# graphdeco-inria/hierarchical-3d-gaussians

Hardware: AMD Instinct MI355X
Metric: fwd+bwd frames/s @1080p, 1M Gaussians (higher is better)
Workload: dtype f32

## Files before the change

hierarchical-3d-gaussians_amd/csrc/abi.cpp:

```cpp
#include "common.h"

#include <pthread.h>
#include <sched.h>
#include <stdlib.h>
#include <time.h>
#include <string.h>

#include <atomic>
#include <cmath>
#include <mutex>
#include <vector>

namespace hgs {

enum Stage { ST_PREPROCESS_FWD = 0, ST_SCAN, ST_DUPLICATE, ST_SORT, ST_RANGES, ST_SORT_DEPTH, ST_RENDER_FWD,
             ST_MEMSET_BWD, ST_RENDER_BWD, ST_PREPROCESS_BWD, ST_SH_BATCHED, ST_COUNT };
static const char* kStageNames[ST_COUNT] = {"preprocess_fwd", "scan", "duplicate_keys", "tile_sort", "tile_ranges",
                                            "tile_depth_sort", "render_fwd", "memset_bwd", "render_bwd",
                                            "preprocess_bwd", "sh_bwd_batched"};
struct Pending { int stage; hipEvent_t a, b; };
static uint32_t g_timing = 0;
static std::mutex g_tmu;
static std::vector<Pending> g_pending;
static std::vector<hipEvent_t> g_pool;
static double g_ms[ST_COUNT];
static uint32_t g_calls[ST_COUNT];

struct StageTimer {
  int stage; hipStream_t s; hipEvent_t a = nullptr, b = nullptr; bool on;
  StageTimer(int st, hipStream_t stream) : stage(st), s(stream), on((g_timing & (1u | (2u << st))) != 0) {
    if (!on) return;
    std::lock_guard<std::mutex> lk(g_tmu);
    for (hipEvent_t* e : {&a, &b}) {
      if (!g_pool.empty()) { *e = g_pool.back(); g_pool.pop_back(); }
      else if (hipEventCreate(e) != hipSuccess) { on = false; return; }
    }
    (void)hipEventRecord(a, s);
  }
  ~StageTimer() {
    if (!on) return;
    (void)hipEventRecord(b, s);
    std::lock_guard<std::mutex> lk(g_tmu);
    g_pending.push_back({stage, a, b});
  }
};
#define HGS_TIMED(stage, stream, expr) [&]() { hgs::StageTimer _t(stage, stream); return (expr); }()

static thread_local char g_err[512] = "";

constexpr int kMaxDevices = 16;
struct ThreadHost {
  uint32_t* pinned_L = nullptr;
  hipEvent_t ev[kMaxDevices] = {};
};
static pthread_key_t g_host_key;
static pthread_once_t g_host_once = PTHREAD_ONCE_INIT;
static void thread_host_free(void* p) {
  ThreadHost* h = static_cast<ThreadHost*>(p);
  if (!h) return;
  for (int i = 0; i < kMaxDevices; ++i)
    if (h->ev[i]) (void)hipEventDestroy(h->ev[i]);
  if (h->pinned_L) (void)hipHostFree(h->pinned_L);
  delete h;
}
static void thread_host_key_init() { (void)pthread_key_create(&g_host_key, thread_host_free); }
static ThreadHost* thread_host(int device) {
  if (device < 0 || device >= kMaxDevices) return nullptr;
  (void)pthread_once(&g_host_once, thread_host_key_init);
  ThreadHost* h = static_cast<ThreadHost*>(pthread_getspecific(g_host_key));
  if (!h) {
    h = new ThreadHost();
    if (hipHostMalloc(reinterpret_cast<void**>(&h->pinned_L), sizeof(uint32_t), hipHostMallocPortable | hipHostMallocMapped) != hipSuccess) {
      thread_host_free(h);
      return nullptr;
    }
    (void)pthread_setspecific(g_host_key, h);
  }
  if (!h->ev[device] && hipEventCreateWithFlags(&h->ev[device], hipEventDisableTiming) != hipSuccess) {
    h->ev[device] = nullptr;
    return nullptr;
  }
  return h;
}

static bool blocking_waits() {
  static const bool b = getenv("HGS_BLOCKING_WAIT") != nullptr;
  return b;
}
static inline void cpu_relax() {
#if defined(__x86_64__) || defined(__i386__)
  __builtin_ia32_pause();
#elif defined(__aarch64__) || defined(__arm__)
  __asm__ __volatile__("yield");
#else
  sched_yield();
#endif
}
template <typename Query>
static bool poll_done(Query query, hipError_t* result) {
  if (blocking_waits()) return false;
  timespec t0;
  clock_gettime(CLOCK_MONOTONIC, &t0);
  for (unsigned i = 0;; ++i) {
    const hipError_t q = query();
    if (q != hipErrorNotReady) { *result = q; return true; }
    (void)hipGetLastError();
    cpu_relax();
    if ((i & 255u) == 255u) {
      timespec t;
      clock_gettime(CLOCK_MONOTONIC, &t);
      if ((t.tv_sec - t0.tv_sec) * 1000000000LL + (t.tv_nsec - t0.tv_nsec) > 200000000LL) return false;
    }
  }
}
hipError_t wait_stream(hipStream_t s) {
  hipError_t r;
  if (poll_done([&] { return hipStreamQuery(s); }, &r)) return r;
  return hipStreamSynchronize(s);
}
hipError_t wait_event(hipEvent_t e) {
  hipError_t r;
  if (poll_done([&] { return hipEventQuery(e); }, &r)) return r;
  return hipEventSynchronize(e);
}

int scan_resident_workgroups() {
  static std::atomic<int> cus[kMaxDevices];
  static const bool masked = getenv("HSA_CU_MASK") || getenv("ROC_GLOBAL_CU_MASK") || getenv("HSA_CU_MASK_SKIP_INIT");
  if (masked) return 1;
  int dev = 0;
  if (hipGetDevice(&dev) != hipSuccess || dev < 0 || dev >= kMaxDevices) return 1;
  int n = cus[dev].load(std::memory_order_relaxed);
  if (n == 0) {
    if (hipDeviceGetAttribute(&n, hipDeviceAttributeMultiprocessorCount, dev) != hipSuccess || n < 1) n = 1;
    cus[dev].store(n, std::memory_order_relaxed);
  }
  return n;
}
bool scan_split_forced() {
  static const bool b = getenv("HGS_SCAN_SPLIT") != nullptr;
  return b;
}

void set_error(const char* fmt, ...) {
  va_list ap;
  va_start(ap, fmt);
  vsnprintf(g_err, sizeof(g_err), fmt, ap);
  va_end(ap);
}

size_t GeomWs::bytes(int32_t P) {
  const size_t p = (size_t)(P > 0 ? P : 1);
  const size_t nblk = (p + kPreBlock - 1) / kPreBlock;
  const size_t jac_rows = (p + 63) / 64 * 64;
  return align_up(p * kRecFloats * 4) + align_up(p * 4) + align_up(p * 8) + 3 * align_up(p * 4) +
         align_up((nblk + 1) * 4) + align_up((nblk + 1) * kBands * 4) + align_up(jac_rows * kJacStride * 4) +
         align_up((size_t)(1 + kBands) * scan_chunks(nblk) * 8) + kAlign;
}
GeomWs GeomWs::carve_from(void* base, int32_t P) {
  const size_t p = (size_t)(P > 0 ? P : 1);
  const size_t nblk = (p + kPreBlock - 1) / kPreBlock;
  const size_t jac_rows = (p + 63) / 64 * 64;
  char* c = static_cast<char*>(base);
  GeomWs g;
  g.records = carve<float>(c, p * kRecFloats);
  g.depths = carve<float>(c, p);
  g.rects = carve<uint32_t>(c, p * 2);
  g.tiles_touched = carve<uint32_t>(c, p);
  g.offsets = carve<uint32_t>(c, p);
  g.flags = carve<uint32_t>(c, p);
  g.block_sums = carve<uint32_t>(c, nblk + 1);
  g.block_band = carve<uint32_t>(c, (nblk + 1) * kBands);
  g.shjac = carve<float>(c, jac_rows * kJacStride);
  g.scan_chain = carve<unsigned long long>(c, (size_t)(1 + kBands) * scan_chunks(nblk));
  return g;
}

size_t BinWs::bytes(uint32_t L, int32_t T) {
  const size_t l = L ? L : 1;
  const size_t tmp_sort = sort_tmp_bytes(L ? L : 1), tmp_bin = tile_bin_tmp_bytes(L, T);
  return 4 * align_up(l * 4) + align_up((size_t)T * 8) + align_up(((size_t)T * 3 + 3) * 4) + align_up(((size_t)T + 8) * 4) +
         (tmp_sort > tmp_bin ? tmp_sort : tmp_bin) + kAlign;
}
BinWs BinWs::carve_from(void* base, uint32_t L, int32_t T) {
  const size_t l = L ? L : 1;
  char* c = static_cast<char*>(base);
  BinWs b;
  b.keys_in = carve<uint32_t>(c, l);
  b.vals_in = carve<uint32_t>(c, l);
  b.keys_out = carve<uint32_t>(c, l);
  b.vals_out = carve<uint32_t>(c, l);
  b.ranges = carve<uint32_t>(c, (size_t)T * 2);
  b.big_tiles = carve<uint32_t>(c, (size_t)T * 3 + 3);
  b.tile_order = carve<uint32_t>(c, (size_t)T + 8);
  b.sort_tmp = c;
  return b;
}

size_t ImgWs::bytes(int32_t W, int32_t H) { return 2 * align_up((size_t)W * H * 4) + kAlign; }
ImgWs ImgWs::carve_from(void* base, int32_t W, int32_t H) {
  char* c = static_cast<char*>(base);
  ImgWs im;
  im.final_T = carve<float>(c, (size_t)W * H);
  im.n_contrib = carve<uint32_t>(c, (size_t)W * H);
  return im;
}

static int validate(const hgs_raster_args* a) {
  if (!a) { set_error("null args"); return HGS_ERR_INVALID; }
  if (a->P < 0 || a->width <= 0 || a->height <= 0) { set_error("bad sizes P=%d W=%d H=%d", a->P, a->width, a->height); return HGS_ERR_INVALID; }
  if (grid_x(a->width) > 1023 || grid_y(a->height) > 1023) { set_error("image larger than 16368 px per side is not supported"); return HGS_ERR_INVALID; }
  if (!a->bg || !a->viewmatrix || !a->projmatrix || !a->campos) { set_error("bg/viewmatrix/projmatrix/campos must be device pointers"); return HGS_ERR_INVALID; }
  if (a->P > 0) {
    if (!a->means3D || !a->opacities) { set_error("means3D/opacities missing"); return HGS_ERR_INVALID; }
    if ((a->shs != nullptr) == (a->colors_precomp != nullptr)) { set_error("provide exactly one of shs / colors_precomp"); return HGS_ERR_INVALID; }
    const bool sr = a->scales && a->rotations;
    if (sr == (a->cov3D_precomp != nullptr) || ((a->scales != nullptr) != (a->rotations != nullptr))) {
      set_error("provide exactly one of (scales, rotations) / cov3D_precomp");
      return HGS_ERR_INVALID;
    }
    if (a->shs) {
      if (a->sh_degree < 0 || a->sh_degree > 3) { set_error("sh_degree %d not in 0..3", a->sh_degree); return HGS_ERR_INVALID; }
      if (a->M < (a->sh_degree + 1) * (a->sh_degree + 1) || a->M > 16) { set_error("M=%d incompatible with sh_degree=%d (max 16 coefficients)", a->M, a->sh_degree); return HGS_ERR_INVALID; }
    }
    if (((uintptr_t)a->shs | (uintptr_t)a->shs_rest | (uintptr_t)a->rotations) & 15u) { set_error("shs / shs_rest / rotations must be 16-byte aligned"); return HGS_ERR_INVALID; }
    if (a->defer_sh_bwd && a->shs_rest) { set_error("defer_sh_bwd is not available with split SH storage (shs_rest)"); return HGS_ERR_INVALID; }
    if (a->shs_rest && (!a->shs || a->M < 2)) { set_error("shs_rest needs shs (features_dc) and M >= 2"); return HGS_ERR_INVALID; }
    if ((a->activations & HGS_ACT_OPACITY_SIGMOID) && (a->activations & HGS_ACT_OPACITY_ABS)) { set_error("choose one opacity activation"); return HGS_ERR_INVALID; }
    if ((a->activations & (HGS_ACT_SCALE_EXP | HGS_ACT_ROT_NORMALIZE)) && a->cov3D_precomp) { set_error("scale / rotation activations need scales and rotations"); return HGS_ERR_INVALID; }
    if ((a->interpolation_weights != nullptr) != (a->num_node_kids != nullptr)) { set_error("interpolation_weights and num_node_kids must be given together"); return HGS_ERR_INVALID; }
    if ((a->lod_render_indices != nullptr) != (a->lod_parent_indices != nullptr)) { set_error("lod_render_indices and lod_parent_indices must be given together"); return HGS_ERR_INVALID; }
    if (a->lod_render_indices) {
      if (!a->shs || a->shs_rest || !a->scales || !a->rotations || a->activations || !a->interpolation_weights) { set_error("in-kernel LOD interpolation needs shs, scales, rotations, interpolation_weights / num_node_kids and no activations"); return HGS_ERR_INVALID; }
      if (a->lod_n < 0 || a->lod_n > a->P || a->lod_rows < a->P - a->lod_n) { set_error("bad lod_n / lod_rows (P=%d lod_n=%d lod_rows=%d)", a->P, a->lod_n, a->lod_rows); return HGS_ERR_INVALID; }
      if (a->defer_sh_bwd || a->accumulate_grads) { set_error("defer_sh_bwd / accumulate_grads are not available with in-kernel LOD interpolation"); return HGS_ERR_INVALID; }
    }
  }
  return HGS_OK;
}

}

using namespace hgs;

extern "C" {

int hgs_abi_version(void) { return HGS_ABI_VERSION; }
const char* hgs_last_error(void) { return g_err; }
int hgs_device_count(void) {
  int n = 0;
  if (hipGetDeviceCount(&n) != hipSuccess) return -1;
  return n;
}

int hgs_raster_ws_sizes(int32_t P, int32_t width, int32_t height, uint32_t L, size_t* geom_bytes,
                        size_t* bin_bytes, size_t* img_bytes, size_t* bwd_bytes) {
  if (P < 0 || width <= 0 || height <= 0) { set_error("bad sizes"); return HGS_ERR_INVALID; }
  const int T = grid_x(width) * grid_y(height);
  if (geom_bytes) *geom_bytes = GeomWs::bytes(P);
  if (bin_bytes) *bin_bytes = BinWs::bytes(L, T);
  if (img_bytes) *img_bytes = ImgWs::bytes(width, height);
  if (bwd_bytes) *bwd_bytes = bwd_ws_bytes(L, P);
  return HGS_OK;
}

int hgs_raster_fwd_stage1(const hgs_raster_args* a, void* geom_ws, int32_t* radii, uint32_t* L_out_host,
                          hgs_stream_t stream, int device) {
  int rc = validate(a);
  if (rc) return rc;
  if (!geom_ws || !L_out_host || (a->P > 0 && !radii)) { set_error("null workspace/output"); return HGS_ERR_INVALID; }
  HGS_HIP(hipSetDevice(device));
  hipStream_t s = static_cast<hipStream_t>(stream);
  const GeomWs g = GeomWs::carve_from(geom_ws, a->P);
  *L_out_host = 0;
  if (a->P == 0) return HGS_OK;
  if ((rc = HGS_TIMED(ST_PREPROCESS_FWD, s, launch_preprocess_fwd(*a, g, radii, s)))) return rc;
  if ((rc = HGS_TIMED(ST_SCAN, s, launch_scan_block_sums(g, a->P, s, a->debug)))) return rc;
  const int nblk = (a->P + kPreBlock - 1) / kPreBlock;
  HGS_HIP(hipMemcpyAsync(L_out_host, g.block_sums + nblk, sizeof(uint32_t), hipMemcpyDeviceToHost, s));
  HGS_HIP(wait_stream(s));
  return HGS_OK;
}

static int enqueue_stage2(const hgs_raster_args* a, const GeomWs& g, const BinWs& b, const ImgWs& im, uint32_t L,
                          const uint32_t* L_dev, int T, float* out_color, float* out_invdepth, hipStream_t s,
                          uint32_t* super = nullptr, uint32_t* mirror = nullptr, uint32_t* stage = nullptr,
                          hipEvent_t ev = nullptr) {
  int rc;
  const bool bin = L > 0 && tile_bin_supported(T);
  if ((rc = HGS_TIMED(ST_DUPLICATE, s, launch_duplicate_tiles(*a, g, b, L, bin, s, super, mirror)))) return rc;
  if (super) {
    if (!mirror) HGS_HIP(hipMemcpyAsync(stage, L_dev, sizeof(uint32_t), hipMemcpyDeviceToHost, s));
    HGS_HIP(hipEventRecord(ev, s));
  }
  if (bin) {
    const int nblk = (a->P + kPreBlock - 1) / kPreBlock;
    if ((rc = HGS_TIMED(ST_SORT, s, launch_tile_bin(b.keys_in, b.vals_in, b.vals_out, b.sort_tmp, L, g.block_band, nblk, T, b.ranges, b.big_tiles, b.tile_order, super, s, a->debug)))) return rc;
  } else {
    if (L > 0) {
      if ((rc = HGS_TIMED(ST_SORT, s, sort_pairs32(b.keys_in, b.vals_in, b.keys_out, b.vals_out, b.sort_tmp, L, L_dev, tile_bits(T), s, a->debug)))) return rc;
    }
    if ((rc = HGS_TIMED(ST_RANGES, s, launch_tile_ranges(b, L, L_dev, T, s, a->debug)))) return rc;
  }
  if ((rc = HGS_TIMED(ST_SORT_DEPTH, s, launch_tile_depth_sort(*a, g, b, L, T, bin && a->debug, s)))) return rc;
  if (!bin && (rc = launch_tile_order(b, T, s, a->debug))) return rc;
  return HGS_TIMED(ST_RENDER_FWD, s, launch_render_fwd(*a, g, b, im, out_color, out_invdepth, s));
}

int hgs_raster_fwd_stage2(const hgs_raster_args* a, void* geom_ws, void* bin_ws, void* img_ws, uint32_t L,
                          float* out_color, float* out_invdepth, hgs_stream_t stream, int device) {
  int rc = validate(a);
  if (rc) return rc;
  if (!geom_ws || !bin_ws || !img_ws || !out_color) { set_error("null workspace/output"); return HGS_ERR_INVALID; }
  HGS_HIP(hipSetDevice(device));
  hipStream_t s = static_cast<hipStream_t>(stream);
  const int T = grid_x(a->width) * grid_y(a->height);
  const GeomWs g = GeomWs::carve_from(geom_ws, a->P);
  const BinWs b = BinWs::carve_from(bin_ws, L, T);
  const ImgWs im = ImgWs::carve_from(img_ws, a->width, a->height);
  return enqueue_stage2(a, g, b, im, L, nullptr, T, out_color, out_invdepth, s);
}

int hgs_raster_fwd(const hgs_raster_args* a, void* geom_ws, void* bin_ws, void* img_ws, uint32_t L_cap,
                   int32_t* radii, float* out_color, float* out_invdepth, uint32_t* L_out_host,
                   hgs_stream_t stream, int device) {
  int rc = validate(a);
  if (rc) return rc;
  if (!geom_ws || !bin_ws || !img_ws || !out_color || !L_out_host || (a->P > 0 && !radii)) {
    set_error("null workspace/output");
    return HGS_ERR_INVALID;
  }
  HGS_HIP(hipSetDevice(device));
  hipStream_t s = static_cast<hipStream_t>(stream);
  const int T = grid_x(a->width) * grid_y(a->height);
  const GeomWs g = GeomWs::carve_from(geom_ws, a->P);
  const BinWs b = BinWs::carve_from(bin_ws, L_cap, T);
  const ImgWs im = ImgWs::carve_from(img_ws, a->width, a->height);
  *L_out_host = 0;
  if (a->P == 0) return enqueue_stage2(a, g, b, im, 0, nullptr, T, out_color, out_invdepth, s);
  ThreadHost* th = thread_host(device);
  if (!th) { set_error("cannot allocate pinned host memory / event (device %d)", device); return HGS_ERR_NOMEM; }
  hipEvent_t ev = th->ev[device];
  uint32_t* stage = th->pinned_L;
  static const bool by_copy = getenv("HGS_COUNT_BY_COPY") != nullptr;
  void* mirror = nullptr;
  if (by_copy || hipHostGetDevicePointer(&mirror, stage, 0) != hipSuccess) { (void)hipGetLastError(); mirror = nullptr; }
  const int nblk = (a->P + kPreBlock - 1) / kPreBlock;
  uint32_t* super = nullptr;
  if (L_cap > 0 && tile_bin_supported(T) && nblk <= kSuper * kMaxSuper) super = super_block_acquire(s);
  if ((rc = HGS_TIMED(ST_PREPROCESS_FWD, s, launch_preprocess_fwd(*a, g, radii, s, super, super ? k3_heavy_threshold(L_cap, a->P) : 0u)))) {
    if (super) super_block_mark_dirty(super);
    return rc;
  }
  const uint32_t* L_dev = g.block_sums + nblk;
  hipError_t e = hipSuccess;
  if (!super) {
    if ((rc = HGS_TIMED(ST_SCAN, s, launch_scan_block_sums(g, a->P, s, a->debug, static_cast<uint32_t*>(mirror))))) return rc;
    if (!mirror) HGS_HIP(hipMemcpyAsync(stage, L_dev, sizeof(uint32_t), hipMemcpyDeviceToHost, s));
    e = hipEventRecord(ev, s);
  }
  if (e == hipSuccess) rc = enqueue_stage2(a, g, b, im, L_cap, L_dev, T, out_color, out_invdepth, s, super,
                                           static_cast<uint32_t*>(mirror), stage, ev);
  if (rc || e != hipSuccess) {
    if (super) super_block_mark_dirty(super);
    if (rc) return rc;
  }
  if (e == hipSuccess) e = wait_event(ev);
  if (e != hipSuccess) { set_error("hgs_raster_fwd: %s", hipGetErrorString(e)); return HGS_ERR_HIP; }
  *L_out_host = *stage;
  if (rc) return rc;
  if (*L_out_host > L_cap) {
    if (super) {
      HGS_HIP(hipMemsetAsync(g.scan_chain, 0, (size_t)(1 + kBands) * scan_chunks(nblk) * sizeof(unsigned long long), s));
      if ((rc = launch_scan_block_sums(g, a->P, s, a->debug, nullptr))) return rc;
    }
    set_error("instance count %u exceeds the capacity %u given to hgs_raster_fwd", *L_out_host, L_cap);
    return HGS_ERR_CAPACITY;
  }
  return HGS_OK;
}

int hgs_release_device_state(int device) { return super_block_release(device); }

int hgs_raster_bwd(const hgs_raster_args* a, const void* geom_ws, const void* bin_ws, const void* img_ws,
                   void* bwd_ws, uint32_t L, const float* out_color, const float* out_invdepth,
                   const float* dL_dcolor, const float* dL_dinvdepth, const hgs_raster_grads* grads,
                   hgs_stream_t stream, int device) {
  int rc = validate(a);
  if (rc) return rc;
  if (!geom_ws || !bin_ws || !img_ws || !bwd_ws || !out_color || !dL_dcolor || !grads) { set_error("null workspace/input"); return HGS_ERR_INVALID; }
  if (a->lod_render_indices && !a->prepare_backward) { set_error("the backward of an in-kernel LOD interpolation needs prepare_backward = 1 in the forward and the backward call"); return HGS_ERR_INVALID; }
  if (a->lod_scatter && (!a->lod_render_indices || ((a->M * 3) & 3) != 0 || a->accumulate_grads || a->defer_sh_bwd)) { set_error("lod_scatter needs in-kernel LOD interpolation, 3M %% 4 == 0, no accumulation and no deferred SH backward"); return HGS_ERR_INVALID; }
  if (a->P > 0) {
    if (!grads->dL_dmeans3D || !grads->dL_dmeans2D || !grads->dL_dopacity) { set_error("missing gradient outputs"); return HGS_ERR_INVALID; }
    if ((a->shs && !grads->dL_dshs) || (a->shs_rest && !grads->dL_dshs_rest) || (a->colors_precomp && !grads->dL_dcolors) ||
        (a->scales && (!grads->dL_dscales || !grads->dL_drotations)) || (a->cov3D_precomp && !grads->dL_dcov3D)) {
      set_error("gradient outputs do not match the inputs that were provided");
      return HGS_ERR_INVALID;
    }
  }
  HGS_HIP(hipSetDevice(device));
  hipStream_t s = static_cast<hipStream_t>(stream);
  if (a->P == 0) return HGS_OK;
  const int T = grid_x(a->width) * grid_y(a->height);
  const GeomWs g = GeomWs::carve_from(const_cast<void*>(geom_ws), a->P);
  const BinWs b = BinWs::carve_from(const_cast<void*>(bin_ws), L, T);
  const ImgWs im = ImgWs::carve_from(const_cast<void*>(img_ws), a->width, a->height);
  float* inst = static_cast<float*>(bwd_ws);
  float* drgb = bwd_ws_drgb(bwd_ws, L);
  if (L > 0) {
    if ((rc = HGS_TIMED(ST_RENDER_BWD, s, launch_render_bwd(*a, g, b, im, out_color, out_invdepth, dL_dcolor, dL_dinvdepth, inst, s)))) return rc;
  }
  hgs_raster_grads gr = *grads;
  if (!a->shs) gr.dL_dshs = nullptr;
  if (!a->shs_rest) gr.dL_dshs_rest = nullptr;
  if (!a->colors_precomp) gr.dL_dcolors = nullptr;
  if (!a->scales) { gr.dL_dscales = nullptr; gr.dL_drotations = nullptr; }
  if (!a->cov3D_precomp) gr.dL_dcov3D = nullptr;
  uint32_t* lod_flag = nullptr;
  if (a->lod_render_indices && a->lod_scatter) {
    lod_flag = bwd_ws_lod_flag(bwd_ws, L, a->P);
    HGS_HIP(hipMemsetAsync(lod_flag, 0, sizeof(uint32_t), s));
    if ((rc = launch_lod_monotone(a->lod_parent_indices, a->lod_n, lod_flag, s))) return rc;
  }
  return HGS_TIMED(ST_PREPROCESS_BWD, s, launch_preprocess_bwd(*a, g, inst, drgb, bwd_ws_dmean(bwd_ws, L, a->P), lod_flag, gr, L,
                                                             bwd_ws_work(bwd_ws, L, a->P), bwd_ws_work_counter(bwd_ws, L, a->P), s));
}

int hgs_raster_sh_bwd_batched(const hgs_sh_bwd_view* views, int32_t n_views, int32_t P, int32_t M, int32_t sh_degree,
                              const float* means3D, const float* shs, float* dL_dshs, float* dL_dmeans3D,
                              int32_t accumulate, hgs_stream_t stream, int device) {
  if (n_views <= 0 || P <= 0) return HGS_OK;
  if (!views || n_views > HGS_MAX_DEFERRED_VIEWS) { set_error("1..%d deferred views per call", HGS_MAX_DEFERRED_VIEWS); return HGS_ERR_INVALID; }
  if (!means3D || !shs || !dL_dshs || !dL_dmeans3D) { set_error("null argument"); return HGS_ERR_INVALID; }
  if (sh_degree < 0 || sh_degree > 3 || M < (sh_degree + 1) * (sh_degree + 1) || M > 16) { set_error("M=%d incompatible with sh_degree=%d", M, sh_degree); return HGS_ERR_INVALID; }
  if (((uintptr_t)shs | (uintptr_t)dL_dshs) & 15u) { set_error("shs / dL_dshs must be 16-byte aligned"); return HGS_ERR_INVALID; }
  ShBwdViews v;
  v.n = n_views;
  v.color = 0;
  for (int i = 0; i < HGS_MAX_DEFERRED_VIEWS; ++i) {
    const hgs_sh_bwd_view& w = views[i < n_views ? i : 0];
    if (!w.geom_ws || !w.bwd_ws || !w.campos) { set_error("deferred view %d has a null pointer", i); return HGS_ERR_INVALID; }
    v.mask[i] = GeomWs::carve_from(const_cast<void*>(w.geom_ws), P).tiles_touched;
    v.drgb[i] = bwd_ws_drgb(const_cast<void*>(w.bwd_ws), w.L);
    v.campos[i] = w.campos;
  }
  HGS_HIP(hipSetDevice(device));
  return HGS_TIMED(ST_SH_BATCHED, static_cast<hipStream_t>(stream),
                   launch_sh_bwd_batched(v, P, M, sh_degree, means3D, shs, dL_dshs, dL_dmeans3D, accumulate != 0,
                                         static_cast<hipStream_t>(stream)));
}

static int sh_color_check(const hgs_sh_color_view* views, int32_t n_views, int32_t M, int32_t sh_degree,
                          const float* means3D, const float* shs, bool backward) {
  if (!views || n_views > HGS_MAX_DEFERRED_VIEWS) { set_error("1..%d views per call", HGS_MAX_DEFERRED_VIEWS); return HGS_ERR_INVALID; }
  if (!means3D || !shs) { set_error("null argument"); return HGS_ERR_INVALID; }
  if (sh_degree < 0 || sh_degree > 3 || M < (sh_degree + 1) * (sh_degree + 1) || M > 16) { set_error("M=%d incompatible with sh_degree=%d", M, sh_degree); return HGS_ERR_INVALID; }
  if ((uintptr_t)shs & 15u) { set_error("shs must be 16-byte aligned"); return HGS_ERR_INVALID; }
  for (int i = 0; i < n_views; ++i)
    if (!views[i].campos || !views[i].clamp || (backward ? !views[i].d_rgb : !views[i].rgb)) { set_error("colour view %d has a null pointer", i); return HGS_ERR_INVALID; }
  return HGS_OK;
}

int hgs_sh_colors_batched(const hgs_sh_color_view* views, int32_t n_views, int32_t P, int32_t M, int32_t sh_degree,
                          const float* means3D, const float* shs, hgs_stream_t stream, int device) {
  if (n_views <= 0 || P <= 0) return HGS_OK;
  int rc = sh_color_check(views, n_views, M, sh_degree, means3D, shs, false);
  if (rc) return rc;
  ShFwdViews v;
  v.n = n_views;
  for (int i = 0; i < HGS_MAX_DEFERRED_VIEWS; ++i) {
    const hgs_sh_color_view& w = views[i < n_views ? i : 0];
    v.campos[i] = w.campos;
    v.rgb_out[i] = w.rgb;
    v.clamp_out[i] = w.clamp;
  }
  HGS_HIP(hipSetDevice(device));
  return launch_sh_colors_batched(v, P, M, sh_degree, means3D, shs, static_cast<hipStream_t>(stream));
}

int hgs_sh_colors_batched_bwd(const hgs_sh_color_view* views, int32_t n_views, int32_t P, int32_t M, int32_t sh_degree,
                              const float* means3D, const float* shs, float* dL_dshs, float* dL_dmeans3D,
                              int32_t accumulate, hgs_stream_t stream, int device) {
  if (n_views <= 0 || P <= 0) return HGS_OK;
  if (!dL_dshs || !dL_dmeans3D || ((uintptr_t)dL_dshs & 15u)) { set_error("dL_dshs (16-byte aligned) / dL_dmeans3D missing"); return HGS_ERR_INVALID; }
  int rc = sh_color_check(views, n_views, M, sh_degree, means3D, shs, true);
  if (rc) return rc;
  ShBwdViews v;
  v.n = n_views;
  v.color = 1;
  for (int i = 0; i < HGS_MAX_DEFERRED_VIEWS; ++i) {
    const hgs_sh_color_view& w = views[i < n_views ? i : 0];
    v.mask[i] = w.clamp;
    v.drgb[i] = w.d_rgb;
    v.campos[i] = w.campos;
  }
  HGS_HIP(hipSetDevice(device));
  return HGS_TIMED(ST_SH_BATCHED, static_cast<hipStream_t>(stream),
                   launch_sh_bwd_batched(v, P, M, sh_degree, means3D, shs, dL_dshs, dL_dmeans3D, accumulate != 0,
                                         static_cast<hipStream_t>(stream)));
}

int hgs_raster_views_get(int32_t P, int32_t width, int32_t height, uint32_t L, const void* geom_ws,
                         const void* bin_ws, const void* img_ws, hgs_raster_views* out) {
  if (!out || !geom_ws || !bin_ws || !img_ws) { set_error("null argument"); return HGS_ERR_INVALID; }
  const int T = grid_x(width) * grid_y(height);
  const GeomWs g = GeomWs::carve_from(const_cast<void*>(geom_ws), P);
  const BinWs b = BinWs::carve_from(const_cast<void*>(bin_ws), L, T);
  const ImgWs im = ImgWs::carve_from(const_cast<void*>(img_ws), width, height);
  out->tile_ids_sorted = b.keys_out;
  out->point_list = b.vals_out;
  out->ranges = b.ranges;
  out->tiles_touched = g.tiles_touched;
  out->offsets = g.offsets;
  out->depths = g.depths;
  out->rects = g.rects;
  out->records = g.records;
  out->final_T = im.final_T;
  out->n_contrib = im.n_contrib;
  return HGS_OK;
}

int hgs_timing_enable(int on) {
  std::lock_guard<std::mutex> lk(g_tmu);
  g_timing = (uint32_t)on;
  return HGS_OK;
}
int hgs_timing_stage_count(void) { return ST_COUNT; }
const char* hgs_timing_stage_name(int i) { return (i >= 0 && i < ST_COUNT) ? kStageNames[i] : ""; }
int hgs_timing_read(double* ms_out, uint32_t* calls_out, int reset) {
  std::lock_guard<std::mutex> lk(g_tmu);
  for (const Pending& p : g_pending) {
    float ms = 0.f;
    if (hipEventSynchronize(p.b) == hipSuccess && hipEventElapsedTime(&ms, p.a, p.b) == hipSuccess) {
      g_ms[p.stage] += ms;
      g_calls[p.stage] += 1;
    }
    g_pool.push_back(p.a);
    g_pool.push_back(p.b);
  }
  g_pending.clear();
  for (int i = 0; i < ST_COUNT; ++i) {
    if (ms_out) ms_out[i] = g_ms[i];
    if (calls_out) calls_out[i] = g_calls[i];
    if (reset) { g_ms[i] = 0.0; g_calls[i] = 0; }
  }
  return HGS_OK;
}

size_t hgs_sort_tmp_bytes(uint32_t n) { return sort_tmp_bytes(n ? n : 1); }

int hgs_sort_pairs(const uint64_t* keys_in, const uint32_t* vals_in, uint64_t* keys_out, uint32_t* vals_out,
                   void* tmp, uint32_t n, int end_bit, hgs_stream_t stream, int device) {
  if (n && (!keys_in || !vals_in || !keys_out || !vals_out || !tmp)) { set_error("null argument"); return HGS_ERR_INVALID; }
  HGS_HIP(hipSetDevice(device));
  return sort_pairs(keys_in, vals_in, keys_out, vals_out, tmp, n, end_bit, static_cast<hipStream_t>(stream), false);
}

constexpr int32_t kHierBuildMaxP = 1 << 30;

size_t hgs_hier_build_tmp_bytes(int32_t P) {
  if (P < 1 || P > kHierBuildMaxP) return 0;
  return hier_build_tmp_bytes(P);
}

int hgs_hier_build(const float* xyz, const float* scales, const float* rots, const float* opacity, const float* shs,
                   int32_t P, int32_t M, float* out_xyz, float* out_shs, float* out_alpha, float* out_log_scales,
                   float* out_rots, int32_t* out_nodes, float* out_boxes, void* tmp, hgs_stream_t stream, int device) {
  if (P < 1 || P > kHierBuildMaxP) { set_error("bad sizes: P=%d not in [1, 2^30]", P); return HGS_ERR_INVALID; }
  if (M != 1 && M != 4 && M != 9 && M != 16) { set_error("bad sizes: M=%d not in {1, 4, 9, 16}", M); return HGS_ERR_INVALID; }
  if (!xyz || !scales || !rots || !opacity || !shs || !out_xyz || !out_shs || !out_alpha || !out_log_scales ||
      !out_rots || !out_nodes || !out_boxes || !tmp) {
    set_error("null argument");
    return HGS_ERR_INVALID;
  }
  if (((uintptr_t)out_shs | (uintptr_t)out_rots | (uintptr_t)out_boxes) & 15u) { set_error("out_shs / out_rots / out_boxes must be 16-byte aligned"); return HGS_ERR_INVALID; }
  if ((uintptr_t)tmp & (kAlign - 1)) { set_error("tmp must be %d-byte aligned", (int)kAlign); return HGS_ERR_INVALID; }
  HGS_HIP(hipSetDevice(device));
  return launch_hier_build(xyz, scales, rots, opacity, shs, P, M, out_xyz, out_shs, out_alpha, out_log_scales, out_rots,
// ... 127 lines not shown
```

hierarchical-3d-gaussians_amd/csrc/binning.hip:

```cpp
#include "common.h"

#include <stdlib.h>

namespace hgs {
namespace {

__device__ __forceinline__ void divmod_rect(uint32_t k, uint32_t w, uint32_t& q, uint32_t& r) {
  q = (uint32_t)(((float)k + 0.5f) * __builtin_amdgcn_rcpf((float)w));
  r = k - q * w;
}


__device__ __forceinline__ uint32_t rect_count(uint2 r) {
  return ((r.y & 0xffffu) - (r.x & 0xffffu)) * ((r.y >> 16) - (r.x >> 16));
}

__global__ __launch_bounds__(kPreBlock) void duplicate_tiles_kernel(int P, int gx, GeomWs g, uint32_t cap,
                                                                    uint32_t* __restrict__ tile_keys,
                                                                    uint32_t* __restrict__ vals,
                                                                    uint32_t* __restrict__ ranges, int n_ranges) {
  for (int r = blockIdx.x * kPreBlock + threadIdx.x; r < n_ranges; r += gridDim.x * kPreBlock) ranges[r] = 0u;
  __shared__ uint32_t excl[kPreBlock + 1];
  __shared__ uint2 lrect[kPreBlock];
  __shared__ uint32_t wave_tot[kPreBlock / 64];
  const int tid = threadIdx.x, lane = tid & 63, wave = tid >> 6;
  const int i = blockIdx.x * kPreBlock + tid;
  const uint32_t gid = (uint32_t)i;
  const uint2 myrect = (i < P) ? reinterpret_cast<const uint2*>(g.rects)[gid] : make_uint2(0u, 0u);
  const uint32_t cnt = rect_count(myrect);
  lrect[tid] = myrect;
  uint32_t inc = cnt;
#pragma unroll
  for (int off = 1; off < 64; off <<= 1) {
    const uint32_t t = __shfl_up(inc, off, 64);
    if (lane >= off) inc += t;
  }
  if (lane == 63) wave_tot[wave] = inc;
  __syncthreads();
  uint32_t wbase = 0;
  for (int w = 0; w < wave; ++w) wbase += wave_tot[w];
  const uint32_t my_excl = wbase + inc - cnt;
  excl[tid] = my_excl;
  if (tid == kPreBlock - 1) excl[kPreBlock] = wbase + inc;
  const uint32_t block_base = g.block_sums[blockIdx.x];
  if (i < P && cnt) g.offsets[gid] = block_base + my_excl;
  __syncthreads();
  const uint32_t total = excl[kPreBlock];
  for (uint32_t s = tid; s < total; s += kPreBlock) {
    int lo = 0, hi = kPreBlock;
#pragma unroll
    for (int it = 0; it < 8; ++it) {
      const int mid = (lo + hi) >> 1;
      if (excl[mid] <= s) lo = mid; else hi = mid;
    }
    const uint32_t gg = blockIdx.x * kPreBlock + lo;
    const uint32_t k = s - excl[lo];
    const uint2 rc = lrect[lo];
    const uint32_t minx = rc.x & 0xffffu, miny = rc.x >> 16;
    const uint32_t w = (rc.y & 0xffffu) - minx;
    uint32_t kq, kr;
    divmod_rect(k, w, kq, kr);
    const uint32_t ty = miny + kq, tx = minx + kr;
    if (block_base + s < cap) {
      tile_keys[block_base + s] = ty * (uint32_t)gx + tx;
      vals[block_base + s] = gg;
    }
  }
}


template <int CTRL, int ROW_MASK>
__device__ __forceinline__ uint32_t dpp_add_u32(uint32_t v) {
  return v + (uint32_t)__builtin_amdgcn_update_dpp(0, (int)v, CTRL, ROW_MASK, 0xf, false);
}
__device__ __forceinline__ uint32_t wave_scan_incl(uint32_t v) {
  v = dpp_add_u32<0x111, 0xf>(v);
  v = dpp_add_u32<0x112, 0xf>(v);
  v = dpp_add_u32<0x114, 0xf>(v);
  v = dpp_add_u32<0x118, 0xf>(v);
  v = dpp_add_u32<0x142, 0xa>(v);
  v = dpp_add_u32<0x143, 0xc>(v);
  return v;
}

constexpr uint32_t kHeavyFloor = 4096u, kHeavyFactor = 2u, kShareMin = 1024u;

struct K3Lds {
  uint32_t pre9[1 + kBands], tot9[1 + kBands];
  uint32_t excl[kPreBlock + 1];
  uint2 lrect[kPreBlock];
  uint32_t wave_tot[kPreBlock / 64][kBands + 1];
  uint32_t bpos[kBands];
  uint32_t rb[kBands][kPreBlock];
  uint32_t hl_blk[kMaxHeavy], hl_pe[kMaxHeavy + 1];
  uint32_t scan_tmp[kPreBlock / 64];
};

__device__ __forceinline__ uint32_t k3_wg_scan_excl(uint32_t v, uint32_t* tmp, uint32_t& total) {
  const int lane = threadIdx.x & 63, wave = threadIdx.x >> 6;
  const uint32_t inc = wave_scan_incl(v);
  __syncthreads();
  if (lane == 63) tmp[wave] = inc;
  __syncthreads();
  uint32_t base = 0, t = 0;
#pragma unroll
  for (int w = 0; w < kPreBlock / 64; ++w) {
    const uint32_t x = tmp[w];
    base += (w < wave) ? x : 0u;
    t += x;
  }
  total = t;
  return base + inc - v;
}

template <bool OWN>
__device__ __forceinline__ void k3_prologue(K3Lds& l, int blk, int nblk, int P, int gx, int T, int per, const GeomWs& g,
                                            const uint32_t* __restrict__ super, uint32_t* __restrict__ total_mirror,
                                            uint32_t& heavy_n) {
  const int tid = threadIdx.x, lane = tid & 63, wave = tid >> 6;
  const int i = blk * kPreBlock + tid;
  const uint32_t gid = (uint32_t)i;
  const uint2 myrect = (i < P) ? reinterpret_cast<const uint2*>(g.rects)[gid] : make_uint2(0u, 0u);
  const int col = nblk + 1;
  uint32_t block_base = 0;
  uint32_t band_tot = 0, band_off = 0;
  heavy_n = 0u;
  if (!super) {
    block_base = g.block_sums[blk];
    if (tid < kBands) {
      band_tot = g.block_band[(size_t)tid * col + nblk];
      band_off = g.block_band[(size_t)tid * col + blk];
    }
  } else {
    const int sb = blk / kSuper, nsb = (nblk + kSuper - 1) / kSuper;
    constexpr int kWaves = kPreBlock / 64, kPer = (1 + kBands + kWaves - 1) / kWaves;
    uint32_t pre[kPer], x0[kPer];
    const int j = min(sb * kSuper + lane, blk);
#pragma unroll
    for (int u = 0; u < kPer; ++u) {
      const int a = min(wave + u * kWaves, kBands);
      const uint32_t* raw = a == 0 ? g.block_sums : g.block_band + (size_t)(a - 1) * col;
      pre[u] = raw[j];
      x0[u] = super[a * kMaxSuper + min(lane, nsb - 1)];
    }
    if constexpr (OWN) heavy_n = super[kHeavyRow];
#pragma unroll
    for (int u = 0; u < kPer; ++u) {
      const int a = min(wave + u * kWaves, kBands);
      uint32_t p = (sb * kSuper + lane < blk) ? pre[u] : 0u;
      uint32_t tot = (lane < nsb) ? x0[u] : 0u;
      p += (lane < sb) ? tot : 0u;
      for (int s0 = 64; s0 < nsb; s0 += 64) {
        const uint32_t x = (s0 + lane < nsb) ? super[a * kMaxSuper + s0 + lane] : 0u;
        tot += x;
        p += (s0 + lane < sb) ? x : 0u;
      }
      p = wave_scan_incl(p);
      tot = wave_scan_incl(tot);
      if (lane == 63) { l.pre9[a] = p; l.tot9[a] = tot; }
    }
  }
  const uint32_t cnt = rect_count(myrect);
  l.lrect[tid] = myrect;
  uint32_t cb[kBands];
#pragma unroll
  for (int b = 0; b < kBands; ++b) cb[b] = 0u;
  if (cnt) {
    const int minx = (int)(myrect.x & 0xffffu), miny = (int)(myrect.x >> 16);
    const int maxx = (int)(myrect.y & 0xffffu), maxy = (int)(myrect.y >> 16);
    const int w = maxx - minx;
    const int t_first = miny * gx + minx, t_last = (maxy - 1) * gx + maxx - 1;
    int b_first = 0, b_last = 0;
#pragma unroll
    for (int b = 1; b < kBands; ++b) {
      b_first += (t_first >= b * per) ? 1 : 0;
      b_last += (t_last >= b * per) ? 1 : 0;
    }
    if (b_first == b_last) {
#pragma unroll
      for (int b = 0; b < kBands; ++b) cb[b] = (b == b_first) ? cnt : 0u;
    } else {
      int prev = 0;
#pragma unroll
      for (int b = 0; b < kBands; ++b) {
        const int x = min((b + 1) * per, T);
        const int xr = x / gx, xc = x - xr * gx;
        int c = (min(max(xr, miny), maxy) - miny) * w;
        if (xr >= miny && xr < maxy) c += min(max(xc - minx, 0), w);
        cb[b] = (uint32_t)(c - prev);
        prev = c;
      }
    }
  }
  const uint32_t inc = wave_scan_incl(cnt);
  uint32_t incb[kBands];
#pragma unroll
  for (int b = 0; b < kBands; ++b) incb[b] = wave_scan_incl(cb[b]);
  if (lane == 63) {
    l.wave_tot[wave][kBands] = inc;
#pragma unroll
    for (int b = 0; b < kBands; ++b) l.wave_tot[wave][b] = incb[b];
  }
  if (!super && wave == 0) {
    const uint32_t incl = wave_scan_incl(tid < kBands ? band_tot : 0u);
    if (tid < kBands) l.bpos[tid] = incl - band_tot + band_off;
  }
  __syncthreads();
  if (super) {
    block_base = l.pre9[0];
    if (wave == 0) {
      if (tid < kBands) { band_tot = l.tot9[1 + tid]; band_off = l.pre9[1 + tid]; }
      const uint32_t incl = wave_scan_incl(tid < kBands ? band_tot : 0u);
      if (tid < kBands) l.bpos[tid] = incl - band_tot + band_off;
    }
    if (OWN && blk == nblk - 1 && tid <= kBands) {
      uint32_t* arr = tid == 0 ? g.block_sums : g.block_band + (size_t)(tid - 1) * col;
      arr[nblk] = l.tot9[tid];
      if (tid == 0 && total_mirror) *total_mirror = l.tot9[0];
    }
  }
  uint32_t wbase = 0;
  for (int w = 0; w < wave; ++w) wbase += l.wave_tot[w][kBands];
  const uint32_t my_excl = wbase + inc - cnt;
  l.excl[tid] = my_excl;
  if (tid == kPreBlock - 1) l.excl[kPreBlock] = wbase + inc;
  {
    uint32_t below = 0;
#pragma unroll
    for (int b = 0; b < kBands; ++b) {
      uint32_t wb = 0;
      for (int w = 0; w < wave; ++w) wb += l.wave_tot[w][b];
      l.rb[b][tid] = wb + incb[b] - cb[b] - below;
      below += cb[b];
    }
  }
  if (OWN && i < P && cnt) g.offsets[gid] = block_base + my_excl;
  __syncthreads();
}

__device__ __attribute__((noinline)) void k3_prologue_other(K3Lds* l, int blk, int nblk, int P, int gx, int T, int per,
                                                            uint32_t* rects, uint32_t* block_sums, uint32_t* block_band,
                                                            const uint32_t* super) {
  GeomWs g{};
  g.rects = rects;
  g.block_sums = block_sums;
  g.block_band = block_band;
  uint32_t unused;
  k3_prologue<false>(*l, blk, nblk, P, gx, T, per, g, super, nullptr, unused);
}

__device__ __forceinline__ void k3_emit(const K3Lds& l, int blk, uint32_t s_begin, uint32_t s_end, int gx, int per,
                                        uint32_t cap, uint32_t* __restrict__ tile_keys, uint32_t* __restrict__ vals) {
  const float rcp_per = __builtin_amdgcn_rcpf((float)per);
  for (uint32_t s = s_begin + threadIdx.x; s < s_end; s += kPreBlock) {
    int lo = 0, hi = kPreBlock;
#pragma unroll
    for (int it = 0; it < 8; ++it) {
      const int mid = (lo + hi) >> 1;
      if (l.excl[mid] <= s) lo = mid; else hi = mid;
    }
    const uint32_t gg = (uint32_t)blk * kPreBlock + lo;
    const uint32_t k = s - l.excl[lo];
    const uint2 rc = l.lrect[lo];
    const uint32_t minx = rc.x & 0xffffu, miny = rc.x >> 16;
    const uint32_t w = (rc.y & 0xffffu) - minx;
    uint32_t kq, kr;
    divmod_rect(k, w, kq, kr);
    const uint32_t tile = (miny + kq) * (uint32_t)gx + minx + kr;
    const uint32_t band = (uint32_t)(((float)tile + 0.5f) * rcp_per);
    const uint32_t pos = l.bpos[band] + l.rb[band][lo] + k;
    if (pos < cap) {
      tile_keys[pos] = tile - band * (uint32_t)per;
      vals[pos] = gg;
    }
  }
}

__global__ __launch_bounds__(kPreBlock) void duplicate_tiles_banded_kernel(int P, int gx, int T, int per, GeomWs g,
                                                                           uint32_t cap,
                                                                           uint32_t* __restrict__ tile_keys,
                                                                           uint32_t* __restrict__ vals,
                                                                           uint32_t* __restrict__ ranges, int n_ranges,
                                                                           const uint32_t* __restrict__ super,
                                                                           uint32_t* __restrict__ total_mirror,
                                                                           uint32_t* __restrict__ zero_words, int n_zero,
                                                                           int share_max, uint32_t thr) {
  for (int r = blockIdx.x * kPreBlock + threadIdx.x; r < n_ranges; r += gridDim.x * kPreBlock) ranges[r] = 0u;
  for (int r = blockIdx.x * kPreBlock + threadIdx.x; r < n_zero; r += gridDim.x * kPreBlock) zero_words[r] = 0u;
  __shared__ K3Lds l;
  const int tid = threadIdx.x, nblk = (int)gridDim.x, own = (int)blockIdx.x;
  uint32_t heavy_n;
  k3_prologue<true>(l, own, nblk, P, gx, T, per, g, super, total_mirror, heavy_n);
  const uint32_t total = l.excl[kPreBlock];
  if (!(super && share_max > 0 && thr != 0u && heavy_n != 0u)) {
    k3_emit(l, own, 0u, total, gx, per, cap, tile_keys, vals);
    return;
  }
  const int nh = (int)min(min(heavy_n, (uint32_t)kMaxHeavy), (uint32_t)share_max);
  if (tid < nh) {
    l.hl_blk[tid] = super[kHeavyRow + 1 + 2 * tid];
    l.hl_pe[tid] = super[kHeavyRow + 2 + 2 * tid] - thr;
  }
  __syncthreads();
  const uint32_t e = tid < nh ? l.hl_pe[tid] : 0u;
  const bool mine_listed = tid < nh && l.hl_blk[tid] == (uint32_t)own;
  uint32_t E;
  const uint32_t pe = k3_wg_scan_excl(e, l.scan_tmp, E);
  if (tid < nh) l.hl_pe[tid] = pe;
  if (tid == 0) l.hl_pe[nh] = E;
  const bool own_listed = __syncthreads_or(mine_listed) != 0;
  k3_emit(l, own, 0u, own_listed ? thr : total, gx, per, cap, tile_keys, vals);
  const uint64_t q = max((uint64_t)kShareMin, ((uint64_t)E + (uint64_t)nblk - 1u) / (uint64_t)nblk);
  const uint64_t lo = (uint64_t)own * q, hi = min(lo + q, (uint64_t)E);
  if (lo >= hi) return;
#pragma nounroll
  for (int i = 0; i < nh; ++i) {
    const uint64_t p0 = (uint32_t)__builtin_amdgcn_readfirstlane((int)l.hl_pe[i]);
    const uint64_t p1 = (uint32_t)__builtin_amdgcn_readfirstlane((int)l.hl_pe[i + 1]);
    if (p1 <= lo) continue;
    if (p0 >= hi) break;
    const int blk = __builtin_amdgcn_readfirstlane((int)l.hl_blk[i]);
    const uint32_t s0 = thr + (uint32_t)(max(lo, p0) - p0), s1 = thr + (uint32_t)(min(hi, p1) - p0);
    __syncthreads();
    k3_prologue_other(&l, blk, nblk, P, gx, T, per, g.rects, g.block_sums, g.block_band, super);
    k3_emit(l, blk, s0, s1, gx, per, cap, tile_keys, vals);
  }
}

constexpr uint32_t kLargeCap = 16384;

template <typename T>
__device__ __forceinline__ void cmp_swap(T& a, T& b, bool up) {
  const bool sw = (a > b) == up;
  const T lo = sw ? b : a, hi = sw ? a : b;
  a = lo;
  b = hi;
}

template <int LX>
__device__ __forceinline__ uint32_t lane_xor32(uint32_t v, int lane) {
  if constexpr (LX == 1) {
    return (uint32_t)__builtin_amdgcn_mov_dpp((int)v, 0xB1, 0xf, 0xf, true);
  } else if constexpr (LX == 2) {
    return (uint32_t)__builtin_amdgcn_mov_dpp((int)v, 0x4E, 0xf, 0xf, true);
  } else if constexpr (LX == 8) {
    return (uint32_t)__builtin_amdgcn_mov_dpp((int)v, 0x128, 0xf, 0xf, true);
  } else if constexpr (LX == 16) {
    const auto r = __builtin_amdgcn_permlane16_swap(v, v, false, false);
    return (lane & 16) ? r[0] : r[1];
  } else if constexpr (LX == 32) {
    const auto r = __builtin_amdgcn_permlane32_swap(v, v, false, false);
    return (lane & 32) ? r[0] : r[1];
  } else {
    return (uint32_t)__shfl_xor((int)v, LX, 64);
  }
}
template <int LX>
__device__ __forceinline__ uint64_t lane_xor64(uint64_t v, int lane) {
  return ((uint64_t)lane_xor32<LX>((uint32_t)(v >> 32), lane) << 32) | lane_xor32<LX>((uint32_t)v, lane);
}

template <int LX>
__device__ __forceinline__ uint64_t lane_xor(uint64_t v, int lane) { return lane_xor64<LX>(v, lane); }
template <int LX>
__device__ __forceinline__ uint32_t lane_xor(uint32_t v, int lane) { return lane_xor32<LX>(v, lane); }

template <int E, int K, int J, typename T>
__device__ __forceinline__ void wave_sort_stage(T (&key)[E], int lane, uint32_t base) {
  if constexpr (J >= E) {
    constexpr int LX = J / E;
    const bool lower = (lane & LX) == 0;
// ... 675 lines not shown
```

hierarchical-3d-gaussians_amd/csrc/common.h:

```cpp
#pragma once
#include <hip/hip_runtime.h>
#include <stdint.h>
#include <stddef.h>
#include <stdio.h>
#include <stdarg.h>

#include "../../include/hgs.h"

namespace hgs {

void set_error(const char* fmt, ...);

#define HGS_HIP(call)                                                                   \
  do {                                                                                  \
    hipError_t _e = (call);                                                             \
    if (_e != hipSuccess) {                                                             \
      hgs::set_error("%s:%d: %s -> %s", __FILE__, __LINE__, #call, hipGetErrorString(_e)); \
      return HGS_ERR_HIP;                                                               \
    }                                                                                   \
  } while (0)

#define HGS_LAUNCH_CHECK(name, stream, debug)                                           \
  do {                                                                                  \
    hipError_t _e = hipGetLastError();                                                  \
    if (_e == hipSuccess && (debug)) _e = hipStreamSynchronize(stream);                 \
    if (_e != hipSuccess) {                                                             \
      hgs::set_error("kernel %s failed: %s", name, hipGetErrorString(_e));              \
      return HGS_ERR_HIP;                                                               \
    }                                                                                   \
  } while (0)

constexpr size_t kAlign = 256;
inline size_t align_up(size_t x) { return (x + kAlign - 1) / kAlign * kAlign; }

template <typename T>
inline T* carve(char*& p, size_t count) {
  T* r = reinterpret_cast<T*>(p);
  p += align_up(count * sizeof(T));
  return r;
}

constexpr int kTile = HGS_TILE;
constexpr int kRecFloats = 16;
constexpr int kRecVec = kRecFloats / 4;
constexpr int kInstStride = HGS_INST_GRAD_STRIDE;
constexpr int kJacStride = 9;
constexpr int kPreBlock = 256;
constexpr int kBands = 8;
__host__ __device__ inline int band_tiles(int T) { return (T + kBands - 1) / kBands; }

struct GeomWs {
  float* records;
  float* depths;
  uint32_t* rects;
  uint32_t* tiles_touched;
  uint32_t* offsets;
  uint32_t* flags;
  uint32_t* block_sums;
  uint32_t* block_band;
  float* shjac;
  unsigned long long* scan_chain;
  static size_t bytes(int32_t P);
  static GeomWs carve_from(void* base, int32_t P);
};

struct BinWs {
  uint32_t* keys_in;
  uint32_t* vals_in;
  uint32_t* keys_out;
  uint32_t* vals_out;
  uint32_t* ranges;
  uint32_t* big_tiles;
  uint32_t* tile_order;
  void* sort_tmp;
  static size_t bytes(uint32_t L, int32_t T);
  static BinWs carve_from(void* base, uint32_t L, int32_t T);
};

struct ImgWs {
  float* final_T;
  uint32_t* n_contrib;
  static size_t bytes(int32_t W, int32_t H);
  static ImgWs carve_from(void* base, int32_t W, int32_t H);
};

inline int grid_x(int W) { return (W + kTile - 1) / kTile; }
inline int grid_y(int H) { return (H + kTile - 1) / kTile; }
inline int tile_bits(int T) {
  int b = 0;
  while ((1 << b) < T) ++b;
  return b < 1 ? 1 : b;
}

constexpr int kScanPer = 8;
constexpr int kScanChunk = 1024 * kScanPer;
__host__ __device__ inline int scan_chunks(size_t n) { return (int)((n + kScanChunk - 1) / kScanChunk) + (n == 0 ? 1 : 0); }

#ifdef __HIPCC__
__device__ __forceinline__ uint32_t chained_scan_inplace(uint32_t* __restrict__ sums, int n,
                                                         unsigned long long* __restrict__ chain, int c_off = 0,
                                                         int chunks_all = 0) {
  __shared__ uint32_t scan_wave_tot[16];
  __shared__ uint32_t scan_prefix;
  const int tid = threadIdx.x, lane = tid & 63, wave = tid >> 6;
  const int c = (int)blockIdx.x + c_off, chunks = chunks_all ? chunks_all : (int)gridDim.x;
  const int i0 = c * kScanChunk + tid * kScanPer;
  uint32_t v[kScanPer], mine = 0;
#pragma unroll
  for (int k = 0; k < kScanPer; ++k) v[k] = sums[max(min(i0 + k, n - 1), 0)];
#pragma unroll
  for (int k = 0; k < kScanPer; ++k) {
    v[k] = (i0 + k < n) ? v[k] : 0u;
    mine += v[k];
  }
  uint32_t inc = mine;
#pragma unroll
  for (int off = 1; off < 64; off <<= 1) {
    const uint32_t t = __shfl_up(inc, off, 64);
    if (lane >= off) inc += t;
  }
  if (lane == 63) scan_wave_tot[wave] = inc;
  __syncthreads();
  uint32_t wbase = 0, total = 0;
#pragma unroll
  for (int w = 0; w < 16; ++w) {
    const uint32_t t = scan_wave_tot[w];
    wbase += (w < wave) ? t : 0u;
    total += t;
  }
  if (tid == 0) __hip_atomic_store(&chain[c], (1ull << 32) | (unsigned long long)total, __ATOMIC_RELEASE, __HIP_MEMORY_SCOPE_AGENT);
  if (wave == 0) {
    uint32_t before = 0;
    for (int q = lane; q < c; q += 64) {
      unsigned long long x;
      do { x = __hip_atomic_load(&chain[q], __ATOMIC_ACQUIRE, __HIP_MEMORY_SCOPE_AGENT); } while ((x >> 32) == 0ull);
      before += (uint32_t)x;
    }
#pragma unroll
    for (int off = 32; off > 0; off >>= 1) before += __shfl_xor(before, off, 64);
    if (lane == 0) scan_prefix = before;
  }
  __syncthreads();
  const uint32_t prefix = scan_prefix;
  uint32_t run = prefix + wbase + inc - mine;
#pragma unroll
  for (int k = 0; k < kScanPer; ++k) {
    if (i0 + k < n) sums[i0 + k] = run;
    run += v[k];
  }
  if (c != chunks - 1) return 0u;
  if (tid == 0) sums[n] = prefix + total;
  return prefix + total;
}
#endif

hipError_t wait_stream(hipStream_t s);
hipError_t wait_event(hipEvent_t e);

int scan_resident_workgroups();
bool scan_split_forced();

int launch_preprocess_fwd(const hgs_raster_args& a, const GeomWs& g, int32_t* radii, hipStream_t s,
                          uint32_t* super = nullptr, uint32_t heavy_thr = 0);
constexpr int kSuper = 64;
constexpr int kMaxSuper = 1024;
constexpr int kMaxHeavy = 256;
constexpr int kHeavyRow = (1 + kBands) * kMaxSuper;
static_assert(1 + 2 * kMaxHeavy <= kMaxSuper, "the heavy list fits the row");
uint32_t k3_heavy_threshold(uint32_t L_cap, int32_t P);
uint32_t* super_block_acquire(hipStream_t s);
size_t super_block_bytes();
void super_block_mark_dirty(const uint32_t* words);
int super_block_release(int device);
int launch_scan_block_sums(const GeomWs& g, int32_t P, hipStream_t s, bool debug, uint32_t* total_mirror = nullptr);
int launch_duplicate_tiles(const hgs_raster_args& a, const GeomWs& g, const BinWs& b, uint32_t L_cap, bool banded,
                           hipStream_t s, const uint32_t* super = nullptr, uint32_t* total_mirror = nullptr);
uint32_t* tile_bin_zero_words(void* tmp, uint32_t L_cap, int32_t T);
int tile_bin_zero_count(int32_t T);
int launch_tile_ranges(const BinWs& b, uint32_t L_cap, const uint32_t* L_dev, int32_t T, hipStream_t s, bool debug);
int launch_tile_order(const BinWs& b, int32_t T, hipStream_t s, bool debug);
int launch_tile_depth_sort(const hgs_raster_args& a, const GeomWs& g, const BinWs& b, uint32_t L, int32_t T,
                           bool fill_tile_ids, hipStream_t s);
int launch_render_fwd(const hgs_raster_args& a, const GeomWs& g, const BinWs& b, const ImgWs& im,
                      float* out_color, float* out_invdepth, hipStream_t s);
int launch_render_bwd(const hgs_raster_args& a, const GeomWs& g, const BinWs& b, const ImgWs& im,
                      const float* out_color, const float* out_invdepth, const float* dL_dcolor,
                      const float* dL_dinvdepth, float* inst_grads, hipStream_t s);
int launch_preprocess_bwd(const hgs_raster_args& a, const GeomWs& g, const float* inst_grads, float* drgb,
                          float* dmean_rows, const uint32_t* lod_flag, const hgs_raster_grads& out, uint32_t L,
                          uint2* work, uint32_t* work_counter, hipStream_t s);
int launch_lod_monotone(const int32_t* parent_indices, int32_t n, uint32_t* flag, hipStream_t s);
struct ShBwdViews {
  const void* mask[HGS_MAX_DEFERRED_VIEWS];
  const float* drgb[HGS_MAX_DEFERRED_VIEWS];
  const float* campos[HGS_MAX_DEFERRED_VIEWS];
  int n;
  int color;
};
struct ShFwdViews {
  const float* campos[HGS_MAX_DEFERRED_VIEWS];
  float* rgb_out[HGS_MAX_DEFERRED_VIEWS];
  uint8_t* clamp_out[HGS_MAX_DEFERRED_VIEWS];
  int n;
};
int launch_sh_colors_batched(const ShFwdViews& v, int32_t P, int32_t M, int32_t sh_degree, const float* means3D,
                             const float* shs, hipStream_t s);
int launch_sh_bwd_batched(const ShBwdViews& v, int32_t P, int32_t M, int32_t sh_degree, const float* means3D,
                          const float* shs, float* dL_dshs, float* dL_dmeans3D, bool accumulate, hipStream_t s);
inline float* bwd_ws_drgb(void* bwd_ws, uint32_t L) {
  return reinterpret_cast<float*>(static_cast<char*>(bwd_ws) + align_up((size_t)(L ? L : 1) * kInstStride * 4));
}
inline float* bwd_ws_dmean(void* bwd_ws, uint32_t L, int32_t P) {
  return reinterpret_cast<float*>(reinterpret_cast<char*>(bwd_ws_drgb(bwd_ws, L)) + align_up((size_t)(P > 0 ? P : 1) * 3 * 4));
}
inline uint32_t* bwd_ws_lod_flag(void* bwd_ws, uint32_t L, int32_t P) {
  return reinterpret_cast<uint32_t*>(reinterpret_cast<char*>(bwd_ws_dmean(bwd_ws, L, P)) + align_up((size_t)(P > 0 ? P : 1) * 3 * 4));
}
constexpr uint32_t kK8LongRun = 48;
constexpr uint32_t kK8Seg = 512;
inline uint32_t* bwd_ws_work_counter(void* bwd_ws, uint32_t L, int32_t P) { return bwd_ws_lod_flag(bwd_ws, L, P) + 16; }
inline uint2* bwd_ws_work(void* bwd_ws, uint32_t L, int32_t P) {
  return reinterpret_cast<uint2*>(reinterpret_cast<char*>(bwd_ws_lod_flag(bwd_ws, L, P)) + kAlign);
}
inline size_t bwd_ws_work_items(uint32_t L) { return (size_t)(L ? L : 1) / kK8LongRun + 2; }
inline size_t bwd_ws_bytes(uint32_t L, int32_t P) {
  return align_up((size_t)(L ? L : 1) * kInstStride * 4) + 2 * align_up((size_t)(P > 0 ? P : 1) * 3 * 4) + 2 * kAlign +
         align_up(bwd_ws_work_items(L) * sizeof(uint2));
}
bool tile_bin_supported(int32_t T);
size_t tile_bin_tmp_bytes(uint32_t L, int32_t T);
int launch_tile_bin(const uint32_t* keys, const uint32_t* vals, uint32_t* vals_out, void* tmp, uint32_t L_cap,
                    const uint32_t* band_totals, int32_t nblk, int32_t T, uint32_t* ranges, uint32_t* big,
                    uint32_t* tile_order, uint32_t* super, hipStream_t s, bool debug);
size_t sort_tmp_bytes(uint32_t n);
int sort_pairs(const uint64_t* keys_in, const uint32_t* vals_in, uint64_t* keys_out, uint32_t* vals_out,
               void* tmp, uint32_t n, int end_bit, hipStream_t s, bool debug);
int sort_pairs32(const uint32_t* keys_in, const uint32_t* vals_in, uint32_t* keys_out, uint32_t* vals_out,
                 void* tmp, uint32_t n, const uint32_t* n_dev, int end_bit, hipStream_t s, bool debug);
size_t hier_build_tmp_bytes(int32_t P);
int launch_hier_build(const float* xyz, const float* scales, const float* rots, const float* opacity, const float* shs,
                      int32_t P, int32_t M, float* out_xyz, float* out_shs, float* out_alpha, float* out_log_scales,
                      float* out_rots, int32_t* out_nodes, float* out_boxes, void* tmp, hipStream_t s);
int launch_hier_merge_place(const hgs_hier_view& chunk, int32_t index, int64_t base, const hgs_hier_view& merged,
                            void* tmp, hgs_hier_merge_report* report, hipStream_t s);
int launch_hier_merge_root(const hgs_hier_view& merged, int32_t k, hipStream_t s);
size_t hier_align_tmp_bytes(int64_t N);
int launch_hier_align(const int32_t* nodes, int64_t N, float* log_scales, float* rots, void* tmp,
                      hgs_hier_align_report* report, hipStream_t s);
bool ssim_sizes_ok(int32_t N, int32_t C, int32_t H, int32_t W);
size_t ssim_tmp_bytes(int32_t N, int32_t C, int32_t H, int32_t W);
int launch_ssim_fwd(const float* img1, const float* img2, int32_t N, int32_t C, int32_t H, int32_t W,
                    float* out_image, float* out_mean, float* maps, void* tmp, hipStream_t s);
int launch_ssim_bwd(const float* img1, const float* img2, const float* maps, const float* grad_out, int32_t per_image,
                    int32_t N, int32_t C, int32_t H, int32_t W, float* grad_img1, hipStream_t s);
size_t photo_tmp_bytes(int32_t N, int32_t C, int32_t H, int32_t W);
int launch_photo_fwd(const hgs_photo_args& a, float* out, float* maps, void* tmp, hipStream_t s);
int launch_photo_bwd(const hgs_photo_args& a, const float* maps, const float* grad_out, float* grad_rendered,
                     float* grad_exposure, float* grad_invdepth, void* tmp, hipStream_t s);

}
```

hierarchical-3d-gaussians_amd/csrc/gaussian_math.h:

```cpp
#pragma once
#include "common.h"

namespace hgs {

struct Proj {
  float tx, ty, tz;
  float hx, hy, hw, pw;
  float txc, tyc;
  bool clampx, clampy;
  float fx, fy;
  float J00, J02, J11, J12;
  float T0[3], T1[3];
  float U0[3], U1[3];
  float c3[6];
  float a, b, c, det;
  float conA, conB, conC;
  float px, py;
  float rad_f;
  int minx, miny, maxx, maxy;
  bool visible;
};

__device__ __forceinline__ void quat_to_rot(const float q[4], float R[9]) {
#pragma clang fp contract(off)
// ... 84 lines not shown
#pragma unroll
  for (int j = 0; j < 3; ++j) {
    o.U0[j] = (o.T0[0] * S[0][j] + o.T0[1] * S[1][j]) + o.T0[2] * S[2][j];
    o.U1[j] = (o.T1[0] * S[0][j] + o.T1[1] * S[1][j]) + o.T1[2] * S[2][j];
  }
  o.a = ((o.U0[0] * o.T0[0] + o.U0[1] * o.T0[1]) + o.U0[2] * o.T0[2]) + 0.3f;
  o.b = (o.U0[0] * o.T1[0] + o.U0[1] * o.T1[1]) + o.U0[2] * o.T1[2];
  o.c = ((o.U1[0] * o.T1[0] + o.U1[1] * o.T1[1]) + o.U1[2] * o.T1[2]) + 0.3f;
  o.det = o.a * o.c - o.b * o.b;
  if (o.det == 0.0f) o.visible = false;
  const float det_inv = 1.0f / o.det;
  o.conA = o.c * det_inv;
  o.conB = (-o.b) * det_inv;
  o.conC = o.a * det_inv;

  const float mid = 0.5f * (o.a + o.c);
  const float disc = fmaxf(0.1f, mid * mid - o.det);
  const float sq = sqrtf(disc);
  const float lam = fmaxf(mid + sq, mid - sq);
  o.rad_f = ceilf(3.0f * sqrtf(lam));
  o.px = ((ndcx + 1.0f) * (float)W - 1.0f) * 0.5f;
  o.py = ((ndcy + 1.0f) * (float)H - 1.0f) * 0.5f;
  o.minx = tile_clamp(o.px - o.rad_f, gx);
  o.maxx = tile_clamp(o.px + o.rad_f + 15.0f, gx);
  o.miny = tile_clamp(o.py - o.rad_f, gy);
  o.maxy = tile_clamp(o.py + o.rad_f + 15.0f, gy);
  const bool finite = (fabsf(o.rad_f) <= 3.0e38f) && (fabsf(o.px) <= 3.0e38f) && (fabsf(o.py) <= 3.0e38f);
  if (!finite || (o.maxx - o.minx) * (o.maxy - o.miny) <= 0) o.visible = false;
}


__device__ __forceinline__ double rcp_d(double d) {
  const double r = (double)__builtin_amdgcn_rcpf((float)d);
  return fma(fma(-d, r, 1.0), r, r);
}

struct ProjD {
  double tx, ty, tz, hx, hy, hw, pw, itz, di;
  double txc, tyc, fx, fy;
  double T0[3], T1[3], U0[3], U1[3];
  double c3[6];
  double R[9], s[3];
  double a, b, c, det, conA, conB, conC;
  double px, py;
};

__device__ __forceinline__ void cov3d_from_scale_rot_d(const float sc[3], float mod, const float q[4], ProjD& o) {
  const double r = q[0], x = q[1], y = q[2], z = q[3];
  o.s[0] = (double)mod * sc[0];
  o.s[1] = (double)mod * sc[1];
  o.s[2] = (double)mod * sc[2];
  double* R = o.R;
  R[0] = 1.0 - 2.0 * (y * y + z * z); R[1] = 2.0 * (x * y - r * z);       R[2] = 2.0 * (x * z + r * y);
  R[3] = 2.0 * (x * y + r * z);       R[4] = 1.0 - 2.0 * (x * x + z * z); R[5] = 2.0 * (y * z - r * x);
  R[6] = 2.0 * (x * z - r * y);       R[7] = 2.0 * (y * z + r * x);       R[8] = 1.0 - 2.0 * (x * x + y * y);
  double L[9];
#pragma unroll
  for (int i = 0; i < 3; ++i)
#pragma unroll
    for (int k = 0; k < 3; ++k) L[i * 3 + k] = R[i * 3 + k] * o.s[k];
  int n = 0;
#pragma unroll
  for (int i = 0; i < 3; ++i)
#pragma unroll
    for (int j = i; j < 3; ++j)
      o.c3[n++] = L[i * 3 + 0] * L[j * 3 + 0] + L[i * 3 + 1] * L[j * 3 + 1] + L[i * 3 + 2] * L[j * 3 + 2];
}

__device__ __forceinline__ void project_gaussian_d(const float p[3], const float* vm, const float* pm, int W, int H,
                                                   float tanfovx, float tanfovy, bool clampx, bool clampy,
                                                   ProjD& o) {
  const double x = p[0], y = p[1], z = p[2];
  o.tx = (double)vm[0] * x + (double)vm[4] * y + (double)vm[8] * z + (double)vm[12];
  o.ty = (double)vm[1] * x + (double)vm[5] * y + (double)vm[9] * z + (double)vm[13];
  o.tz = (double)vm[2] * x + (double)vm[6] * y + (double)vm[10] * z + (double)vm[14];
  o.hx = (double)pm[0] * x + (double)pm[4] * y + (double)pm[8] * z + (double)pm[12];
  o.hy = (double)pm[1] * x + (double)pm[5] * y + (double)pm[9] * z + (double)pm[13];
  o.hw = (double)pm[3] * x + (double)pm[7] * y + (double)pm[11] * z + (double)pm[15];
  o.pw = rcp_d(o.hw + 1e-7);
  o.px = ((o.hx * o.pw + 1.0) * (double)W - 1.0) * 0.5;
  o.py = ((o.hy * o.pw + 1.0) * (double)H - 1.0) * 0.5;
  o.fx = (double)W / (2.0 * (double)tanfovx);
  o.fy = (double)H / (2.0 * (double)tanfovy);
  const double limx = 1.3 * (double)tanfovx, limy = 1.3 * (double)tanfovy;
  o.txc = clampx ? (o.tx < 0.0 ? -limx : limx) * o.tz : o.tx;
  o.tyc = clampy ? (o.ty < 0.0 ? -limy : limy) * o.tz : o.ty;
  const double itz = o.itz = rcp_d(o.tz);
  const double J00 = o.fx * itz, J02 = -(o.fx * o.txc) * itz * itz;
  const double J11 = o.fy * itz, J12 = -(o.fy * o.tyc) * itz * itz;
#pragma unroll
  for (int j = 0; j < 3; ++j) {
    o.T0[j] = J00 * (double)vm[j * 4 + 0] + J02 * (double)vm[j * 4 + 2];
    o.T1[j] = J11 * (double)vm[j * 4 + 1] + J12 * (double)vm[j * 4 + 2];
  }
  const double* c3 = o.c3;
  const double S[3][3] = {{c3[0], c3[1], c3[2]}, {c3[1], c3[3], c3[4]}, {c3[2], c3[4], c3[5]}};
#pragma unroll
  for (int j = 0; j < 3; ++j) {
    o.U0[j] = o.T0[0] * S[0][j] + o.T0[1] * S[1][j] + o.T0[2] * S[2][j];
    o.U1[j] = o.T1[0] * S[0][j] + o.T1[1] * S[1][j] + o.T1[2] * S[2][j];
  }
  o.a = o.U0[0] * o.T0[0] + o.U0[1] * o.T0[1] + o.U0[2] * o.T0[2] + 0.3;
  o.b = o.U0[0] * o.T1[0] + o.U0[1] * o.T1[1] + o.U0[2] * o.T1[2];
  o.c = o.U1[0] * o.T1[0] + o.U1[1] * o.T1[1] + o.U1[2] * o.T1[2] + 0.3;
  o.det = o.a * o.c - o.b * o.b;
  const double di = o.di = rcp_d(o.det);
  o.conA = o.c * di;
  o.conB = -o.b * di;
  o.conC = o.a * di;
}

struct LodRow {
  size_t r, p;
  float w, u;
};
template <bool LOD>
__device__ __forceinline__ LodRow lod_row(const hgs_raster_args& a, int idx) {
  LodRow l;
  if constexpr (!LOD) { l.r = l.p = (size_t)idx; l.w = 1.0f; l.u = 0.0f; return l; }
  if (idx < a.lod_n) {
    l.r = (size_t)a.lod_render_indices[idx];
    l.p = (size_t)a.lod_parent_indices[idx];
    l.w = a.interpolation_weights[idx];
    l.u = 1.0f - l.w;
  } else {
    l.r = l.p = (size_t)(a.lod_rows - (a.P - a.lod_n) + (idx - a.lod_n));
    l.w = 1.0f; l.u = 0.0f;
  }
  return l;
}
template <bool LOD>
__device__ __forceinline__ LodRow lod_row_gather(const hgs_raster_args& a, int idx) {
  LodRow l = lod_row<LOD>(a, idx);
  if constexpr (LOD) {
    if (l.w == 1.0f) l.p = l.r;
  }
  return l;
}
__device__ __forceinline__ float lod_lerp(float x, float y, float w, float u) {
#pragma clang fp contract(off)
  const float a = w * x, b = u * y;
  return a + b;
}
template <bool LOD>
__device__ __forceinline__ void load_mean(const hgs_raster_args& a, const LodRow& l, float p[3]) {
#pragma unroll
  for (int k = 0; k < 3; ++k) {
    const float x = a.means3D[l.r * 3 + k];
    if constexpr (LOD) p[k] = lod_lerp(x, a.means3D[l.p * 3 + k], l.w, l.u);
    else p[k] = x;
  }
}

template <bool LOD>
__device__ __forceinline__ void load_scale_rot(const hgs_raster_args& a, int idx, float sc[3], float q[4],
                                               double* nrm) {
  if constexpr (LOD) {
    const LodRow l = lod_row_gather<true>(a, idx);
#pragma unroll
    for (int k = 0; k < 3; ++k) sc[k] = lod_lerp(a.scales[l.r * 3 + k], a.scales[l.p * 3 + k], l.w, l.u);
    const float4 qa = reinterpret_cast<const float4*>(a.rotations)[l.r];
    float4 qb = reinterpret_cast<const float4*>(a.rotations)[l.p];
    const float sgn = (qa.x * qb.x + qa.y * qb.y + qa.z * qb.z + qa.w * qb.w) < 0.0f ? -1.0f : 1.0f;
    q[0] = lod_lerp(qa.x, sgn * qb.x, l.w, l.u); q[1] = lod_lerp(qa.y, sgn * qb.y, l.w, l.u);
    q[2] = lod_lerp(qa.z, sgn * qb.z, l.w, l.u); q[3] = lod_lerp(qa.w, sgn * qb.w, l.w, l.u);
    if (nrm) *nrm = 1.0;
    return;
  }
  sc[0] = a.scales[idx * 3 + 0]; sc[1] = a.scales[idx * 3 + 1]; sc[2] = a.scales[idx * 3 + 2];
  if (a.activations & HGS_ACT_SCALE_EXP) {
#pragma unroll
    for (int i = 0; i < 3; ++i) sc[i] = (float)exp((double)sc[i]);
  }
  const float4 qv = reinterpret_cast<const float4*>(a.rotations)[idx];
  q[0] = qv.x; q[1] = qv.y; q[2] = qv.z; q[3] = qv.w;
  double n = 1.0;
  if (a.activations & HGS_ACT_ROT_NORMALIZE) {
    const double w = q[0], x = q[1], y = q[2], z = q[3];
    n = fmax(sqrt(((w * w + x * x) + y * y) + z * z), 1e-12);
    q[0] = (float)(w / n); q[1] = (float)(x / n); q[2] = (float)(y / n); q[3] = (float)(z / n);
  }
  if (nrm) *nrm = n;
}

template <bool LOD>
__device__ __forceinline__ float load_opacity(const hgs_raster_args& a, int idx, double* dact) {
  if constexpr (LOD) {
    const LodRow l = lod_row_gather<true>(a, idx);
    if (dact) *dact = 1.0;
    return lod_lerp(a.opacities[l.r], a.opacities[l.p], l.w, l.u);
  }
  const float raw = a.opacities[idx];
  if (a.activations & HGS_ACT_OPACITY_SIGMOID) {
    const double o = 1.0 / (1.0 + exp(-(double)raw));
    if (dact) *dact = o * (1.0 - o);
    return (float)o;
  }
  if (a.activations & HGS_ACT_OPACITY_ABS) {
    if (dact) *dact = raw > 0.f ? 1.0 : (raw < 0.f ? -1.0 : 0.0);
    return fabsf(raw);
  }
  if (dact) *dact = 1.0;
  return raw;
}

__device__ __forceinline__ float lod_opacity(float o, float w, int kids, float* dout_do) {
  if (kids < 2) {
    if (dout_do) *dout_do = 1.0f;
    return o;
  }
  const float invk = 1.0f / (float)kids;
  const float oc = fminf(o, 0.99f);
  const float base = 1.0f - oc;
  const float pw = powf(base, invk);
  if (dout_do) {
    const float dstack = (o < 0.99f) ? invk * pw / base : 0.0f;
    *dout_do = w + (1.0f - w) * dstack;
  }
  return w * o + (1.0f - w) * (1.0f - pw);
}

__device__ __forceinline__ float unit_dir(const float p[3], const float* cam, float& dx, float& dy, float& dz) {
#pragma clang fp contract(off)
  dx = p[0] - cam[0]; dy = p[1] - cam[1]; dz = p[2] - cam[2];
  const float inv = 1.0f / sqrtf((dx * dx + dy * dy) + dz * dz);
  dx *= inv; dy *= inv; dz *= inv;
  return inv;
}

constexpr float SH_C0 = 0.28209479177387814f;
constexpr float SH_C1 = 0.4886025119029199f;
constexpr float SH_C2_0 = 1.0925484305920792f;
constexpr float SH_C2_1 = -1.0925484305920792f;
constexpr float SH_C2_2 = 0.31539156525252005f;
constexpr float SH_C2_3 = -1.0925484305920792f;
constexpr float SH_C2_4 = 0.5462742152960396f;
constexpr float SH_C3_0 = -0.5900435899266435f;
constexpr float SH_C3_1 = 2.890611442640554f;
constexpr float SH_C3_2 = -0.4570457994644658f;
constexpr float SH_C3_3 = 0.3731763325901154f;
constexpr float SH_C3_4 = -0.4570457994644658f;
constexpr float SH_C3_5 = 1.445305721320277f;
constexpr float SH_C3_6 = -0.5900435899266435f;

__device__ __forceinline__ void sh_basis(int deg, float x, float y, float z, float b[16]) {
#pragma clang fp contract(off)
  b[0] = SH_C0;
  if (deg > 0) {
    b[1] = -SH_C1 * y;
    b[2] = SH_C1 * z;
    b[3] = -SH_C1 * x;
    if (deg > 1) {
      const float xx = x * x, yy = y * y, zz = z * z, xy = x * y, yz = y * z, xz = x * z;
      b[4] = SH_C2_0 * xy;
      b[5] = SH_C2_1 * yz;
      b[6] = SH_C2_2 * (2.0f * zz - xx - yy);
      b[7] = SH_C2_3 * xz;
      b[8] = SH_C2_4 * (xx - yy);
      if (deg > 2) {
        b[9] = SH_C3_0 * y * (3.0f * xx - yy);
        b[10] = SH_C3_1 * xy * z;
        b[11] = SH_C3_2 * y * (4.0f * zz - xx - yy);
        b[12] = SH_C3_3 * z * (2.0f * zz - 3.0f * xx - 3.0f * yy);
        b[13] = SH_C3_4 * x * (4.0f * zz - xx - yy);
        b[14] = SH_C3_5 * z * (xx - yy);
        b[15] = SH_C3_6 * x * (xx - 3.0f * yy);
      }
    }
  }
}

__device__ __forceinline__ void sh_basis_grad(int deg, float x, float y, float z, float dbx[16],
                                              float dby[16], float dbz[16]) {
#pragma clang fp contract(off)
  dbx[0] = dby[0] = dbz[0] = 0.0f;
  if (deg > 0) {
    dbx[1] = 0.0f;      dby[1] = -SH_C1;    dbz[1] = 0.0f;
    dbx[2] = 0.0f;      dby[2] = 0.0f;      dbz[2] = SH_C1;
    dbx[3] = -SH_C1;    dby[3] = 0.0f;      dbz[3] = 0.0f;
    if (deg > 1) {
      const float xx = x * x, yy = y * y, zz = z * z, xy = x * y, yz = y * z, xz = x * z;
      dbx[4] = SH_C2_0 * y;          dby[4] = SH_C2_0 * x;          dbz[4] = 0.0f;
      dbx[5] = 0.0f;                 dby[5] = SH_C2_1 * z;          dbz[5] = SH_C2_1 * y;
      dbx[6] = SH_C2_2 * -2.0f * x;  dby[6] = SH_C2_2 * -2.0f * y;  dbz[6] = SH_C2_2 * 4.0f * z;
      dbx[7] = SH_C2_3 * z;          dby[7] = 0.0f;                 dbz[7] = SH_C2_3 * x;
      dbx[8] = SH_C2_4 * 2.0f * x;   dby[8] = SH_C2_4 * -2.0f * y;  dbz[8] = 0.0f;
      if (deg > 2) {
        dbx[9] = SH_C3_0 * 6.0f * xy;               dby[9] = SH_C3_0 * (3.0f * xx - 3.0f * yy);      dbz[9] = 0.0f;
        dbx[10] = SH_C3_1 * yz;                     dby[10] = SH_C3_1 * xz;                          dbz[10] = SH_C3_1 * xy;
        dbx[11] = SH_C3_2 * -2.0f * xy;             dby[11] = SH_C3_2 * (4.0f * zz - xx - 3.0f * yy); dbz[11] = SH_C3_2 * 8.0f * yz;
        dbx[12] = SH_C3_3 * -6.0f * xz;             dby[12] = SH_C3_3 * -6.0f * yz;                  dbz[12] = SH_C3_3 * (6.0f * zz - 3.0f * xx - 3.0f * yy);
        dbx[13] = SH_C3_4 * (4.0f * zz - 3.0f * xx - yy); dby[13] = SH_C3_4 * -2.0f * xy;            dbz[13] = SH_C3_4 * 8.0f * xz;
        dbx[14] = SH_C3_5 * 2.0f * xz;              dby[14] = SH_C3_5 * -2.0f * yz;                  dbz[14] = SH_C3_5 * (xx - yy);
        dbx[15] = SH_C3_6 * (3.0f * xx - 3.0f * yy); dby[15] = SH_C3_6 * -6.0f * xy;                 dbz[15] = 0.0f;
      }
    }
  }
}

}
```

hierarchical-3d-gaussians_amd/csrc/preprocess.hip:

```cpp
#include "gaussian_math.h"

#include <stdlib.h>

#include <mutex>

namespace hgs {

namespace {

struct CamLds {
  float vm[16];
  float pm[16];
  float cam[3];
};

__device__ __forceinline__ void load_camera(const hgs_raster_args& a, CamLds& c) {
#pragma unroll
  for (int i = 0; i < 16; ++i) {
    c.vm[i] = a.viewmatrix[i];
    c.pm[i] = a.projmatrix[i];
  }
  c.cam[0] = a.campos[0];
  c.cam[1] = a.campos[1];
  c.cam[2] = a.campos[2];
// ... 277 lines not shown
  const char* src = reinterpret_cast<const char*>(shs + (size_t)block_first * 48);
  const int wave_base = (int)(threadIdx.x & ~63u);
  constexpr int kPer = 12;
#pragma unroll
  for (int k = 0; k < kPer; ++k) {
    const int slot = k * kPreBlock + (int)threadIdx.x;
    const int row_l = slot / 12, cs = slot - row_l * 12;
    int c = cs - ((row_l >> 2) & 3);
    c = c < 0 ? c + 12 : c;
    const int row = row_l;
    char* dst = reinterpret_cast<char*>(lds) + (size_t)(k * kPreBlock + wave_base) * 16;
    if (row < count && c < nchunks)
      __builtin_amdgcn_global_load_lds((gptr_t)(src + (size_t)row * 192 + c * 16), (lptr_t)dst, 16, 0, 0);
  }
}
template <int Q>
__device__ __forceinline__ void sh48_read_row_quarter(const float* lds, int row_l, float v[12]) {
  const int f = (row_l >> 2) & 3;
  const float* row = lds + row_l * 48;
#pragma unroll
  for (int c = 0; c < 3; ++c) {
    int sl = Q * 3 + c + f;
    sl = sl >= 12 ? sl - 12 : sl;
    const float4 t = *reinterpret_cast<const float4*>(row + sl * 4);
    v[c * 4 + 0] = t.x; v[c * 4 + 1] = t.y; v[c * 4 + 2] = t.z; v[c * 4 + 3] = t.w;
  }
}
template <bool JAC>
__device__ __forceinline__ void sh48_row_from_lds(const float* lds, int row_l, bool vis, int deg, float dx, float dy,
                                                  float dz, float rgb[3], float J[9]) {
  const int nb = (deg + 1) * (deg + 1);
  float sh[12];
  sh48_read_row_quarter<0>(lds, row_l, sh);
  if (vis) sh48_accumulate4<JAC, 0>(deg, dx, dy, dz, sh, rgb, J);
  if (nb > 4) {
    sh48_read_row_quarter<1>(lds, row_l, sh);
    if (vis) sh48_accumulate4<JAC, 4>(deg, dx, dy, dz, sh, rgb, J);
    if (nb > 8) {
      sh48_read_row_quarter<2>(lds, row_l, sh);
      if (vis) sh48_accumulate4<JAC, 8>(deg, dx, dy, dz, sh, rgb, J);
      sh48_read_row_quarter<3>(lds, row_l, sh);
      if (vis) sh48_accumulate4<JAC, 12>(deg, dx, dy, dz, sh, rgb, J);
    }
  }
}

__device__ __forceinline__ void k1_band_count(const Proj& pr, uint32_t touched, int gx, int gy, uint32_t* band_cnt) {
  const int T = gx * gy, per = band_tiles(T), w = pr.maxx - pr.minx;
  const int t_first = pr.miny * gx + pr.minx, t_last = (pr.maxy - 1) * gx + pr.maxx - 1;
  int b_first = 0, b_last = 0;
#pragma unroll
  for (int b = 1; b < kBands; ++b) {
    b_first += (t_first >= b * per) ? 1 : 0;
    b_last += (t_last >= b * per) ? 1 : 0;
  }
  if (b_first == b_last) {
    atomicAdd(&band_cnt[b_first], touched);
  } else {
    int prev = 0;
    for (int b = b_first; b <= b_last; ++b) {
      const int x = min((b + 1) * per, T);
      const int xr = x / gx, xc = x - xr * gx;
      int cnt = (min(max(xr, pr.miny), pr.maxy) - pr.miny) * w;
      if (xr >= pr.miny && xr < pr.maxy) cnt += min(max(xc - pr.minx, 0), w);
      if (cnt > prev) atomicAdd(&band_cnt[b], (uint32_t)(cnt - prev));
      prev = cnt;
    }
  }
}

struct K1Rec {
  float opac, thr, ext_x, ext_y, invz;
  float gx_hi, gy_hi, gx_lo, gy_lo, A2, B2, C2;
};
__device__ __forceinline__ void k1_continuous(const hgs_raster_args& a, const CamLds& cam, const Proj& pr,
                                              const float p[3], const float sc_act[3], const float q_act[4],
                                              float opac, K1Rec& o) {
  o.opac = opac;
  ProjD pd;
  if (a.cov3D_precomp) {
#pragma unroll
    for (int i = 0; i < 6; ++i) pd.c3[i] = (double)pr.c3[i];
  } else {
    cov3d_from_scale_rot_d(sc_act, a.scale_modifier, q_act, pd);
  }
  project_gaussian_d(p, cam.vm, cam.pm, a.width, a.height, a.tanfovx, a.tanfovy, pr.clampx, pr.clampy, pd);
  o.gx_hi = (float)pd.px; o.gy_hi = (float)pd.py;
  o.gx_lo = (float)(pd.px - (double)o.gx_hi); o.gy_lo = (float)(pd.py - (double)o.gy_hi);
  const double kLog2e = 1.4426950408889634;
  o.A2 = (float)(-0.5 * kLog2e * pd.conA);
  o.B2 = (float)(-kLog2e * pd.conB);
  o.C2 = (float)(-0.5 * kLog2e * pd.conC);
  {
    const double lim = 4.0 * (double)o.A2 * (double)o.C2;
    if (!((double)o.B2 * (double)o.B2 < lim)) o.B2 = (float)copysign(sqrt(fmax(lim, 0.0)) * (1.0 - 1.0e-6), (double)o.B2);
  }
  o.thr = (-7.994353436858858f - 1.0e-3f) - __builtin_amdgcn_logf(opac);
  o.ext_x = -1.0f; o.ext_y = -1.0f;
  {
    const float T2 = -1.3862943611198906f * o.thr;
    const float sxx = (float)pd.a, syy = (float)pd.c;
    if (T2 > 0.0f) {
      const bool sane = sxx < 3.0e38f && syy < 3.0e38f;
      o.ext_x = sane ? sqrtf(T2 * sxx) * 1.0001f + 5.0e-3f : 1.0e9f;
      o.ext_y = sane ? sqrtf(T2 * syy) * 1.0001f + 5.0e-3f : 1.0e9f;
    }
  }
  o.invz = (float)pd.itz;
}

template <int NV>
__device__ __forceinline__ void wave_store_rows(float4* __restrict__ dst, size_t row0, const float4 (&v)[NV],
                                                unsigned long long mask, float4* wave_lds) {
  const int lane = threadIdx.x & 63;
#pragma unroll
  for (int q = 0; q < NV; ++q) wave_lds[lane * NV + q] = v[q];
  __builtin_amdgcn_fence(__ATOMIC_RELEASE, "wavefront");
  __builtin_amdgcn_wave_barrier();
  __builtin_amdgcn_fence(__ATOMIC_ACQUIRE, "wavefront");
#pragma unroll
  for (int j = 0; j < NV; ++j) {
    const int i = j * 64 + lane;
    const int r = i / NV;
    const float4 t = wave_lds[i];
    if ((mask >> r) & 1ull) dst[row0 * NV + i] = t;
  }
  __builtin_amdgcn_fence(__ATOMIC_RELEASE, "wavefront");
  __builtin_amdgcn_wave_barrier();
}

__device__ __forceinline__ void wave_store_jac(float* __restrict__ dst, size_t row0, const float (&J)[9],
                                               unsigned long long mask, float4* wave_lds) {
  const int lane = threadIdx.x & 63;
  float* wl = reinterpret_cast<float*>(wave_lds);
#pragma unroll
  for (int k = 0; k < 9; ++k) wl[lane * 9 + k] = J[k];
  __builtin_amdgcn_fence(__ATOMIC_RELEASE, "wavefront");
  __builtin_amdgcn_wave_barrier();
  __builtin_amdgcn_fence(__ATOMIC_ACQUIRE, "wavefront");
  float4* d4 = reinterpret_cast<float4*>(dst + row0 * kJacStride);
  if (mask) {
#pragma unroll
    for (int j = 0; j < 3; ++j) {
      const int i = j * 64 + lane;
      if (i < 64 * 9 / 4) d4[i] = wave_lds[i];
    }
  }
  __builtin_amdgcn_fence(__ATOMIC_RELEASE, "wavefront");
  __builtin_amdgcn_wave_barrier();
}

template <bool JAC, bool LOD, bool DEFER, bool H48>
__device__ __forceinline__ void preprocess_fwd_body(const hgs_raster_args& a, const GeomWs& g,
                                                    int32_t* __restrict__ radii, uint32_t* __restrict__ super, uint32_t heavy_thr) {
  static_assert(!(H48 && (LOD || DEFER)), "the DMA route is the plain layout's");
  extern __shared__ __attribute__((aligned(16))) unsigned char smem_raw[];
  float* lds_sh = reinterpret_cast<float*>(smem_raw);
  __shared__ uint32_t wave_tot[kPreBlock / 64];
  __shared__ uint32_t band_cnt[kBands];
  if (threadIdx.x < kBands) band_cnt[threadIdx.x] = 0u;
  if (!super && blockIdx.x == 0)
    for (int t = threadIdx.x; t < (1 + kBands) * scan_chunks(gridDim.x); t += kPreBlock) g.scan_chain[t] = 0ull;
  __syncthreads();
  const int idx = blockIdx.x * kPreBlock + threadIdx.x;
  const int gx = (a.width + kTile - 1) / kTile;
  const int gy = (a.height + kTile - 1) / kTile;
  CamLds cam;
  load_camera(a, cam);

  uint32_t touched = 0;
  Proj pr;
  pr.visible = false;
  float p[3] = {0.f, 0.f, 0.f};
  float sc_act[3] = {0.f, 0.f, 0.f}, q_act[4] = {1.f, 0.f, 0.f, 0.f};
  float opac = 0.f;
  constexpr bool lod = LOD;
  const int shn = a.M * 3;
  if (idx < a.P) {
    const LodRow lr = lod_row_gather<LOD>(a, idx);
    load_mean<LOD>(a, lr, p);
    if (lod && a.shs && (shn & 3) == 0) {
      float* pad = lds_sh + threadIdx.x * sh_row_stride(shn) + shn;
      pad[0] = __uint_as_float((uint32_t)lr.r); pad[1] = __uint_as_float((uint32_t)lr.p); pad[2] = lr.w;
    }
    if constexpr (H48) {
      opac = load_opacity<LOD>(a, idx, nullptr);
      if (a.interpolation_weights && a.num_node_kids && !a.lod_per_pixel)
        opac = lod_opacity(opac, a.interpolation_weights[idx], a.num_node_kids[idx], nullptr);
    }
    if (a.cov3D_precomp) {
#pragma unroll
      for (int i = 0; i < 6; ++i) pr.c3[i] = a.cov3D_precomp[(size_t)idx * 6 + i];
    } else {
      load_scale_rot<LOD>(a, idx, sc_act, q_act, nullptr);
      float R[9], s[3];
      cov3d_from_scale_rot(sc_act, a.scale_modifier, q_act, pr.c3, R, s);
    }
    project_gaussian(p, cam.vm, cam.pm, a.width, a.height, a.tanfovx, a.tanfovy, gx, gy, pr);
  }
  if (idx < a.P && pr.visible) {
    touched = (uint32_t)((pr.maxx - pr.minx) * (pr.maxy - pr.miny));
    k1_band_count(pr, touched, gx, gy, band_cnt);
  }
  {
    const uint32_t ws = wave_sum_u32(touched);
    if ((threadIdx.x & 63) == 0) wave_tot[threadIdx.x >> 6] = ws;
  }
  bool coop = false, deferred = false;
  const bool sh_lds = a.shs && (shn & 3) == 0;
  const int nvis = __syncthreads_count(pr.visible);
  if (threadIdx.x < 64) {
    uint32_t mine = 0;
    if (threadIdx.x == 0) {
#pragma unroll
      for (int w = 0; w < kPreBlock / 64; ++w) mine += wave_tot[w];
      g.block_sums[blockIdx.x] = mine;
    } else if (threadIdx.x <= kBands) {
      mine = band_cnt[threadIdx.x - 1];
      g.block_band[(size_t)(threadIdx.x - 1) * (gridDim.x + 1) + blockIdx.x] = mine;
    }
    if (super && threadIdx.x <= kBands && mine)
      __hip_atomic_fetch_add(&super[threadIdx.x * kMaxSuper + (blockIdx.x / kSuper)], mine, __ATOMIC_RELAXED,
                             __HIP_MEMORY_SCOPE_AGENT);
    if (super && threadIdx.x == 0 && heavy_thr != 0u && mine > heavy_thr) {
      const uint32_t slot = __hip_atomic_fetch_add(&super[kHeavyRow], 1u, __ATOMIC_RELAXED, __HIP_MEMORY_SCOPE_AGENT);
      if (slot < (uint32_t)kMaxHeavy) {
        super[kHeavyRow + 1 + 2 * slot] = blockIdx.x;
        super[kHeavyRow + 2 + 2 * slot] = mine;
      }
    }
  }
  float4 shreg[DEFER ? 12 : 1];
  if (sh_lds) {
    coop = nvis * 2 >= kPreBlock;
    if (coop) {
      if constexpr (H48) {
        sh48_issue_rows(a.shs, blockIdx.x * kPreBlock, a.P, ((a.sh_degree + 1) * (a.sh_degree + 1) * 3 + 3) / 4, lds_sh);
      } else if (lod) {
        coop_gather_sh(a.shs, blockIdx.x * kPreBlock, a.P, shn, lds_sh);
      } else if (a.shs_rest) {
        coop_load_seg(a.shs, blockIdx.x * kPreBlock, a.P, 3, 0, sh_row_stride(shn), lds_sh);
        coop_load_seg(a.shs_rest, blockIdx.x * kPreBlock, a.P, shn - 3, 3, sh_row_stride(shn), lds_sh);
      } else if constexpr (DEFER) {
        coop_issue_sh(a.shs, blockIdx.x * kPreBlock, a.P, shn, shreg);
        deferred = true;
      } else {
        coop_load_sh(a.shs, blockIdx.x * kPreBlock, a.P, shn, lds_sh);
      }
    }
  }
  int32_t rad = 0;
  uint32_t flags = 0;
  K1Rec rec;
  rec.opac = 0.f; rec.thr = 0.f; rec.ext_x = -1.0f; rec.ext_y = -1.0f; rec.invz = 0.f;
  rec.gx_hi = 0.f; rec.gy_hi = 0.f; rec.gx_lo = 0.f; rec.gy_lo = 0.f; rec.A2 = 0.f; rec.B2 = 0.f; rec.C2 = 0.f;
  if (idx < a.P && pr.visible) {
    rad = (int32_t)pr.rad_f;
    if (pr.clampx) flags |= 8u;
    if (pr.clampy) flags |= 16u;
    if constexpr (!H48) {
      opac = load_opacity<LOD>(a, idx, nullptr);
      if (a.interpolation_weights && a.num_node_kids && !a.lod_per_pixel)
        opac = lod_opacity(opac, a.interpolation_weights[idx], a.num_node_kids[idx], nullptr);
    }
    k1_continuous(a, cam, pr, p, sc_act, q_act, opac, rec);
  }
  if constexpr (DEFER) {
    if (deferred) coop_commit_sh(shreg, blockIdx.x * kPreBlock, a.P, shn, lds_sh);
  }
  if constexpr (H48) {
    if (coop) asm volatile("s_waitcnt vmcnt(0)" ::: "memory");
  }
  if (coop) __syncthreads();
  float rgb[3] = {0.f, 0.f, 0.f};
  const bool vis = idx < a.P && pr.visible;
  float J[JAC ? 9 : 1];
  if constexpr (H48) {
    float dx, dy, dz;
    unit_dir(p, cam.cam, dx, dy, dz);
    float Jt[9] = {0.f, 0.f, 0.f, 0.f, 0.f, 0.f, 0.f, 0.f, 0.f};
    if (coop) {
      sh48_row_from_lds<JAC>(lds_sh, (int)threadIdx.x, vis, a.sh_degree, dx, dy, dz, rgb, Jt);
    } else if (vis) {
      sh48_row_from_global<JAC>(a.shs, idx, a.sh_degree, dx, dy, dz, rgb, Jt);
    }
    if constexpr (JAC) {
#pragma unroll
      for (int i = 0; i < 9; ++i) J[i] = Jt[i];
    }
    if (vis) {
      rgb[0] += 0.5f; rgb[1] += 0.5f; rgb[2] += 0.5f;
      if (rgb[0] < 0.f) { rgb[0] = 0.f; flags |= 1u; }
      if (rgb[1] < 0.f) { rgb[1] = 0.f; flags |= 2u; }
      if (rgb[2] < 0.f) { rgb[2] = 0.f; flags |= 4u; }
    }
  } else if (vis) {
    if (a.colors_precomp) {
      rgb[0] = a.colors_precomp[idx * 3 + 0];
      rgb[1] = a.colors_precomp[idx * 3 + 1];
      rgb[2] = a.colors_precomp[idx * 3 + 2];
    } else {
      float sh[48];
      if (coop) lds_row_read(lds_sh, shn, sh);
      else if (lod) load_sh_lod(a, idx, sh);
      else if (a.shs_rest) load_sh_split(a.shs, a.shs_rest, idx, a.M, sh);
      else load_sh(a.shs, idx, a.M, sh);
      float dx, dy, dz;
      unit_dir(p, cam.cam, dx, dy, dz);
      float Jt[9] = {0.f, 0.f, 0.f, 0.f, 0.f, 0.f, 0.f, 0.f, 0.f};
      sh48_accumulate4<JAC, 0>(a.sh_degree, dx, dy, dz, sh, rgb, Jt);
      sh48_accumulate4<JAC, 4>(a.sh_degree, dx, dy, dz, sh + 12, rgb, Jt);
      sh48_accumulate4<JAC, 8>(a.sh_degree, dx, dy, dz, sh + 24, rgb, Jt);
      sh48_accumulate4<JAC, 12>(a.sh_degree, dx, dy, dz, sh + 36, rgb, Jt);
      if constexpr (JAC) {
        float* jd = g.shjac + (size_t)idx * kJacStride;
#pragma unroll
        for (int k = 0; k < 9; ++k) jd[k] = Jt[k];
      }
      float r0 = rgb[0], r1 = rgb[1], r2 = rgb[2];
      r0 += 0.5f; r1 += 0.5f; r2 += 0.5f;
      if (r0 < 0.f) { r0 = 0.f; flags |= 1u; }
      if (r1 < 0.f) { r1 = 0.f; flags |= 2u; }
      if (r2 < 0.f) { r2 = 0.f; flags |= 4u; }
      rgb[0] = r0; rgb[1] = r1; rgb[2] = r2;
    }
  }
  const uint32_t rectbits = (uint32_t)pr.minx | ((uint32_t)pr.miny << 10) | ((uint32_t)(pr.maxx - pr.minx) << 20);
  bool rows_stored = false;
  if constexpr (H48) {
    if (coop) {
      rows_stored = true;
      float4* wl = reinterpret_cast<float4*>(reinterpret_cast<char*>(lds_sh) +
                                             (threadIdx.x >> 6) * (kK1ImageBytes / (kPreBlock / 64)));
      const unsigned long long vmask = __ballot(vis);
      const size_t row0 = (size_t)blockIdx.x * kPreBlock + (threadIdx.x & ~63u);
      const float4 r4[4] = {make_float4(rec.gx_hi, rec.gy_hi, rec.A2, rec.B2), make_float4(rec.C2, rec.opac, rgb[0], rgb[1]),
                            make_float4(rgb[2], rec.invz, rec.ext_x, __uint_as_float(rectbits)),
                            make_float4(rec.gx_lo, rec.gy_lo, rec.thr, rec.ext_y)};
      wave_store_rows<4>(reinterpret_cast<float4*>(g.records), row0, r4, vmask, wl);
      if constexpr (JAC) {
        wave_store_jac(g.shjac, row0, J, vmask, wl);
      }
    }
  }
  if (idx < a.P) {
    if (pr.visible && !rows_stored) {
      float4* recp = reinterpret_cast<float4*>(g.records) + (size_t)idx * kRecVec;
      recp[0] = make_float4(rec.gx_hi, rec.gy_hi, rec.A2, rec.B2);
      recp[1] = make_float4(rec.C2, rec.opac, rgb[0], rgb[1]);
      recp[2] = make_float4(rgb[2], rec.invz, rec.ext_x, __uint_as_float(rectbits));
      recp[3] = make_float4(rec.gx_lo, rec.gy_lo, rec.thr, rec.ext_y);
      if constexpr (H48 && JAC) {
        float* jd = g.shjac + (size_t)idx * kJacStride;
#pragma unroll
        for (int k = 0; k < 9; ++k) jd[k] = J[k];
      }
    }
    reinterpret_cast<uint2*>(g.rects)[idx] =
        pr.visible ? make_uint2((uint32_t)pr.minx | ((uint32_t)pr.miny << 16), (uint32_t)pr.maxx | ((uint32_t)pr.maxy << 16))
                   : make_uint2(0u, 0u);
    radii[idx] = rad;
    g.depths[idx] = pr.tz;
    g.tiles_touched[idx] = touched;
    g.flags[idx] = flags;
  }
}

template <bool JAC, bool LOD, bool DEFER>
__global__ __launch_bounds__(kPreBlock) void preprocess_fwd_kernel(hgs_raster_args a, GeomWs g,
                                                                   int32_t* __restrict__ radii, uint32_t* __restrict__ super, uint32_t heavy_thr) {
  preprocess_fwd_body<JAC, LOD, DEFER, false>(a, g, radii, super, heavy_thr);
}
template <bool JAC>
__global__ __launch_bounds__(kPreBlock, 4) void preprocess_fwd_h48_kernel(hgs_raster_args a, GeomWs g,
                                                                          int32_t* __restrict__ radii,
                                                                          uint32_t* __restrict__ super, uint32_t heavy_thr) {
  preprocess_fwd_body<JAC, false, false, true>(a, g, radii, super, heavy_thr);
}

__global__ __launch_bounds__(1024) void scan_block_sums_kernel(uint32_t* __restrict__ sums0,
                                                               uint32_t* __restrict__ bands, int n,
                                                               unsigned long long* __restrict__ chain,
                                                               uint32_t* __restrict__ total_mirror, int c_off,
                                                               int chunks) {
  uint32_t* __restrict__ sums = blockIdx.y == 0 ? sums0 : bands + (size_t)(blockIdx.y - 1) * (n + 1);
  const uint32_t total = chained_scan_inplace(sums, n, chain + (size_t)blockIdx.y * chunks, c_off, chunks);
  if (threadIdx.x == 0 && blockIdx.y == 0 && (int)blockIdx.x + c_off == chunks - 1 && total_mirror) *total_mirror = total;
}

__device__ __forceinline__ int lod_parent_at(const hgs_raster_args& a, int i) {
  return i < a.lod_n ? a.lod_parent_indices[i] : a.lod_rows - (a.P - a.lod_n) + (i - a.lod_n);
}
struct LodRun {
  bool leader;
  bool atomic;
  int end;
};
__device__ __forceinline__ LodRun lod_run(const hgs_raster_args& a, const int* lds_par, int t, int count, int block_first,
                                          bool nonmono) {
  LodRun r;
  const int p = lds_par[t];
  r.leader = (t == 0) || lds_par[t - 1] != p;
  r.end = t + 1;
  r.atomic = nonmono;
  if (r.leader) {
    while (r.end < count && lds_par[r.end] == p) ++r.end;
    if (t == 0 && block_first > 0 && lod_parent_at(a, block_first - 1) == p) r.atomic = true;
    if (r.end == count && block_first + count < a.P && lod_parent_at(a, block_first + count) == p) r.atomic = true;
  }
  return r;
}
__device__ __forceinline__ void lod_add(float* dst, float v, bool atomic) {
  if (atomic) atomicAdd(dst, v); else *dst = v;
}

__device__ __forceinline__ uint32_t k8_nseg(uint32_t n) {
  uint32_t c = (n + kK8Seg - 1u) / kK8Seg;
  if (c > 1u && n - (c - 1u) * kK8Seg < 2u) --c;
  return c;
}
constexpr int kWorklistGrid = 256;
__global__ __launch_bounds__(kPreBlock) void k8_worklist_kernel(int P, const uint32_t* __restrict__ tiles_touched,
                                                                uint2* __restrict__ work, uint32_t* __restrict__ counter) {
  __shared__ uint32_t wave_tot[kPreBlock / 64];
  __shared__ uint32_t base_s;
  const int lane = threadIdx.x & 63, wave = threadIdx.x >> 6;
  const int nblk = (P + kPreBlock - 1) / kPreBlock;
  const int per = (nblk + (int)gridDim.x - 1) / (int)gridDim.x;
  const int b0 = (int)blockIdx.x * per, b1 = min(b0 + per, nblk);
  uint32_t mine = 0;
  for (int b = b0; b < b1; ++b) {
    const int idx = b * kPreBlock + (int)threadIdx.x;
    const uint32_t n = idx < P ? tiles_touched[idx] : 0u;
    mine += n > kK8LongRun ? k8_nseg(n) : 0u;
  }
#pragma unroll
  for (int off = 32; off > 0; off >>= 1) mine += __shfl_xor(mine, off, 64);
  if (lane == 0) wave_tot[wave] = mine;
  __syncthreads();
  uint32_t total = 0;
#pragma unroll
  for (int w = 0; w < kPreBlock / 64; ++w) total += wave_tot[w];
  if (total == 0u) return;
  if (threadIdx.x == 0) base_s = atomicAdd(counter, total);
  __syncthreads();
  uint32_t run = base_s;
  for (int b = b0; b < b1; ++b) {
    const int idx = b * kPreBlock + (int)threadIdx.x;
    const uint32_t n = idx < P ? tiles_touched[idx] : 0u;
    const uint32_t c = n > kK8LongRun ? k8_nseg(n) : 0u;
    uint32_t inc = c;
#pragma unroll
    for (int off = 1; off < 64; off <<= 1) {
      const uint32_t t = __shfl_up(inc, off, 64);
      if (lane >= off) inc += t;
    }
    __syncthreads();
    if (lane == 63) wave_tot[wave] = inc;
    __syncthreads();
    uint32_t before = 0, tot = 0;
#pragma unroll
    for (int w = 0; w < kPreBlock / 64; ++w) {
      const uint32_t t = wave_tot[w];
      before += w < wave ? t : 0u;
      tot += t;
    }
    uint2* dst = work + run + before + inc - c;
    for (uint32_t j = 0; j < c; ++j) dst[j] = make_uint2((uint32_t)idx, j);
    run += tot;
  }
}

constexpr int kPresumGrid = 2048;
__global__ __launch_bounds__(kPreBlock) void k8_presum_work_kernel(const uint2* __restrict__ work,
                                                                   const uint32_t* __restrict__ counter,
                                                                   const uint32_t* __restrict__ tiles_touched,
                                                                   const uint32_t* __restrict__ offsets,
                                                                   float* __restrict__ inst) {
  __shared__ double red_all[kPreBlock / 64][640 + 40];
  const int lane = threadIdx.x & 63, wave = threadIdx.x >> 6;
  const uint32_t n_work = *counter;
  double* red = red_all[wave];
  for (uint32_t item = blockIdx.x * (kPreBlock / 64) + wave; item < n_work; item += gridDim.x * (kPreBlock / 64)) {
    const uint2 w = work[item];
    const uint32_t n = tiles_touched[w.x];
    const uint32_t r0 = w.y * kK8Seg;
    const uint32_t r1 = (w.y + 1u == k8_nseg(n)) ? n : r0 + kK8Seg;
    const size_t rbase = (size_t)offsets[w.x] + r0;
    const float2* ip = reinterpret_cast<const float2*>(inst) + rbase * 5;
    double t[10];
#pragma unroll
    for (int i = 0; i < 10; ++i) t[i] = 0.0;
#pragma unroll 4
    for (uint32_t k = (uint32_t)lane; k < r1 - r0; k += 64u) {
      const float2 v0 = ip[k * 5 + 0], v1 = ip[k * 5 + 1], v2 = ip[k * 5 + 2], v3 = ip[k * 5 + 3], v4 = ip[k * 5 + 4];
      t[0] += v0.x; t[1] += v0.y; t[2] += v1.x; t[3] += v1.y;
      t[4] += v2.x; t[5] += v2.y; t[6] += v3.x; t[7] += v3.y;
      t[8] += v4.x; t[9] += v4.y;
    }
#pragma unroll
    for (int i = 0; i < 10; ++i) red[i * 64 + lane] = t[i];
    __builtin_amdgcn_fence(__ATOMIC_RELEASE, "wavefront");
    __builtin_amdgcn_wave_barrier();
    __builtin_amdgcn_fence(__ATOMIC_ACQUIRE, "wavefront");
    if (lane < 40) {
      double acc = 0.0;
      const double* src = red + (lane >> 2) * 64 + (lane & 3) * 16;
#pragma unroll
      for (int j = 0; j < 16; ++j) acc += src[j];
      red[640 + lane] = acc;
    }
    __builtin_amdgcn_fence(__ATOMIC_RELEASE, "wavefront");
    __builtin_amdgcn_wave_barrier();
    __builtin_amdgcn_fence(__ATOMIC_ACQUIRE, "wavefront");
    if (lane < 10) {
      const double* q = red + 640 + lane * 4;
      reinterpret_cast<double*>(inst + rbase * kInstStride)[lane] = ((q[0] + q[1]) + q[2]) + q[3];
    }
    __builtin_amdgcn_fence(__ATOMIC_RELEASE, "wavefront");
    __builtin_amdgcn_wave_barrier();
  }
}

constexpr uint32_t kK8StageRec = 256;
__device__ __forceinline__ void k8_sum_runs(const GeomWs& g, const float* __restrict__ inst, int idx, uint32_t n,
                                            int presummed, float2* st, double (&s)[10]) {
  const int lane = threadIdx.x & 63;
  const unsigned long long long_mask = presummed ? __ballot(n > kK8LongRun) : 0ull;
  if (long_mask == 0ull) {
    uint32_t incl = n;
#pragma unroll
    for (int off = 1; off < 64; off <<= 1) {
      const uint32_t t = __shfl_up(incl, off, 64);
      if (lane >= off) incl += t;
    }
    const uint32_t my0 = incl - n, my1 = incl;
    const uint32_t total = __shfl(incl, 63, 64);
    if (total) {
      const unsigned long long nz = __ballot(n != 0u);
      const int first = __ffsll((long long)nz) - 1;
      const uint32_t off_mine = n ? g.offsets[idx] : 0u;
      const size_t base = (size_t)__shfl(off_mine, first, 64);
      for (uint32_t c0 = 0; c0 < total; c0 += kK8StageRec) {
        const uint32_t cn = min(kK8StageRec, total - c0) * 5u;
        const float2* src = reinterpret_cast<const float2*>(inst) + (base + c0) * 5;
        for (uint32_t t0 = 0; t0 < cn; t0 += 64u * 4u) {
          float2 v[4];
#pragma unroll
          for (int j = 0; j < 4; ++j) {
            const uint32_t t = t0 + (uint32_t)j * 64u + (uint32_t)lane;
            v[j] = src[min(t, cn - 1u)];
          }
#pragma unroll
          for (int j = 0; j < 4; ++j) {
            const uint32_t t = t0 + (uint32_t)j * 64u + (uint32_t)lane;
            if (t < cn) st[t] = v[j];
          }
        }
        __builtin_amdgcn_fence(__ATOMIC_RELEASE, "wavefront");
        __builtin_amdgcn_wave_barrier();
        __builtin_amdgcn_fence(__ATOMIC_ACQUIRE, "wavefront");
        const uint32_t k0 = max(my0, c0), k1 = min(my1, c0 + kK8StageRec);
        for (uint32_t k = k0; k < k1; ++k) {
          const float2* r = st + (k - c0) * 5u;
          const float2 v0 = r[0], v1 = r[1], v2 = r[2], v3 = r[3], v4 = r[4];
          s[0] += v0.x; s[1] += v0.y; s[2] += v1.x; s[3] += v1.y;
          s[4] += v2.x; s[5] += v2.y; s[6] += v3.x; s[7] += v3.y;
          s[8] += v4.x; s[9] += v4.y;
        }
        __builtin_amdgcn_fence(__ATOMIC_RELEASE, "wavefront");
        __builtin_amdgcn_wave_barrier();
      }
    }
  } else if (n != 0u) {
    const size_t off = (size_t)g.offsets[idx];
    if (n > kK8LongRun) {
      const uint32_t nseg = k8_nseg(n);
      for (uint32_t j = 0; j < nseg; ++j) {
        const double* ps = reinterpret_cast<const double*>(inst + (off + (size_t)j * kK8Seg) * kInstStride);
#pragma unroll
        for (int i = 0; i < 10; ++i) s[i] += ps[i];
      }
    } else {
      const float2* ip = reinterpret_cast<const float2*>(inst) + off * 5;
#pragma unroll 2
      for (uint32_t k = 0; k < n; ++k) {
        const float2 v0 = ip[k * 5 + 0], v1 = ip[k * 5 + 1], v2 = ip[k * 5 + 2], v3 = ip[k * 5 + 3], v4 = ip[k * 5 + 4];
        s[0] += v0.x; s[1] += v0.y; s[2] += v1.x; s[3] += v1.y;
        s[4] += v2.x; s[5] += v2.y; s[6] += v3.x; s[7] += v3.y;
        s[8] += v4.x; s[9] += v4.y;
      }
    }
  }
}

template <bool LOD>
__device__ __forceinline__ void k8_chain(const hgs_raster_args& a, const GeomWs& g, int idx, const double (&s)[10],
                                         float (&p)[3], float (&d_mean)[3], float (&d_m2)[3], float& d_op,
                                         float (&d_scale)[3], float (&d_rot)[4], float (&d_c3)[6], float (&gr)[3]) {
  CamLds cam;
  load_camera(a, cam);
  gr[0] = (float)s[6]; gr[1] = (float)s[7]; gr[2] = (float)s[8];
  const uint32_t flags = g.flags[idx];
  load_mean<LOD>(a, lod_row_gather<LOD>(a, idx), p);
  float q[4] = {1.f, 0.f, 0.f, 0.f};
  float sc[3] = {1.f, 1.f, 1.f};
  double qnorm = 1.0;
  ProjD pd;
  if (a.cov3D_precomp) {
#pragma unroll
    for (int i = 0; i < 6; ++i) pd.c3[i] = (double)a.cov3D_precomp[(size_t)idx * 6 + i];
  } else {
    load_scale_rot<LOD>(a, idx, sc, q, &qnorm);
    cov3d_from_scale_rot_d(sc, a.scale_modifier, q, pd);
  }
  project_gaussian_d(p, cam.vm, cam.pm, a.width, a.height, a.tanfovx, a.tanfovy, (flags & 8u) != 0,
                     (flags & 16u) != 0, pd);

  const double A = pd.conA, B = pd.conB, C = pd.conC;
  const double gA = -0.5 * s[2], gB = -s[3], gC = -0.5 * s[4];
  const double ggx = -(A * s[0] + B * s[1]);
  const double ggy = -(C * s[1] + B * s[0]);
  const double dm2x = ggx * 0.5 * (double)a.width, dm2y = ggy * 0.5 * (double)a.height;
  d_m2[0] = (float)dm2x;
  d_m2[1] = (float)dm2y;
  double dmean[3] = {0.0, 0.0, 0.0};

  const double dhx = dm2x * pd.pw, dhy = dm2y * pd.pw;
  const double dhw = -(dm2x * pd.hx + dm2y * pd.hy) * pd.pw * pd.pw;
#pragma unroll
  for (int j = 0; j < 3; ++j)
    dmean[j] += (double)cam.pm[j * 4 + 0] * dhx + (double)cam.pm[j * 4 + 1] * dhy + (double)cam.pm[j * 4 + 3] * dhw;

  const double a2 = pd.a, b2 = pd.b, c2 = pd.c;
  const double di2 = pd.di * pd.di;
  const double ga = (-c2 * c2 * gA + b2 * c2 * gB - b2 * b2 * gC) * di2;
  const double gb = (2.0 * b2 * c2 * gA - (a2 * c2 + b2 * b2) * gB + 2.0 * a2 * b2 * gC) * di2;
  const double gc = (-b2 * b2 * gA + a2 * b2 * gB - a2 * a2 * gC) * di2;
  const double hb = 0.5 * gb;
  double Gs[3][3];
#pragma unroll
  for (int i = 0; i < 3; ++i)
#pragma unroll
    for (int j = i; j < 3; ++j)
      Gs[i][j] = Gs[j][i] = pd.T0[i] * (ga * pd.T0[j] + hb * pd.T1[j]) + pd.T1[i] * (hb * pd.T0[j] + gc * pd.T1[j]);
  d_c3[0] = (float)Gs[0][0];
  d_c3[1] = (float)(2.0 * Gs[0][1]);
  d_c3[2] = (float)(2.0 * Gs[0][2]);
  d_c3[3] = (float)Gs[1][1];
  d_c3[4] = (float)(2.0 * Gs[1][2]);
  d_c3[5] = (float)Gs[2][2];
  double dT0[3], dT1[3];
#pragma unroll
  for (int j = 0; j < 3; ++j) {
    dT0[j] = 2.0 * ga * pd.U0[j] + gb * pd.U1[j];
    dT1[j] = gb * pd.U0[j] + 2.0 * gc * pd.U1[j];
  }
  double gJ00 = 0.0, gJ02 = 0.0, gJ11 = 0.0, gJ12 = 0.0;
#pragma unroll
  for (int j = 0; j < 3; ++j) {
    gJ00 += dT0[j] * (double)cam.vm[j * 4 + 0];
    gJ02 += dT0[j] * (double)cam.vm[j * 4 + 2];
    gJ11 += dT1[j] * (double)cam.vm[j * 4 + 1];
    gJ12 += dT1[j] * (double)cam.vm[j * 4 + 2];
  }
  const double itz = pd.itz, itz2 = itz * itz, itz3 = itz2 * itz;
  const double g_txc = -pd.fx * itz2 * gJ02;
  const double g_tyc = -pd.fy * itz2 * gJ12;
  double g_tz = -pd.fx * itz2 * gJ00 + 2.0 * pd.fx * pd.txc * itz3 * gJ02 - pd.fy * itz2 * gJ11 +
                2.0 * pd.fy * pd.tyc * itz3 * gJ12;
  double g_tx = 0.0, g_ty = 0.0;
  if (flags & 8u) g_tz += g_txc * (pd.txc * itz); else g_tx = g_txc;
  if (flags & 16u) g_tz += g_tyc * (pd.tyc * itz); else g_ty = g_tyc;
  g_tz += -s[9] * itz2;
#pragma unroll
  for (int j = 0; j < 3; ++j)
    dmean[j] += (double)cam.vm[j * 4 + 0] * g_tx + (double)cam.vm[j * 4 + 1] * g_ty + (double)cam.vm[j * 4 + 2] * g_tz;
  d_mean[0] = (float)dmean[0]; d_mean[1] = (float)dmean[1]; d_mean[2] = (float)dmean[2];

  if (!a.cov3D_precomp) {
    const double* R = pd.R;
    const double* sv = pd.s;
    double dM[3][3];
#pragma unroll
    for (int i = 0; i < 3; ++i)
#pragma unroll
      for (int k = 0; k < 3; ++k) {
        double acc = 0.0;
#pragma unroll
        for (int j = 0; j < 3; ++j) acc += Gs[i][j] * (R[j * 3 + k] * sv[k]);
        dM[i][k] = 2.0 * acc;
      }
    double gR[3][3];
#pragma unroll
    for (int k = 0; k < 3; ++k) {
      double acc = 0.0;
#pragma unroll
      for (int i = 0; i < 3; ++i) {
        acc += R[i * 3 + k] * dM[i][k];
        gR[i][k] = dM[i][k] * sv[k];
      }
      double dsk = (double)a.scale_modifier * acc;
      if (a.activations & HGS_ACT_SCALE_EXP) dsk *= (double)sc[k];
      d_scale[k] = (float)dsk;
    }
    const double r = q[0], x = q[1], y = q[2], z = q[3];
    double dq[4];
    dq[0] = 2.0 * (-z * gR[0][1] + y * gR[0][2] + z * gR[1][0] - x * gR[1][2] - y * gR[2][0] + x * gR[2][1]);
    dq[1] = 2.0 * (y * gR[0][1] + z * gR[0][2] + y * gR[1][0] - 2.0 * x * gR[1][1] - r * gR[1][2] +
                   z * gR[2][0] + r * gR[2][1] - 2.0 * x * gR[2][2]);
    dq[2] = 2.0 * (-2.0 * y * gR[0][0] + x * gR[0][1] + r * gR[0][2] + x * gR[1][0] + z * gR[1][2] -
                   r * gR[2][0] + z * gR[2][1] - 2.0 * y * gR[2][2]);
    dq[3] = 2.0 * (-2.0 * z * gR[0][0] - r * gR[0][1] + x * gR[0][2] + r * gR[1][0] - 2.0 * z * gR[1][1] +
                   y * gR[1][2] + x * gR[2][0] + y * gR[2][1]);
    if (a.activations & HGS_ACT_ROT_NORMALIZE) {
      const double dot = r * dq[0] + x * dq[1] + y * dq[2] + z * dq[3];
      const double inv = 1.0 / qnorm;
      dq[0] = (dq[0] - r * dot) * inv; dq[1] = (dq[1] - x * dot) * inv;
      dq[2] = (dq[2] - y * dot) * inv; dq[3] = (dq[3] - z * dot) * inv;
    }
    d_rot[0] = (float)dq[0]; d_rot[1] = (float)dq[1]; d_rot[2] = (float)dq[2]; d_rot[3] = (float)dq[3];
  }

  {
    float dod = 1.0f;
    double dact = 1.0;
    const float o_act = load_opacity<LOD>(a, idx, &dact);
    float o_rec = o_act;
    if (a.interpolation_weights && a.num_node_kids && !a.lod_per_pixel)
      o_rec = lod_opacity(o_act, a.interpolation_weights[idx], a.num_node_kids[idx], &dod);
    const float sums5 = o_rec > 0.0f ? (float)(s[5] / (double)o_rec) : 0.0f;
    d_op = a.activations ? (float)((double)sums5 * (double)dod * dact) : sums5 * dod;
  }

  if (!a.colors_precomp) {
    if (flags & 1u) gr[0] = 0.f;
    if (flags & 2u) gr[1] = 0.f;
    if (flags & 4u) gr[2] = 0.f;
  }
}

template <bool ACC>
__device__ __forceinline__ void k8_store_row(const hgs_raster_grads& out, int idx, const float (&d_m2)[3], float d_op,
                                             const float (&d_scale)[3], const float (&d_rot)[4], const float (&d_c3)[6],
                                             const float (&d_col)[3]) {
  constexpr bool acc = ACC;
#pragma unroll
  for (int j = 0; j < 3; ++j) out.dL_dmeans2D[idx * 3 + j] = d_m2[j];
  out.dL_dopacity[idx] = d_op + (acc ? out.dL_dopacity[idx] : 0.f);
  if (out.dL_dcolors) {
#pragma unroll
    for (int j = 0; j < 3; ++j) out.dL_dcolors[idx * 3 + j] = d_col[j];
  }
  if (out.dL_dscales) {
#pragma unroll
    for (int j = 0; j < 3; ++j) out.dL_dscales[idx * 3 + j] = d_scale[j] + (acc ? out.dL_dscales[idx * 3 + j] : 0.f);
  }
  if (out.dL_drotations) {
    float4* dst = reinterpret_cast<float4*>(out.dL_drotations) + idx;
    float4 v = make_float4(d_rot[0], d_rot[1], d_rot[2], d_rot[3]);
    if (acc) { const float4 o = *dst; v.x += o.x; v.y += o.y; v.z += o.z; v.w += o.w; }
    *dst = v;
  }
  if (out.dL_dcov3D) {
#pragma unroll
    for (int j = 0; j < 6; ++j) out.dL_dcov3D[(size_t)idx * 6 + j] = d_c3[j] + (acc ? out.dL_dcov3D[(size_t)idx * 6 + j] : 0.f);
  }
}

template <bool ACC, bool LOD>
__global__ __launch_bounds__(kPreBlock) void preprocess_bwd_kernel(hgs_raster_args a, GeomWs g,
                                                                   const float* __restrict__ inst,
                                                                   float* __restrict__ drgb,
                                                                   float* __restrict__ dmean_rows,
                                                                   const uint32_t* __restrict__ lod_flag,
                                                                   hgs_raster_grads out, int presummed) {
  const int idx = blockIdx.x * kPreBlock + threadIdx.x;
  const bool in_range = idx < a.P;
  const uint32_t n = in_range ? g.tiles_touched[idx] : 0u;

  double s[10];
#pragma unroll
  for (int i = 0; i < 10; ++i) s[i] = 0.0;
  static_assert(kInstStride == 10, "instance record = the ten sums, 40 bytes");
  __shared__ float2 stage[kPreBlock / 64][kK8StageRec * 5];
  k8_sum_runs(g, inst, idx, n, presummed, stage[threadIdx.x >> 6], s);
  if constexpr (!LOD) {
    if (!in_range) return;
  }

  float d_mean[3] = {0.f, 0.f, 0.f};
  float d_m2[3] = {0.f, 0.f, 0.f};
  float d_op = 0.f;
  float d_scale[3] = {0.f, 0.f, 0.f};
  float d_rot[4] = {0.f, 0.f, 0.f, 0.f};
  float d_c3[6] = {0.f, 0.f, 0.f, 0.f, 0.f, 0.f};
  float gr[3] = {0.f, 0.f, 0.f};
  float d_col[3] = {0.f, 0.f, 0.f};
  if (n != 0) {
    float p[3];
    k8_chain<LOD>(a, g, idx, s, p, d_mean, d_m2, d_op, d_scale, d_rot, d_c3, gr);
    if (a.colors_precomp) {
      d_col[0] = gr[0]; d_col[1] = gr[1]; d_col[2] = gr[2];
    } else {
      drgb[idx * 3 + 0] = gr[0];
      drgb[idx * 3 + 1] = gr[1];
      drgb[idx * 3 + 2] = gr[2];
    }
  }

  if constexpr (LOD) {
    if (a.lod_scatter) {
      __shared__ float lds_v[8 * kPreBlock];
      __shared__ int lds_par[kPreBlock];
      __shared__ unsigned char lds_vis[kPreBlock];
      const int t = threadIdx.x;
      const int block_first = blockIdx.x * kPreBlock;
      const int count = min(kPreBlock, a.P - block_first);
      LodRow l;
      l.r = l.p = 0; l.w = 1.0f; l.u = 0.0f;
      if (in_range) l = lod_row<true>(a, idx);
      const bool self = l.p == l.r;
      const bool vis = in_range && n != 0;
      const float wn = self ? 1.0f : l.w, u = (self || !vis) ? 0.0f : l.u;
      float sgn = 1.0f;
      if (vis && !self && u != 0.0f) {
        const float4 qa = reinterpret_cast<const float4*>(a.rotations)[l.r];
        const float4 qb = reinterpret_cast<const float4*>(a.rotations)[l.p];
        sgn = (qa.x * qb.x + qa.y * qb.y + qa.z * qb.z + qa.w * qb.w) < 0.0f ? -1.0f : 1.0f;
      }
      if (in_range) {
#pragma unroll
        for (int j = 0; j < 3; ++j) {
          dmean_rows[idx * 3 + j] = d_mean[j];
          out.dL_dmeans2D[idx * 3 + j] = d_m2[j];
        }
      }
      if (vis) {
        out.dL_dopacity[l.r] = wn * d_op;
#pragma unroll
        for (int j = 0; j < 3; ++j) out.dL_dscales[l.r * 3 + j] = wn * d_scale[j];
        reinterpret_cast<float4*>(out.dL_drotations)[l.r] = make_float4(wn * d_rot[0], wn * d_rot[1], wn * d_rot[2], wn * d_rot[3]);
      }
      lds_par[t] = in_range ? (int)l.p : -1;
      lds_vis[t] = (vis && !self) ? 1 : 0;
#pragma unroll
      for (int j = 0; j < 3; ++j) lds_v[j * kPreBlock + t] = u * d_scale[j];
#pragma unroll
      for (int j = 0; j < 4; ++j) lds_v[(3 + j) * kPreBlock + t] = (u * sgn) * d_rot[j];
      lds_v[7 * kPreBlock + t] = u * d_op;
      __syncthreads();
      if (t < count) {
        const LodRun run = lod_run(a, lds_par, t, count, block_first, *lod_flag != 0u);
        if (run.leader) {
          float acc8[8] = {0.f, 0.f, 0.f, 0.f, 0.f, 0.f, 0.f, 0.f};
          bool any = false;
          for (int j = t; j < run.end; ++j) {
            if (!lds_vis[j]) continue;
            any = true;
#pragma unroll
            for (int k = 0; k < 8; ++k) acc8[k] += lds_v[k * kPreBlock + j];
          }
          if (any) {
            const size_t pp = (size_t)lds_par[t];
#pragma unroll
            for (int k = 0; k < 3; ++k) lod_add(out.dL_dscales + pp * 3 + k, acc8[k], run.atomic);
#pragma unroll
            for (int k = 0; k < 4; ++k) lod_add(out.dL_drotations + pp * 4 + k, acc8[3 + k], run.atomic);
            lod_add(out.dL_dopacity + pp, acc8[7], run.atomic);
          }
        }
      }
      return;
    }
    if (!in_range) return;
  }
#pragma unroll
  for (int j = 0; j < 3; ++j) out.dL_dmeans3D[idx * 3 + j] = d_mean[j] + (ACC ? out.dL_dmeans3D[idx * 3 + j] : 0.f);
  k8_store_row<ACC>(out, idx, d_m2, d_op, d_scale, d_rot, d_c3, d_col);
}


template <bool ACC, bool JAC, bool LOD>
__global__ __launch_bounds__(kPreBlock) void sh_bwd_kernel(hgs_raster_args a, GeomWs g,
                                                           const float* __restrict__ drgb,
                                                           const float* __restrict__ dmean_rows,
                                                           const uint32_t* __restrict__ lod_flag, hgs_raster_grads out) {
  extern __shared__ __attribute__((aligned(16))) unsigned char smem_raw[];
  float* lds = reinterpret_cast<float*>(smem_raw);
  const int n = a.M * 3;
  const bool split = a.shs_rest != nullptr;
  const bool coop = (n & 3) == 0;
// ... 43 lines not shown
      gdz = gr[0] * J[6] + gr[1] * J[7] + gr[2] * J[8];
#pragma unroll
      for (int k = 0; k < 16; ++k) {
        if (k < nb) { dsh[k * 3 + 0] = b[k] * gr[0]; dsh[k * 3 + 1] = b[k] * gr[1]; dsh[k * 3 + 2] = b[k] * gr[2]; }
      }
    } else {
      float dbx[16], dby[16], dbz[16];
      sh_basis_grad(a.sh_degree, ux, uy, uz, dbx, dby, dbz);
#pragma unroll
      for (int k = 0; k < 16; ++k) {
        if (k < nb) {
          dsh[k * 3 + 0] = b[k] * gr[0]; dsh[k * 3 + 1] = b[k] * gr[1]; dsh[k * 3 + 2] = b[k] * gr[2];
          const float dotc = gr[0] * sh[k * 3 + 0] + gr[1] * sh[k * 3 + 1] + gr[2] * sh[k * 3 + 2];
          gdx += dbx[k] * dotc; gdy += dby[k] * dotc; gdz += dbz[k] * dotc;
        }
      }
    }
    const float dot = ux * gdx + uy * gdy + uz * gdz;
    vdir[0] = (gdx - ux * dot) * inv; vdir[1] = (gdy - uy * dot) * inv; vdir[2] = (gdz - uz * dot) * inv;
    if (!(LOD && a.lod_scatter)) {
      out.dL_dmeans3D[idx * 3 + 0] += vdir[0];
      out.dL_dmeans3D[idx * 3 + 1] += vdir[1];
      out.dL_dmeans3D[idx * 3 + 2] += vdir[2];
    }
  }
  if constexpr (LOD) {
    if (a.lod_scatter) {
      __shared__ float lds_m[3 * kPreBlock];
      __shared__ int lds_par[kPreBlock];
      const int t = threadIdx.x;
      const int count = min(kPreBlock, a.P - block_first);
      const int stride = sh_row_stride(n), cpr = n >> 2;
      LodRow l;
      l.r = l.p = 0; l.w = 1.0f; l.u = 0.0f;
      if (valid) l = lod_row<true>(a, idx);
      if (valid) {
        lds_row_write(lds, n, dsh);
        float* pad = lds + t * stride + n;
        pad[0] = __uint_as_float((uint32_t)l.r); pad[1] = __uint_as_float((uint32_t)l.p); pad[2] = l.w;
        pad[3] = __uint_as_float(active ? 1u : 0u);
#pragma unroll
        for (int j = 0; j < 3; ++j) lds_m[j * kPreBlock + t] = active ? dmean_rows[idx * 3 + j] + vdir[j] : 0.0f;
      }
      lds_par[t] = valid ? (int)l.p : -1;
      __syncthreads();
      const bool nonmono = *lod_flag != 0u;
      float4* dsh_full = reinterpret_cast<float4*>(out.dL_dshs);
      for (int v = t; v < count * cpr; v += kPreBlock) {
        const int row = v / cpr, c = v - row * cpr;
        const float* rp = lds + row * stride;
        const uint32_t r = __float_as_uint(rp[n]), pr = __float_as_uint(rp[n + 1]);
        const bool self = r == pr;
        if (__float_as_uint(rp[n + 3])) {
          const float wn = self ? 1.0f : rp[n + 2];
          const float4 g4 = *reinterpret_cast<const float4*>(rp + c * 4);
          dsh_full[(size_t)r * cpr + c] = make_float4(wn * g4.x, wn * g4.y, wn * g4.z, wn * g4.w);
        }
        const LodRun run = lod_run(a, lds_par, row, count, block_first, nonmono);
        if (run.leader) {
          float4 acc = make_float4(0.f, 0.f, 0.f, 0.f);
          bool any = false;
          for (int j = row; j < run.end; ++j) {
            const float* rj = lds + j * stride;
            if (!__float_as_uint(rj[n + 3]) || __float_as_uint(rj[n]) == __float_as_uint(rj[n + 1])) continue;
            any = true;
            const float uj = 1.0f - rj[n + 2];
            const float4 g4 = *reinterpret_cast<const float4*>(rj + c * 4);
            acc.x += uj * g4.x; acc.y += uj * g4.y; acc.z += uj * g4.z; acc.w += uj * g4.w;
          }
          if (any) {
            float* dst = reinterpret_cast<float*>(dsh_full + (size_t)pr * cpr + c);
            if (run.atomic) {
              atomicAdd(dst + 0, acc.x); atomicAdd(dst + 1, acc.y); atomicAdd(dst + 2, acc.z); atomicAdd(dst + 3, acc.w);
            } else {
              *reinterpret_cast<float4*>(dst) = acc;
            }
          }
        }
      }
      if (t < count) {
        const float* rp = lds + t * stride;
        const uint32_t r = __float_as_uint(rp[n]), pr = __float_as_uint(rp[n + 1]);
        const bool self = r == pr;
        if (__float_as_uint(rp[n + 3])) {
          const float wn = self ? 1.0f : rp[n + 2];
#pragma unroll
          for (int j = 0; j < 3; ++j) out.dL_dmeans3D[(size_t)r * 3 + j] = wn * lds_m[j * kPreBlock + t];
        }
        const LodRun run = lod_run(a, lds_par, t, count, block_first, nonmono);
        if (run.leader) {
          float acc3[3] = {0.f, 0.f, 0.f};
          bool any = false;
          for (int j = t; j < run.end; ++j) {
            const float* rj = lds + j * stride;
            if (!__float_as_uint(rj[n + 3]) || __float_as_uint(rj[n]) == __float_as_uint(rj[n + 1])) continue;
            any = true;
            const float uj = 1.0f - rj[n + 2];
#pragma unroll
            for (int k = 0; k < 3; ++k) acc3[k] += uj * lds_m[k * kPreBlock + j];
          }
          if (any) {
#pragma unroll
            for (int k = 0; k < 3; ++k) lod_add(out.dL_dmeans3D + (size_t)pr * 3 + k, acc3[k], run.atomic);
          }
        }
      }
      return;
    }
  }
  if (coop) {
    if (valid) lds_row_write(lds, n, dsh);
    __syncthreads();
    if (split) {
      coop_store_seg<ACC>(out.dL_dshs, block_first, a.P, 3, 0, sh_row_stride(n), lds);
      coop_store_seg<ACC>(out.dL_dshs_rest, block_first, a.P, n - 3, 3, sh_row_stride(n), lds);
    } else {
      coop_store_sh<ACC>(out.dL_dshs, block_first, a.P, n, lds);
    }
  } else if (valid && split) {
    float* d0 = out.dL_dshs + (size_t)idx * 3;
    float* d1 = out.dL_dshs_rest + (size_t)idx * (n - 3);
#pragma unroll
    for (int i = 0; i < 48; ++i) {
      if (i < 3) d0[i] = dsh[i] + (ACC ? d0[i] : 0.f);
      else if (i < n) d1[i - 3] = dsh[i] + (ACC ? d1[i - 3] : 0.f);
    }
  } else if (valid) {
    if (ACC) {
      const float* old = out.dL_dshs + (size_t)idx * n;
#pragma unroll
      for (int i = 0; i < 48; ++i)
        if (i < n) dsh[i] += old[i];
    }
    store_sh(out.dL_dshs, idx, a.M, dsh);
  }
}

__device__ __forceinline__ float k8_dot3(float x0, float y0, float x1, float y1, float x2, float y2) {
#pragma clang fp contract(off)
  return __fmaf_rn(x2, y2, __fmaf_rn(x0, y0, x1 * y1));
}
__device__ __forceinline__ void k8_add_view_term(const float (&gr)[3], const float (&J)[9], float ux, float uy, float uz,
                                                 float inv, float (&d_mean)[3]) {
#pragma clang fp contract(off)
  const float gdx = k8_dot3(gr[0], J[0], gr[1], J[1], gr[2], J[2]);
  const float gdy = k8_dot3(gr[0], J[3], gr[1], J[4], gr[2], J[5]);
  const float gdz = k8_dot3(gr[0], J[6], gr[1], J[7], gr[2], J[8]);
  const float dot = k8_dot3(ux, gdx, uy, gdy, uz, gdz);
  d_mean[0] = __fmaf_rn(__fmaf_rn(-ux, dot, gdx), inv, d_mean[0] + 0.f);
  d_mean[1] = __fmaf_rn(__fmaf_rn(-uy, dot, gdy), inv, d_mean[1] + 0.f);
  d_mean[2] = __fmaf_rn(__fmaf_rn(-uz, dot, gdz), inv, d_mean[2] + 0.f);
}

__global__ __launch_bounds__(kPreBlock) void preprocess_bwd_sh_kernel(hgs_raster_args a, GeomWs g,
                                                                         const float* __restrict__ inst,
                                                                         hgs_raster_grads out, int presummed) {
  extern __shared__ __attribute__((aligned(16))) unsigned char smem_raw[];
  const int block_first = blockIdx.x * kPreBlock;
  const int idx = block_first + threadIdx.x;
  const bool in_range = idx < a.P;
  const uint32_t n = in_range ? g.tiles_touched[idx] : 0u;

  double s[10];
#pragma unroll
  for (int i = 0; i < 10; ++i) s[i] = 0.0;
  k8_sum_runs(g, inst, idx, n, presummed, reinterpret_cast<float2*>(smem_raw) + (threadIdx.x >> 6) * (kK8StageRec * 5), s);

  float d_mean[3] = {0.f, 0.f, 0.f};
  float d_m2[3] = {0.f, 0.f, 0.f};
  float d_op = 0.f;
  float d_scale[3] = {0.f, 0.f, 0.f};
  float d_rot[4] = {0.f, 0.f, 0.f, 0.f};
  float d_c3[6] = {0.f, 0.f, 0.f, 0.f, 0.f, 0.f};
  float gr[3] = {0.f, 0.f, 0.f};
  float b[16];
  const int nb = (a.sh_degree + 1) * (a.sh_degree + 1);
  float p[3];
  if (n != 0) k8_chain<false>(a, g, idx, s, p, d_mean, d_m2, d_op, d_scale, d_rot, d_c3, gr);
  if (in_range) {
    const float d_col[3] = {0.f, 0.f, 0.f};
    k8_store_row<false>(out, idx, d_m2, d_op, d_scale, d_rot, d_c3, d_col);
  }
  __builtin_amdgcn_sched_barrier(0);
  if (n != 0) {
    float ux, uy, uz;
    const float inv = unit_dir(p, a.campos, ux, uy, uz);
    sh_basis(a.sh_degree, ux, uy, uz, b);
    const float* jp = g.shjac + (size_t)idx * kJacStride;
    float J[9];
#pragma unroll
    for (int k = 0; k < 9; ++k) J[k] = jp[k];
    k8_add_view_term(gr, J, ux, uy, uz, inv, d_mean);
  } else {
#pragma unroll
    for (int j = 0; j < 3; ++j) d_mean[j] = 0.f;
  }
  if (in_range) {
#pragma unroll
    for (int j = 0; j < 3; ++j) out.dL_dmeans3D[idx * 3 + j] = d_mean[j];
  }

  float* lds = reinterpret_cast<float*>(smem_raw);
  const int nc = a.M * 3, stride = sh_row_stride(nc);
  __syncthreads();
  if (in_range) {
    float* row = lds + threadIdx.x * stride;
#pragma unroll
    for (int i = 0; i < 12; ++i) {
      if (i * 4 < nc) {
        float v[4];
#pragma unroll
        for (int c = 0; c < 4; ++c) {
          const int k = (i * 4 + c) / 3, ch = (i * 4 + c) % 3;
          v[c] = (n != 0 && k < nb) ? b[k] * gr[ch] : 0.f;
        }
        *reinterpret_cast<float4*>(row + i * 4) = make_float4(v[0], v[1], v[2], v[3]);
      }
    }
  }
  __syncthreads();
  coop_store_sh<false>(out.dL_dshs, block_first, a.P, nc, lds);
}

template <bool ACC, bool COOP, bool COLOR>
__device__ __forceinline__ void sh_bwd_batched_body(const ShBwdViews& v, int P, int M, int sh_degree,
                                                    const float* __restrict__ means3D, const float* __restrict__ shs,
                                                    float* __restrict__ dL_dshs, float* __restrict__ dL_dmeans3D) {
  extern __shared__ __attribute__((aligned(16))) unsigned char smem_raw[];
  float* lds = reinterpret_cast<float*>(smem_raw);
  const int n = M * 3;
  constexpr bool coop = COOP;
  const int block_first = blockIdx.x * kPreBlock;
  const int idx = block_first + threadIdx.x;
  const bool valid = idx < P;
  if (coop) {
    coop_load_sh(shs, block_first, P, n, lds);
    __syncthreads();
  }
  float sh_reg[COOP ? 1 : 48];
  if constexpr (!COOP) { if (valid) load_sh(shs, idx, M, sh_reg); }
  float dsh[48];
#pragma unroll
  for (int i = 0; i < 48; ++i) dsh[i] = 0.f;
  float gm0 = 0.f, gm1 = 0.f, gm2 = 0.f;
  if (valid) {
    const float px = means3D[idx * 3 + 0], py = means3D[idx * 3 + 1], pz = means3D[idx * 3 + 2];
    const int nb = (sh_degree + 1) * (sh_degree + 1);
    for (int w = 0; w < v.n; ++w) {
      if (!COLOR && static_cast<const uint32_t*>(v.mask[w])[idx] == 0) continue;
      float gr0 = v.drgb[w][idx * 3 + 0], gr1 = v.drgb[w][idx * 3 + 1], gr2 = v.drgb[w][idx * 3 + 2];
      if (COLOR) {
        const uint32_t m = static_cast<const uint8_t*>(v.mask[w])[idx];
        if (m & 1u) gr0 = 0.f;
        if (m & 2u) gr1 = 0.f;
        if (m & 4u) gr2 = 0.f;
        if (gr0 == 0.f && gr1 == 0.f && gr2 == 0.f) continue;
      }
      float dotc[16];
#pragma unroll
      for (int k = 0; k < 16; ++k) dotc[k] = 0.f;
      if constexpr (COOP) {
        const float4* row4 = reinterpret_cast<const float4*>(lds + threadIdx.x * sh_row_stride(n));
#pragma unroll
        for (int i = 0; i < 12; ++i) {
          if (i * 4 < n) {
            const float4 t = row4[i];
            const float tv[4] = {t.x, t.y, t.z, t.w};
#pragma unroll
            for (int c = 0; c < 4; ++c) {
              const int ch = (i * 4 + c) % 3;
              dotc[(i * 4 + c) / 3] += (ch == 0 ? gr0 : ch == 1 ? gr1 : gr2) * tv[c];
            }
          }
        }
      } else {
#pragma unroll
        for (int i = 0; i < 48; ++i) dotc[i / 3] += (i % 3 == 0 ? gr0 : i % 3 == 1 ? gr1 : gr2) * sh_reg[i];
      }
      const float pxyz[3] = {px, py, pz};
      float ux, uy, uz;
      const float inv = unit_dir(pxyz, v.campos[w], ux, uy, uz);
      {
        float b[16];
        sh_basis(sh_degree, ux, uy, uz, b);
#pragma unroll
        for (int k = 0; k < 16; ++k) {
          if (k < nb) { dsh[k * 3 + 0] += b[k] * gr0; dsh[k * 3 + 1] += b[k] * gr1; dsh[k * 3 + 2] += b[k] * gr2; }
        }
      }
      float gdx = 0.f, gdy = 0.f, gdz = 0.f;
      {
        float dbx[16], dby[16], dbz[16];
        sh_basis_grad(sh_degree, ux, uy, uz, dbx, dby, dbz);
#pragma unroll
        for (int k = 0; k < 16; ++k) {
          if (k < nb) { gdx += dbx[k] * dotc[k]; gdy += dby[k] * dotc[k]; gdz += dbz[k] * dotc[k]; }
        }
      }
      const float dot = ux * gdx + uy * gdy + uz * gdz;
      gm0 += (gdx - ux * dot) * inv;
      gm1 += (gdy - uy * dot) * inv;
      gm2 += (gdz - uz * dot) * inv;
    }
    dL_dmeans3D[idx * 3 + 0] += gm0;
    dL_dmeans3D[idx * 3 + 1] += gm1;
    dL_dmeans3D[idx * 3 + 2] += gm2;
  }
  if (coop) {
    __syncthreads();
    if (valid) lds_row_write(lds, n, dsh);
    __syncthreads();
    coop_store_sh<ACC>(dL_dshs, block_first, P, n, lds);
  } else if (valid) {
    if (ACC) {
      const float* old = dL_dshs + (size_t)idx * n;
#pragma unroll
      for (int i = 0; i < 48; ++i)
        if (i < n) dsh[i] += old[i];
    }
    store_sh(dL_dshs, idx, M, dsh);
  }
}

}

template <bool ACC, bool COOP>
__global__ __launch_bounds__(kPreBlock) void sh_bwd_batched_kernel(ShBwdViews v, int P, int M, int sh_degree,
                                                                   const float* __restrict__ means3D,
                                                                   const float* __restrict__ shs,
                                                                   float* __restrict__ dL_dshs,
                                                                   float* __restrict__ dL_dmeans3D) {
  sh_bwd_batched_body<ACC, COOP, false>(v, P, M, sh_degree, means3D, shs, dL_dshs, dL_dmeans3D);
}
template <bool ACC, bool COOP>
__global__ __launch_bounds__(kPreBlock, 3) void sh_bwd_batched_color_kernel(ShBwdViews v, int P, int M, int sh_degree,
                                                                            const float* __restrict__ means3D,
                                                                            const float* __restrict__ shs,
                                                                            float* __restrict__ dL_dshs,
                                                                            float* __restrict__ dL_dmeans3D) {
  sh_bwd_batched_body<ACC, COOP, true>(v, P, M, sh_degree, means3D, shs, dL_dshs, dL_dmeans3D);
}

__global__ __launch_bounds__(kPreBlock) void sh_colors_batched_kernel(ShFwdViews v, int P, int M, int sh_degree,
                                                                      const float* __restrict__ means3D,
                                                                      const float* __restrict__ shs) {
  extern __shared__ __attribute__((aligned(16))) unsigned char smem_raw[];
  float* lds = reinterpret_cast<float*>(smem_raw);
  const int n = M * 3;
  const bool coop = (n & 3) == 0;
  const int block_first = blockIdx.x * kPreBlock;
  const int idx = block_first + threadIdx.x;
  if (coop) {
    coop_load_sh(shs, block_first, P, n, lds);
    __syncthreads();
  }
  if (idx >= P) return;
  float sh[48];
  if (coop) lds_row_read(lds, n, sh); else load_sh(shs, idx, M, sh);
  const float px = means3D[idx * 3 + 0], py = means3D[idx * 3 + 1], pz = means3D[idx * 3 + 2];
  const int nb = (sh_degree + 1) * (sh_degree + 1);
  for (int w = 0; w < v.n; ++w) {
    const float pxyz[3] = {px, py, pz};
    float dx, dy, dz;
    unit_dir(pxyz, v.campos[w], dx, dy, dz);
    float b[16];
    sh_basis(sh_degree, dx, dy, dz, b);
    float r0 = 0.f, r1 = 0.f, r2 = 0.f;
#pragma unroll
    for (int k = 0; k < 16; ++k) {
      if (k < nb) {
        r0 += b[k] * sh[k * 3 + 0];
        r1 += b[k] * sh[k * 3 + 1];
        r2 += b[k] * sh[k * 3 + 2];
      }
    }
    r0 += 0.5f; r1 += 0.5f; r2 += 0.5f;
    uint32_t m = 0;
    if (r0 < 0.f) { r0 = 0.f; m |= 1u; }
    if (r1 < 0.f) { r1 = 0.f; m |= 2u; }
    if (r2 < 0.f) { r2 = 0.f; m |= 4u; }
    v.rgb_out[w][idx * 3 + 0] = r0;
    v.rgb_out[w][idx * 3 + 1] = r1;
    v.rgb_out[w][idx * 3 + 2] = r2;
    v.clamp_out[w][idx] = (uint8_t)m;
  }
}

int launch_sh_colors_batched(const ShFwdViews& v, int32_t P, int32_t M, int32_t sh_degree, const float* means3D,
                             const float* shs, hipStream_t s) {
  const int nblk = (P + kPreBlock - 1) / kPreBlock;
  if (nblk <= 0) return HGS_OK;
  const size_t lds_bytes = (size_t)kPreBlock * (M * 3 + 4) * sizeof(float);
  hipLaunchKernelGGL(sh_colors_batched_kernel, dim3(nblk), dim3(kPreBlock), lds_bytes, s, v, P, M, sh_degree, means3D, shs);
  HGS_LAUNCH_CHECK("sh_colors_batched", s, false);
  return HGS_OK;
}

int launch_sh_bwd_batched(const ShBwdViews& v, int32_t P, int32_t M, int32_t sh_degree, const float* means3D,
                          const float* shs, float* dL_dshs, float* dL_dmeans3D, bool accumulate, hipStream_t s) {
  const int nblk = (P + kPreBlock - 1) / kPreBlock;
  if (nblk <= 0) return HGS_OK;
  const size_t lds_bytes = (size_t)kPreBlock * (M * 3 + 4) * sizeof(float);
  const bool coop = ((M * 3) & 3) == 0;
  const bool color = v.color != 0;
  auto kern = color ? (coop ? (accumulate ? sh_bwd_batched_color_kernel<true, true> : sh_bwd_batched_color_kernel<false, true>)
                            : (accumulate ? sh_bwd_batched_color_kernel<true, false> : sh_bwd_batched_color_kernel<false, false>))
                    : (coop ? (accumulate ? sh_bwd_batched_kernel<true, true> : sh_bwd_batched_kernel<false, true>)
                            : (accumulate ? sh_bwd_batched_kernel<true, false> : sh_bwd_batched_kernel<false, false>));
  hipLaunchKernelGGL(kern, dim3(nblk), dim3(kPreBlock), lds_bytes, s, v, P, M, sh_degree, means3D, shs, dL_dshs,
                     dL_dmeans3D);
  HGS_LAUNCH_CHECK("sh_bwd_batched", s, false);
  return HGS_OK;
}

namespace {
constexpr int kMaxSyncBlocks = 64;
struct SyncBlock { int device; hipStream_t stream; uint32_t* words; bool dirty; };
std::mutex g_sync_mu;
SyncBlock g_sync[kMaxSyncBlocks];
int g_sync_n = 0;
}
size_t super_block_bytes() { return (size_t)(2 + kBands) * kMaxSuper * sizeof(uint32_t); }
uint32_t* super_block_acquire(hipStream_t s) {
  static const bool off = getenv("HGS_SCAN_LAUNCH") != nullptr;
  if (off) return nullptr;
  if (s == hipStreamPerThread) return nullptr;
  hipStreamCaptureStatus cap = hipStreamCaptureStatusNone;
  if (hipStreamIsCapturing(s, &cap) != hipSuccess) { (void)hipGetLastError(); return nullptr; }
  if (cap != hipStreamCaptureStatusNone) return nullptr;
  int dev = 0;
  if (hipGetDevice(&dev) != hipSuccess) { (void)hipGetLastError(); return nullptr; }
  std::lock_guard<std::mutex> lk(g_sync_mu);
  for (int i = 0; i < g_sync_n; ++i) {
    SyncBlock& b = g_sync[i];
    if (b.device != dev || b.stream != s) continue;
    if (b.dirty) {
      if (hipMemsetAsync(b.words, 0, super_block_bytes(), s) != hipSuccess) { (void)hipGetLastError(); return nullptr; }
      b.dirty = false;
    }
    return b.words;
  }
  if (g_sync_n == kMaxSyncBlocks) return nullptr;
  uint32_t* w = nullptr;
  if (hipMalloc(reinterpret_cast<void**>(&w), super_block_bytes()) != hipSuccess) { (void)hipGetLastError(); return nullptr; }
  if (hipMemsetAsync(w, 0, super_block_bytes(), s) != hipSuccess) { (void)hipGetLastError(); (void)hipFree(w); return nullptr; }
  g_sync[g_sync_n++] = {dev, s, w, false};
  return w;
}
int super_block_release(int device) {
  std::lock_guard<std::mutex> lk(g_sync_mu);
  int kept = 0, freed = 0;
  for (int i = 0; i < g_sync_n; ++i) {
    if (device < 0 || g_sync[i].device == device) {
      int cur = 0;
      const bool sw = hipGetDevice(&cur) == hipSuccess && cur != g_sync[i].device && hipSetDevice(g_sync[i].device) == hipSuccess;
      (void)hipFree(g_sync[i].words);
      if (sw) (void)hipSetDevice(cur);
      ++freed;
    } else {
      g_sync[kept++] = g_sync[i];
    }
  }
  g_sync_n = kept;
  return freed;
}
void super_block_mark_dirty(const uint32_t* words) {
  std::lock_guard<std::mutex> lk(g_sync_mu);
  for (int i = 0; i < g_sync_n; ++i)
    if (g_sync[i].words == words) g_sync[i].dirty = true;
}

int launch_preprocess_fwd(const hgs_raster_args& a, const GeomWs& g, int32_t* radii, hipStream_t s, uint32_t* super,
                          uint32_t heavy_thr) {
  const int nblk = (a.P + kPreBlock - 1) / kPreBlock;
  if (nblk > 0) {
    const bool jac = a.prepare_backward && a.shs;
    const bool plain = a.shs && !a.shs_rest && !a.lod_render_indices && ((a.M * 3) & 3) == 0;
    const bool h48 = plain && a.M == 16;
    const bool defer = plain && !h48;
    const size_t lds_bytes = !a.shs ? 0 : h48 ? (size_t)kK1ImageBytes : (size_t)kPreBlock * (a.M * 3 + 4) * sizeof(float);
    auto k1 = a.lod_render_indices ? (jac ? preprocess_fwd_kernel<true, true, false> : preprocess_fwd_kernel<false, true, false>)
              : h48   ? (jac ? preprocess_fwd_h48_kernel<true> : preprocess_fwd_h48_kernel<false>)
              : defer ? (jac ? preprocess_fwd_kernel<true, false, true> : preprocess_fwd_kernel<false, false, true>)
                      : (jac ? preprocess_fwd_kernel<true, false, false> : preprocess_fwd_kernel<false, false, false>);
    hipLaunchKernelGGL(k1, dim3(nblk), dim3(kPreBlock), lds_bytes, s, a, g, radii, super, heavy_thr);
    HGS_LAUNCH_CHECK("preprocess_fwd", s, a.debug);
  }
  return HGS_OK;
}

int launch_scan_block_sums(const GeomWs& g, int32_t P, hipStream_t s, bool debug, uint32_t* total_mirror) {
  const int nblk = (P + kPreBlock - 1) / kPreBlock;
  const int chunks = scan_chunks(nblk), resident = scan_resident_workgroups();
  if (chunks * (1 + kBands) <= resident && !scan_split_forced()) {
    hipLaunchKernelGGL(scan_block_sums_kernel, dim3(chunks, 1 + kBands), dim3(1024), 0, s, g.block_sums, g.block_band,
                       nblk, g.scan_chain, total_mirror, 0, chunks);
    HGS_LAUNCH_CHECK("scan_block_sums", s, debug);
    return HGS_OK;
  }
  for (int y = 0; y < 1 + kBands; ++y) {
    uint32_t* sums = y == 0 ? g.block_sums : g.block_band + (size_t)(y - 1) * (nblk + 1);
    for (int c0 = 0; c0 < chunks; c0 += resident) {
      hipLaunchKernelGGL(scan_block_sums_kernel, dim3(min(resident, chunks - c0), 1), dim3(1024), 0, s, sums, g.block_band,
                         nblk, g.scan_chain + (size_t)y * chunks, y == 0 ? total_mirror : nullptr, c0, chunks);
      HGS_LAUNCH_CHECK("scan_block_sums", s, debug);
    }
  }
  return HGS_OK;
}

int launch_preprocess_bwd(const hgs_raster_args& a, const GeomWs& g, const float* inst_grads, float* drgb,
                          float* dmean_rows, const uint32_t* lod_flag, const hgs_raster_grads& out, uint32_t L,
                          uint2* work, uint32_t* work_counter, hipStream_t s) {
  const int nblk = (a.P + kPreBlock - 1) / kPreBlock;
  if (nblk > 0) {
    static const char* force = getenv("HGS_K8_PRESUM");
    const bool presum = force ? force[0] == '1' : (uint64_t)L > 6ull * (uint64_t)a.P;
    if (presum) {
      HGS_HIP(hipMemsetAsync(work_counter, 0, sizeof(uint32_t), s));
      hipLaunchKernelGGL(k8_worklist_kernel, dim3(nblk < kWorklistGrid ? nblk : kWorklistGrid), dim3(kPreBlock), 0, s, a.P,
                         g.tiles_touched, work, work_counter);
      HGS_LAUNCH_CHECK("preprocess_bwd_worklist", s, a.debug);
      const int want = (int)(((size_t)L / 64 + 3) / 4);
      hipLaunchKernelGGL(k8_presum_work_kernel, dim3(want < 1 ? 1 : (want < kPresumGrid ? want : kPresumGrid)), dim3(kPreBlock), 0,
                         s, work, work_counter, g.tiles_touched, g.offsets, const_cast<float*>(inst_grads));
      HGS_LAUNCH_CHECK("preprocess_bwd_long_runs", s, a.debug);
    }
    const char* fuse_env = getenv("HGS_K8_FUSE");
    const bool fused = !(fuse_env && fuse_env[0] == '0') && !a.lod_render_indices && !a.accumulate_grads &&
                       !a.defer_sh_bwd && a.shs && !a.shs_rest && out.dL_dshs && a.prepare_backward && !a.colors_precomp &&
                       ((a.M * 3) & 3) == 0;
    if (fused) {
      const size_t stage_bytes = (size_t)(kPreBlock / 64) * kK8StageRec * 5 * sizeof(float2);
      const size_t rows_bytes = (size_t)kPreBlock * (a.M * 3 + 4) * sizeof(float);
      hipLaunchKernelGGL(preprocess_bwd_sh_kernel, dim3(nblk), dim3(kPreBlock),
                         stage_bytes > rows_bytes ? stage_bytes : rows_bytes, s, a, g, inst_grads, out, presum ? 1 : 0);
      HGS_LAUNCH_CHECK("preprocess_bwd_sh", s, a.debug);
      return HGS_OK;
    }
    auto k8a = a.lod_render_indices ? preprocess_bwd_kernel<false, true>
                                    : (a.accumulate_grads ? preprocess_bwd_kernel<true, false> : preprocess_bwd_kernel<false, false>);
    hipLaunchKernelGGL(k8a, dim3(nblk), dim3(kPreBlock), 0, s, a, g, inst_grads, drgb, dmean_rows, lod_flag, out,
                       presum ? 1 : 0);
    HGS_LAUNCH_CHECK("preprocess_bwd", s, a.debug);
    if (a.shs && out.dL_dshs && !a.defer_sh_bwd) {
      const size_t lds_bytes = (size_t)kPreBlock * (a.M * 3 + 4) * sizeof(float);
      auto k8b = a.lod_render_indices ? sh_bwd_kernel<false, true, true>
                 : (a.prepare_backward && a.shs) ? (a.accumulate_grads ? sh_bwd_kernel<true, true, false> : sh_bwd_kernel<false, true, false>)
                                                 : (a.accumulate_grads ? sh_bwd_kernel<true, false, false> : sh_bwd_kernel<false, false, false>);
      hipLaunchKernelGGL(k8b, dim3(nblk), dim3(kPreBlock), lds_bytes, s, a, g, drgb, dmean_rows, lod_flag, out);
      HGS_LAUNCH_CHECK("sh_bwd", s, a.debug);
    }
  }
  return HGS_OK;
}

}
```

Before: 1521.

## Hoist per-Gaussian loads early in preprocess kernels, gated by per-stream route history

Adds an early-load path to the H48 forward preprocess kernel and the fused backward SH kernel. Each Gaussian's mean, opacity, scale/rotation, Jacobian and camera data are issued up front, ahead of the SH row DMA and the run summation, to overlap memory latency. A host-side table stores, per thread/stream and per workspace, how many blocks took the non-cooperative route on the last frame, copied back through an extra pinned word, and uses it to decide whether to speculate or load unconditionally. This costs extra registers and LDS, plus wasted loads for culled Gaussians, and adds history-dependent control that is on by default.

```diff
diff --git a/hierarchical-3d-gaussians_amd/csrc/abi.cpp b/hierarchical-3d-gaussians_amd/csrc/abi.cpp
--- a/hierarchical-3d-gaussians_amd/csrc/abi.cpp
+++ b/hierarchical-3d-gaussians_amd/csrc/abi.cpp
@@ -1,4 +1,5 @@
 #include "common.h"
+#include "early_loads.h"
 
 #include <pthread.h>
 #include <sched.h>
@@ -47,6 +48,9 @@
 #define HGS_TIMED(stage, stream, expr) [&]() { hgs::StageTimer _t(stage, stream); return (expr); }()
 
 static thread_local char g_err[512] = "";
+
+static EarlyTable g_early;
+static uintptr_t this_thread() { return (uintptr_t)pthread_self(); }
 
 constexpr int kMaxDevices = 16;
 struct ThreadHost {
@@ -70,7 +74,7 @@
   ThreadHost* h = static_cast<ThreadHost*>(pthread_getspecific(g_host_key));
   if (!h) {
     h = new ThreadHost();
-    if (hipHostMalloc(reinterpret_cast<void**>(&h->pinned_L), sizeof(uint32_t), hipHostMallocPortable | hipHostMallocMapped) != hipSuccess) {
+    if (hipHostMalloc(reinterpret_cast<void**>(&h->pinned_L), 2 * sizeof(uint32_t), hipHostMallocPortable | hipHostMallocMapped) != hipSuccess) {
       thread_host_free(h);
       return nullptr;
     }
@@ -274,7 +278,11 @@
   const GeomWs g = GeomWs::carve_from(geom_ws, a->P);
   *L_out_host = 0;
   if (a->P == 0) return HGS_OK;
-  if ((rc = HGS_TIMED(ST_PREPROCESS_FWD, s, launch_preprocess_fwd(*a, g, radii, s)))) return rc;
+  const EarlyMode early = early_mode(getenv("HGS_EARLY_LOADS"));
+  const bool spec = preprocess_fwd_is_h48(*a) &&
+                    (early == kEarlyForce || (early == kEarlyAuto && g_early.speculate(this_thread(), device, s, a->P)));
+  g_early.record(this_thread(), device, s, geom_ws, a->P, 0, 0, false);
+  if ((rc = HGS_TIMED(ST_PREPROCESS_FWD, s, launch_preprocess_fwd(*a, g, radii, s, nullptr, 0u, spec)))) return rc;
   if ((rc = HGS_TIMED(ST_SCAN, s, launch_scan_block_sums(g, a->P, s, a->debug)))) return rc;
   const int nblk = (a->P + kPreBlock - 1) / kPreBlock;
   HGS_HIP(hipMemcpyAsync(L_out_host, g.block_sums + nblk, sizeof(uint32_t), hipMemcpyDeviceToHost, s));
@@ -290,7 +298,10 @@
   const bool bin = L > 0 && tile_bin_supported(T);
   if ((rc = HGS_TIMED(ST_DUPLICATE, s, launch_duplicate_tiles(*a, g, b, L, bin, s, super, mirror)))) return rc;
   if (super) {
-    if (!mirror) HGS_HIP(hipMemcpyAsync(stage, L_dev, sizeof(uint32_t), hipMemcpyDeviceToHost, s));
+    if (!mirror) {
+      HGS_HIP(hipMemcpyAsync(stage, L_dev, sizeof(uint32_t), hipMemcpyDeviceToHost, s));
+      HGS_HIP(hipMemcpyAsync(stage + 1, super + kNoCoopWord, sizeof(uint32_t), hipMemcpyDeviceToHost, s));
+    }
     HGS_HIP(hipEventRecord(ev, s));
   }
   if (bin) {
@@ -348,7 +359,11 @@
   const int nblk = (a->P + kPreBlock - 1) / kPreBlock;
   uint32_t* super = nullptr;
   if (L_cap > 0 && tile_bin_supported(T) && nblk <= kSuper * kMaxSuper) super = super_block_acquire(s);
-  if ((rc = HGS_TIMED(ST_PREPROCESS_FWD, s, launch_preprocess_fwd(*a, g, radii, s, super, super ? k3_heavy_threshold(L_cap, a->P) : 0u)))) {
+  const EarlyMode early = early_mode(getenv("HGS_EARLY_LOADS"));
+  const bool h48 = preprocess_fwd_is_h48(*a);
+  const bool spec = h48 && (early == kEarlyForce || (early == kEarlyAuto && g_early.speculate(this_thread(), device, s, a->P)));
+  g_early.record(this_thread(), device, s, geom_ws, a->P, 0, 0, false);
+  if ((rc = HGS_TIMED(ST_PREPROCESS_FWD, s, launch_preprocess_fwd(*a, g, radii, s, super, super ? k3_heavy_threshold(L_cap, a->P) : 0u, spec)))) {
     if (super) super_block_mark_dirty(super);
     return rc;
   }
@@ -369,6 +384,7 @@
   if (e != hipSuccess) { set_error("hgs_raster_fwd: %s", hipGetErrorString(e)); return HGS_ERR_HIP; }
   *L_out_host = *stage;
   if (rc) return rc;
+  if (super && h48) g_early.record(this_thread(), device, s, geom_ws, a->P, (uint32_t)nblk, stage[1], true);
   if (*L_out_host > L_cap) {
     if (super) {
       HGS_HIP(hipMemsetAsync(g.scan_chain, 0, (size_t)(1 + kBands) * scan_chunks(nblk) * sizeof(unsigned long long), s));
@@ -380,7 +396,10 @@
   return HGS_OK;
 }
 
-int hgs_release_device_state(int device) { return super_block_release(device); }
+int hgs_release_device_state(int device) {
+  g_early.forget_device(device);
+  return super_block_release(device);
+}
 
 int hgs_raster_bwd(const hgs_raster_args* a, const void* geom_ws, const void* bin_ws, const void* img_ws,
                    void* bwd_ws, uint32_t L, const float* out_color, const float* out_invdepth,
@@ -423,8 +442,11 @@
     HGS_HIP(hipMemsetAsync(lod_flag, 0, sizeof(uint32_t), s));
     if ((rc = launch_lod_monotone(a->lod_parent_indices, a->lod_n, lod_flag, s))) return rc;
   }
+  const EarlyMode early = early_mode(getenv("HGS_EARLY_LOADS"));
+  const int k8_early = early == kEarlyOff ? 0 : (early == kEarlyForce || g_early.unconditional(device, geom_ws, a->P)) ? 2 : 1;
   return HGS_TIMED(ST_PREPROCESS_BWD, s, launch_preprocess_bwd(*a, g, inst, drgb, bwd_ws_dmean(bwd_ws, L, a->P), lod_flag, gr, L,
-                                                             bwd_ws_work(bwd_ws, L, a->P), bwd_ws_work_counter(bwd_ws, L, a->P), s));
+                                                             bwd_ws_work(bwd_ws, L, a->P), bwd_ws_work_counter(bwd_ws, L, a->P), s,
+                                                             k8_early));
 }
 
 int hgs_raster_sh_bwd_batched(const hgs_sh_bwd_view* views, int32_t n_views, int32_t P, int32_t M, int32_t sh_degree,
diff --git a/hierarchical-3d-gaussians_amd/csrc/binning.hip b/hierarchical-3d-gaussians_amd/csrc/binning.hip
--- a/hierarchical-3d-gaussians_amd/csrc/binning.hip
+++ b/hierarchical-3d-gaussians_amd/csrc/binning.hip
@@ -125,6 +125,7 @@
   uint32_t block_base = 0;
   uint32_t band_tot = 0, band_off = 0;
   heavy_n = 0u;
+  uint32_t no_coop = 0u;
   if (!super) {
     block_base = g.block_sums[blk];
     if (tid < kBands) {
@@ -144,6 +145,7 @@
       x0[u] = super[a * kMaxSuper + min(lane, nsb - 1)];
     }
     if constexpr (OWN) heavy_n = super[kHeavyRow];
+    if constexpr (OWN) no_coop = super[kNoCoopWord];
 #pragma unroll
     for (int u = 0; u < kPer; ++u) {
       const int a = min(wave + u * kWaves, kBands);
@@ -216,7 +218,7 @@
     if (OWN && blk == nblk - 1 && tid <= kBands) {
       uint32_t* arr = tid == 0 ? g.block_sums : g.block_band + (size_t)(tid - 1) * col;
       arr[nblk] = l.tot9[tid];
-      if (tid == 0 && total_mirror) *total_mirror = l.tot9[0];
+      if (tid == 0 && total_mirror) { total_mirror[0] = l.tot9[0]; total_mirror[1] = no_coop; }
     }
   }
   uint32_t wbase = 0;
diff --git a/hierarchical-3d-gaussians_amd/csrc/common.h b/hierarchical-3d-gaussians_amd/csrc/common.h
--- a/hierarchical-3d-gaussians_amd/csrc/common.h
+++ b/hierarchical-3d-gaussians_amd/csrc/common.h
@@ -161,12 +161,14 @@
 bool scan_split_forced();
 
 int launch_preprocess_fwd(const hgs_raster_args& a, const GeomWs& g, int32_t* radii, hipStream_t s,
-                          uint32_t* super = nullptr, uint32_t heavy_thr = 0);
+                          uint32_t* super = nullptr, uint32_t heavy_thr = 0, bool speculate = false);
+bool preprocess_fwd_is_h48(const hgs_raster_args& a);
 constexpr int kSuper = 64;
 constexpr int kMaxSuper = 1024;
 constexpr int kMaxHeavy = 256;
 constexpr int kHeavyRow = (1 + kBands) * kMaxSuper;
-static_assert(1 + 2 * kMaxHeavy <= kMaxSuper, "the heavy list fits the row");
+constexpr int kNoCoopWord = kHeavyRow + 1 + 2 * kMaxHeavy;
+static_assert(2 + 2 * kMaxHeavy <= kMaxSuper, "the heavy list and K1's route counter fit the row");
 uint32_t k3_heavy_threshold(uint32_t L_cap, int32_t P);
 uint32_t* super_block_acquire(hipStream_t s);
 size_t super_block_bytes();
@@ -188,7 +190,7 @@
                       const float* dL_dinvdepth, float* inst_grads, hipStream_t s);
 int launch_preprocess_bwd(const hgs_raster_args& a, const GeomWs& g, const float* inst_grads, float* drgb,
                           float* dmean_rows, const uint32_t* lod_flag, const hgs_raster_grads& out, uint32_t L,
-                          uint2* work, uint32_t* work_counter, hipStream_t s);
+                          uint2* work, uint32_t* work_counter, hipStream_t s, int k8_early = 0);
 int launch_lod_monotone(const int32_t* parent_indices, int32_t n, uint32_t* flag, hipStream_t s);
 struct ShBwdViews {
   const void* mask[HGS_MAX_DEFERRED_VIEWS];
diff --git a/hierarchical-3d-gaussians_amd/csrc/early_loads.h b/hierarchical-3d-gaussians_amd/csrc/early_loads.h
--- /dev/null
+++ b/hierarchical-3d-gaussians_amd/csrc/early_loads.h
@@ -0,0 +1,83 @@
+#pragma once
+
+#include <stdint.h>
+#include <string.h>
+
+#include <mutex>
+
+namespace hgs {
+
+enum EarlyMode { kEarlyOff = 0, kEarlyAuto = 1, kEarlyForce = 2 };
+inline EarlyMode early_mode(const char* env) {
+  if (!env) return kEarlyAuto;
+  if (env[0] == '0') return kEarlyOff;
+  return strcmp(env, "force") == 0 ? kEarlyForce : kEarlyAuto;
+}
+
+constexpr uint32_t kEarlyDenom = 16;
+inline bool early_count_low(uint32_t off_route, uint32_t nblk) {
+  return (uint64_t)off_route * kEarlyDenom < (uint64_t)nblk;
+}
+
+class EarlyTable {
+ public:
+  static constexpr int kEntries = 16;
+
+  void record(uintptr_t thread, int device, const void* stream, const void* geom_ws, int32_t P, uint32_t nblk,
+              uint32_t off_route, bool known) {
+    std::lock_guard<std::mutex> lk(mu_);
+    int slot = -1;
+    for (int i = 0; i < kEntries; ++i) {
+      Entry& e = e_[i];
+      if (e.valid && e.device == device &&
+          ((e.thread == thread && e.stream == stream) || e.geom_ws == geom_ws)) e.valid = false;
+      if (!e.valid && slot < 0) slot = i;
+    }
+    if (!known) return;
+    if (slot < 0) {
+      slot = 0;
+      for (int i = 1; i < kEntries; ++i)
+        if (e_[i].tick < e_[slot].tick) slot = i;
+    }
+    e_[slot] = {true, thread, device, stream, geom_ws, P, nblk, off_route, ++tick_};
+  }
+
+  bool speculate(uintptr_t thread, int device, const void* stream, int32_t P) {
+    std::lock_guard<std::mutex> lk(mu_);
+    for (const Entry& e : e_)
+      if (e.valid && e.thread == thread && e.device == device && e.stream == stream)
+        return e.P == P && early_count_low(e.off_route, e.nblk);
+    return false;
+  }
+
+  bool unconditional(int device, const void* geom_ws, int32_t P) {
+    std::lock_guard<std::mutex> lk(mu_);
+    for (const Entry& e : e_)
+      if (e.valid && e.device == device && e.geom_ws == geom_ws)
+        return e.P == P && early_count_low(e.off_route, e.nblk);
+    return false;
+  }
+
+  void forget_device(int device) {
+    std::lock_guard<std::mutex> lk(mu_);
+    for (Entry& e : e_)
+      if (device < 0 || e.device == device) e.valid = false;
+  }
+
+ private:
+  struct Entry {
+    bool valid;
+    uintptr_t thread;
+    int device;
+    const void* stream;
+    const void* geom_ws;
+    int32_t P;
+    uint32_t nblk, off_route;
+    unsigned long long tick;
+  };
+  std::mutex mu_;
+  Entry e_[kEntries] = {};
+  unsigned long long tick_ = 0;
+};
+
+}
diff --git a/hierarchical-3d-gaussians_amd/csrc/gaussian_math.h b/hierarchical-3d-gaussians_amd/csrc/gaussian_math.h
--- a/hierarchical-3d-gaussians_amd/csrc/gaussian_math.h
+++ b/hierarchical-3d-gaussians_amd/csrc/gaussian_math.h
@@ -260,6 +260,22 @@
   }
 }
 
+__device__ __forceinline__ void activate_scale(const hgs_raster_args& a, float sc[3]) {
+  if (a.activations & HGS_ACT_SCALE_EXP) {
+#pragma unroll
+    for (int i = 0; i < 3; ++i) sc[i] = (float)exp((double)sc[i]);
+  }
+}
+__device__ __forceinline__ void activate_rot(const hgs_raster_args& a, float q[4], double* nrm) {
+  double n = 1.0;
+  if (a.activations & HGS_ACT_ROT_NORMALIZE) {
+    const double w = q[0], x = q[1], y = q[2], z = q[3];
+    n = fmax(sqrt(((w * w + x * x) + y * y) + z * z), 1e-12);
+    q[0] = (float)(w / n); q[1] = (float)(x / n); q[2] = (float)(y / n); q[3] = (float)(z / n);
+  }
+  if (nrm) *nrm = n;
+}
+
 template <bool LOD>
 __device__ __forceinline__ void load_scale_rot(const hgs_raster_args& a, int idx, float sc[3], float q[4],
                                                double* nrm) {
@@ -276,19 +292,24 @@
     return;
   }
   sc[0] = a.scales[idx * 3 + 0]; sc[1] = a.scales[idx * 3 + 1]; sc[2] = a.scales[idx * 3 + 2];
-  if (a.activations & HGS_ACT_SCALE_EXP) {
-#pragma unroll
-    for (int i = 0; i < 3; ++i) sc[i] = (float)exp((double)sc[i]);
-  }
+  activate_scale(a, sc);
   const float4 qv = reinterpret_cast<const float4*>(a.rotations)[idx];
   q[0] = qv.x; q[1] = qv.y; q[2] = qv.z; q[3] = qv.w;
-  double n = 1.0;
-  if (a.activations & HGS_ACT_ROT_NORMALIZE) {
-    const double w = q[0], x = q[1], y = q[2], z = q[3];
-    n = fmax(sqrt(((w * w + x * x) + y * y) + z * z), 1e-12);
-    q[0] = (float)(w / n); q[1] = (float)(x / n); q[2] = (float)(y / n); q[3] = (float)(z / n);
-  }
-  if (nrm) *nrm = n;
+  activate_rot(a, q, nrm);
+}
+
+__device__ __forceinline__ float activate_opacity(const hgs_raster_args& a, float raw, double* dact) {
+  if (a.activations & HGS_ACT_OPACITY_SIGMOID) {
+    const double o = 1.0 / (1.0 + exp(-(double)raw));
+    if (dact) *dact = o * (1.0 - o);
+    return (float)o;
+  }
+  if (a.activations & HGS_ACT_OPACITY_ABS) {
+    if (dact) *dact = raw > 0.f ? 1.0 : (raw < 0.f ? -1.0 : 0.0);
+    return fabsf(raw);
+  }
+  if (dact) *dact = 1.0;
+  return raw;
 }
 
 template <bool LOD>
@@ -298,18 +319,7 @@
     if (dact) *dact = 1.0;
     return lod_lerp(a.opacities[l.r], a.opacities[l.p], l.w, l.u);
   }
-  const float raw = a.opacities[idx];
-  if (a.activations & HGS_ACT_OPACITY_SIGMOID) {
-    const double o = 1.0 / (1.0 + exp(-(double)raw));
-    if (dact) *dact = o * (1.0 - o);
-    return (float)o;
-  }
-  if (a.activations & HGS_ACT_OPACITY_ABS) {
-    if (dact) *dact = raw > 0.f ? 1.0 : (raw < 0.f ? -1.0 : 0.0);
-    return fabsf(raw);
-  }
-  if (dact) *dact = 1.0;
-  return raw;
+  return activate_opacity(a, a.opacities[idx], dact);
 }
 
 __device__ __forceinline__ float lod_opacity(float o, float w, int kids, float* dout_do) {
diff --git a/hierarchical-3d-gaussians_amd/csrc/preprocess.hip b/hierarchical-3d-gaussians_amd/csrc/preprocess.hip
--- a/hierarchical-3d-gaussians_amd/csrc/preprocess.hip
+++ b/hierarchical-3d-gaussians_amd/csrc/preprocess.hip
@@ -453,7 +453,8 @@
 
 template <bool JAC, bool LOD, bool DEFER, bool H48>
 __device__ __forceinline__ void preprocess_fwd_body(const hgs_raster_args& a, const GeomWs& g,
-                                                    int32_t* __restrict__ radii, uint32_t* __restrict__ super, uint32_t heavy_thr) {
+                                                    int32_t* __restrict__ radii, uint32_t* __restrict__ super, uint32_t heavy_thr,
+                                                    int speculate) {
   static_assert(!(H48 && (LOD || DEFER)), "the DMA route is the plain layout's");
   extern __shared__ __attribute__((aligned(16))) unsigned char smem_raw[];
   float* lds_sh = reinterpret_cast<float*>(smem_raw);
@@ -477,17 +478,46 @@
   float opac = 0.f;
   constexpr bool lod = LOD;
   const int shn = a.M * 3;
-  if (idx < a.P) {
+  const bool spec = H48 && speculate != 0 && a.shs;
+  if constexpr (H48) {
+    const size_t li = (size_t)min(idx, a.P - 1);
+    const bool lodop = a.interpolation_weights && a.num_node_kids && !a.lod_per_pixel;
+    p[0] = a.means3D[li * 3 + 0]; p[1] = a.means3D[li * 3 + 1]; p[2] = a.means3D[li * 3 + 2];
+    opac = a.opacities[li];
+    float lod_w = 0.f;
+    int lod_k = 0;
+    if (lodop) { lod_w = a.interpolation_weights[li]; lod_k = a.num_node_kids[li]; }
+    const bool cov = a.cov3D_precomp != nullptr;
+    const float* in_a = cov ? a.cov3D_precomp + li * 6 : a.scales + li * 3;
+    const float* in_b = cov ? a.cov3D_precomp + li * 6 + 3 : a.rotations + li * 4;
+    const float in7[7] = {in_a[0], in_a[1], in_a[2], in_b[0], in_b[1], in_b[2], in_b[cov ? 2 : 3]};
+    asm volatile("" ::: "memory");
+    if (spec)
+      sh48_issue_rows(a.shs, blockIdx.x * kPreBlock, a.P, ((a.sh_degree + 1) * (a.sh_degree + 1) * 3 + 3) / 4, lds_sh);
+    if (cov) {
+#pragma unroll
+      for (int i = 0; i < 6; ++i) pr.c3[i] = in7[i];
+    } else {
+      sc_act[0] = in7[0]; sc_act[1] = in7[1]; sc_act[2] = in7[2];
+      q_act[0] = in7[3]; q_act[1] = in7[4]; q_act[2] = in7[5]; q_act[3] = in7[6];
+    }
+    if (idx < a.P) {
+      opac = activate_opacity(a, opac, nullptr);
+      if (lodop) opac = lod_opacity(opac, lod_w, lod_k, nullptr);
+      if (!a.cov3D_precomp) {
+        activate_scale(a, sc_act);
+        activate_rot(a, q_act, nullptr);
+        float R[9], s[3];
+        cov3d_from_scale_rot(sc_act, a.scale_modifier, q_act, pr.c3, R, s);
+      }
+      project_gaussian(p, cam.vm, cam.pm, a.width, a.height, a.tanfovx, a.tanfovy, gx, gy, pr);
+    }
+  } else if (idx < a.P) {
     const LodRow lr = lod_row_gather<LOD>(a, idx);
     load_mean<LOD>(a, lr, p);
     if (lod && a.shs && (shn & 3) == 0) {
       float* pad = lds_sh + threadIdx.x * sh_row_stride(shn) + shn;
       pad[0] = __uint_as_float((uint32_t)lr.r); pad[1] = __uint_as_float((uint32_t)lr.p); pad[2] = lr.w;
-    }
-    if constexpr (H48) {
-      opac = load_opacity<LOD>(a, idx, nullptr);
-      if (a.interpolation_weights && a.num_node_kids && !a.lod_per_pixel)
-        opac = lod_opacity(opac, a.interpolation_weights[idx], a.num_node_kids[idx], nullptr);
     }
     if (a.cov3D_precomp) {
 #pragma unroll
@@ -534,9 +564,14 @@
   float4 shreg[DEFER ? 12 : 1];
   if (sh_lds) {
     coop = nvis * 2 >= kPreBlock;
+    if constexpr (H48) {
+      if (super && !coop && threadIdx.x == 0)
+        __hip_atomic_fetch_add(&super[kNoCoopWord], 1u, __ATOMIC_RELAXED, __HIP_MEMORY_SCOPE_AGENT);
+    }
     if (coop) {
       if constexpr (H48) {
-        sh48_issue_rows(a.shs, blockIdx.x * kPreBlock, a.P, ((a.sh_degree + 1) * (a.sh_degree + 1) * 3 + 3) / 4, lds_sh);
+        if (!spec)
+          sh48_issue_rows(a.shs, blockIdx.x * kPreBlock, a.P, ((a.sh_degree + 1) * (a.sh_degree + 1) * 3 + 3) / 4, lds_sh);
       } else if (lod) {
         coop_gather_sh(a.shs, blockIdx.x * kPreBlock, a.P, shn, lds_sh);
       } else if (a.shs_rest) {
@@ -570,9 +605,9 @@
     if (deferred) coop_commit_sh(shreg, blockIdx.x * kPreBlock, a.P, shn, lds_sh);
   }
   if constexpr (H48) {
-    if (coop) asm volatile("s_waitcnt vmcnt(0)" ::: "memory");
-  }
-  if (coop) __syncthreads();
+    if (coop || spec) asm volatile("s_waitcnt vmcnt(0)" ::: "memory");
+  }
+  if (coop || spec) __syncthreads();
   float rgb[3] = {0.f, 0.f, 0.f};
   const bool vis = idx < a.P && pr.visible;
   float J[JAC ? 9 : 1];
@@ -670,13 +705,14 @@
 template <bool JAC, bool LOD, bool DEFER>
 __global__ __launch_bounds__(kPreBlock) void preprocess_fwd_kernel(hgs_raster_args a, GeomWs g,
                                                                    int32_t* __restrict__ radii, uint32_t* __restrict__ super, uint32_t heavy_thr) {
-  preprocess_fwd_body<JAC, LOD, DEFER, false>(a, g, radii, super, heavy_thr);
+  preprocess_fwd_body<JAC, LOD, DEFER, false>(a, g, radii, super, heavy_thr, 0);
 }
 template <bool JAC>
 __global__ __launch_bounds__(kPreBlock, 4) void preprocess_fwd_h48_kernel(hgs_raster_args a, GeomWs g,
                                                                           int32_t* __restrict__ radii,
-                                                                          uint32_t* __restrict__ super, uint32_t heavy_thr) {
-  preprocess_fwd_body<JAC, false, false, true>(a, g, radii, super, heavy_thr);
+                                                                          uint32_t* __restrict__ super, uint32_t heavy_thr,
+                                                                          int speculate) {
+  preprocess_fwd_body<JAC, false, false, true>(a, g, radii, super, heavy_thr, speculate);
 }
 
 __global__ __launch_bounds__(1024) void scan_block_sums_kernel(uint32_t* __restrict__ sums0,
@@ -824,8 +860,9 @@
 }
 
 constexpr uint32_t kK8StageRec = 256;
+template <bool PRE = false>
 __device__ __forceinline__ void k8_sum_runs(const GeomWs& g, const float* __restrict__ inst, int idx, uint32_t n,
-                                            int presummed, float2* st, double (&s)[10]) {
+                                            int presummed, float2* st, double (&s)[10], uint32_t off_pre = 0u) {
   const int lane = threadIdx.x & 63;
   const unsigned long long long_mask = presummed ? __ballot(n > kK8LongRun) : 0ull;
   if (long_mask == 0ull) {
@@ -840,7 +877,7 @@
     if (total) {
       const unsigned long long nz = __ballot(n != 0u);
       const int first = __ffsll((long long)nz) - 1;
-      const uint32_t off_mine = n ? g.offsets[idx] : 0u;
+      const uint32_t off_mine = PRE ? off_pre : (n ? g.offsets[idx] : 0u);
       const size_t base = (size_t)__shfl(off_mine, first, 64);
       for (uint32_t c0 = 0; c0 < total; c0 += kK8StageRec) {
         const uint32_t cn = min(kK8StageRec, total - c0) * 5u;
@@ -874,7 +911,7 @@
       }
     }
   } else if (n != 0u) {
-    const size_t off = (size_t)g.offsets[idx];
+    const size_t off = (size_t)(PRE ? off_pre : g.offsets[idx]);
     if (n > kK8LongRun) {
       const uint32_t nseg = k8_nseg(n);
       for (uint32_t j = 0; j < nseg; ++j) {
@@ -895,24 +932,37 @@
   }
 }
 
-template <bool LOD>
-__device__ __forceinline__ void k8_chain(const hgs_raster_args& a, const GeomWs& g, int idx, const double (&s)[10],
-                                         float (&p)[3], float (&d_mean)[3], float (&d_m2)[3], float& d_op,
-                                         float (&d_scale)[3], float (&d_rot)[4], float (&d_c3)[6], float (&gr)[3]) {
+constexpr int kK8Pre = 11;
+template <bool LOD, bool PRE>
+__device__ __forceinline__ void k8_chain_impl(const hgs_raster_args& a, const GeomWs& g, int idx, const double (&s)[10],
+                                              float (&p)[3], float (&d_mean)[3], float (&d_m2)[3], float& d_op,
+                                              float (&d_scale)[3], float (&d_rot)[4], float (&d_c3)[6], float (&gr)[3],
+                                              const float (&pre)[kK8Pre], uint32_t pre_flags, const float* pre_tail,
+                                              const CamLds& pre_cam) {
+  static_assert(!(LOD && PRE), "early loads are the plain rows'");
   CamLds cam;
-  load_camera(a, cam);
+  if constexpr (PRE) cam = pre_cam;
+  else load_camera(a, cam);
   gr[0] = (float)s[6]; gr[1] = (float)s[7]; gr[2] = (float)s[8];
-  const uint32_t flags = g.flags[idx];
-  load_mean<LOD>(a, lod_row_gather<LOD>(a, idx), p);
+  const uint32_t flags = PRE ? pre_flags : g.flags[idx];
+  if constexpr (PRE) { p[0] = pre[0]; p[1] = pre[1]; p[2] = pre[2]; }
+  else load_mean<LOD>(a, lod_row_gather<LOD>(a, idx), p);
   float q[4] = {1.f, 0.f, 0.f, 0.f};
   float sc[3] = {1.f, 1.f, 1.f};
   double qnorm = 1.0;
   ProjD pd;
   if (a.cov3D_precomp) {
 #pragma unroll
-    for (int i = 0; i < 6; ++i) pd.c3[i] = (double)a.cov3D_precomp[(size_t)idx * 6 + i];
+    for (int i = 0; i < 6; ++i) pd.c3[i] = (double)(PRE ? pre[4 + i] : a.cov3D_precomp[(size_t)idx * 6 + i]);
   } else {
-    load_scale_rot<LOD>(a, idx, sc, q, &qnorm);
+    if constexpr (PRE) {
+      sc[0] = pre[4]; sc[1] = pre[5]; sc[2] = pre[6];
+      activate_scale(a, sc);
+      q[0] = pre[7]; q[1] = pre[8]; q[2] = pre[9]; q[3] = pre[10];
+      activate_rot(a, q, &qnorm);
+    } else {
+      load_scale_rot<LOD>(a, idx, sc, q, &qnorm);
+    }
     cov3d_from_scale_rot_d(sc, a.scale_modifier, q, pd);
   }
   project_gaussian_d(p, cam.vm, cam.pm, a.width, a.height, a.tanfovx, a.tanfovy, (flags & 8u) != 0,
@@ -1026,10 +1076,13 @@
   {
     float dod = 1.0f;
     double dact = 1.0;
-    const float o_act = load_opacity<LOD>(a, idx, &dact);
+    float o_act;
+    if constexpr (PRE) o_act = activate_opacity(a, pre_tail[0], &dact);
+    else o_act = load_opacity<LOD>(a, idx, &dact);
     float o_rec = o_act;
     if (a.interpolation_weights && a.num_node_kids && !a.lod_per_pixel)
-      o_rec = lod_opacity(o_act, a.interpolation_weights[idx], a.num_node_kids[idx], &dod);
+      o_rec = lod_opacity(o_act, PRE ? pre_tail[kPreBlock] : a.interpolation_weights[idx],
+                          PRE ? (int)__float_as_uint(pre_tail[2 * kPreBlock]) : a.num_node_kids[idx], &dod);
     const float sums5 = o_rec > 0.0f ? (float)(s[5] / (double)o_rec) : 0.0f;
     d_op = a.activations ? (float)((double)sums5 * (double)dod * dact) : sums5 * dod;
   }
@@ -1039,6 +1092,15 @@
     if (flags & 2u) gr[1] = 0.f;
     if (flags & 4u) gr[2] = 0.f;
   }
+}
+
+template <bool LOD>
+__device__ __forceinline__ void k8_chain(const hgs_raster_args& a, const GeomWs& g, int idx, const double (&s)[10],
+                                         float (&p)[3], float (&d_mean)[3], float (&d_m2)[3], float& d_op,
+                                         float (&d_scale)[3], float (&d_rot)[4], float (&d_c3)[6], float (&gr)[3]) {
+  const float none[kK8Pre] = {};
+  const CamLds no_cam = {};
+  k8_chain_impl<LOD, false>(a, g, idx, s, p, d_mean, d_m2, d_op, d_scale, d_rot, d_c3, gr, none, 0u, nullptr, no_cam);
 }
 
 template <bool ACC>
@@ -1388,6 +1450,10 @@
   d_mean[2] = __fmaf_rn(__fmaf_rn(-uz, dot, gdz), inv, d_mean[2] + 0.f);
 }
 
+constexpr size_t kK8StageBytes = (size_t)(kPreBlock / 64) * kK8StageRec * 5 * sizeof(float2);
+constexpr size_t kK8JacBytes = (size_t)kPreBlock * (9 + 3) * sizeof(float);
+static_assert(kK8StageBytes + kK8JacBytes <= (size_t)kPreBlock * (16 * 3 + 4) * sizeof(float), "no more than the M = 16 output stage");
+template <int EARLY>
 __global__ __launch_bounds__(kPreBlock) void preprocess_bwd_sh_kernel(hgs_raster_args a, GeomWs g,
                                                                          const float* __restrict__ inst,
                                                                          hgs_raster_grads out, int presummed) {
@@ -1396,11 +1462,48 @@
   const int idx = block_first + threadIdx.x;
   const bool in_range = idx < a.P;
   const uint32_t n = in_range ? g.tiles_touched[idx] : 0u;
+  constexpr bool pre_on = EARLY != 0;
+  float pre[kK8Pre] = {};
+  uint32_t pre_flags = 0u, pre_off = 0u;
+  float* jac_lds = reinterpret_cast<float*>(smem_raw + kK8StageBytes) + threadIdx.x;
+  float* tail_lds = jac_lds + 9 * kPreBlock;
+  CamLds cam = {};
+  if constexpr (pre_on) {
+    load_camera(a, cam);
+    const bool want = EARLY == 2 ? in_range : n != 0u;
+    const size_t li = want ? (size_t)idx : 0;
+    pre_off = g.offsets[li];
+    pre_flags = g.flags[li];
+    const float* jp = g.shjac + li * kJacStride;
+    float t_j[9];
+#pragma unroll
+    for (int k = 0; k < 9; ++k) t_j[k] = jp[k];
+    pre[0] = a.means3D[li * 3 + 0]; pre[1] = a.means3D[li * 3 + 1]; pre[2] = a.means3D[li * 3 + 2];
+    const float t_op = a.opacities[li];
+    const bool lodop = a.interpolation_weights && a.num_node_kids && !a.lod_per_pixel;
+    float t_w = 0.f;
+    int t_k = 0;
+    if (lodop) { t_w = a.interpolation_weights[li]; t_k = a.num_node_kids[li]; }
+    if (a.cov3D_precomp) {
+#pragma unroll
+      for (int i = 0; i < 6; ++i) pre[4 + i] = a.cov3D_precomp[li * 6 + i];
+    } else {
+      pre[4] = a.scales[li * 3 + 0]; pre[5] = a.scales[li * 3 + 1]; pre[6] = a.scales[li * 3 + 2];
+      const float4 qv = reinterpret_cast<const float4*>(a.rotations)[li];
+      pre[7] = qv.x; pre[8] = qv.y; pre[9] = qv.z; pre[10] = qv.w;
+    }
+#pragma unroll
+    for (int k = 0; k < 9; ++k) jac_lds[k * kPreBlock] = t_j[k];
+    tail_lds[0] = t_op;
+    tail_lds[kPreBlock] = t_w;
+    tail_lds[2 * kPreBlock] = __uint_as_float((uint32_t)t_k);
+  }
 
   double s[10];
 #pragma unroll
   for (int i = 0; i < 10; ++i) s[i] = 0.0;
-  k8_sum_runs(g, inst, idx, n, presummed, reinterpret_cast<float2*>(smem_raw) + (threadIdx.x >> 6) * (kK8StageRec * 5), s);
+  k8_sum_runs<pre_on>(g, inst, idx, n, presummed, reinterpret_cast<float2*>(smem_raw) + (threadIdx.x >> 6) * (kK8StageRec * 5), s,
+                      pre_off);
 
   float d_mean[3] = {0.f, 0.f, 0.f};
   float d_m2[3] = {0.f, 0.f, 0.f};
@@ -1412,7 +1515,7 @@
   float b[16];
   const int nb = (a.sh_degree + 1) * (a.sh_degree + 1);
   float p[3];
-  if (n != 0) k8_chain<false>(a, g, idx, s, p, d_mean, d_m2, d_op, d_scale, d_rot, d_c3, gr);
+  if (n != 0) k8_chain_impl<false, pre_on>(a, g, idx, s, p, d_mean, d_m2, d_op, d_scale, d_rot, d_c3, gr, pre, pre_flags, tail_lds, cam);
   if (in_range) {
     const float d_col[3] = {0.f, 0.f, 0.f};
     k8_store_row<false>(out, idx, d_m2, d_op, d_scale, d_rot, d_c3, d_col);
@@ -1420,12 +1523,12 @@
   __builtin_amdgcn_sched_barrier(0);
   if (n != 0) {
     float ux, uy, uz;
-    const float inv = unit_dir(p, a.campos, ux, uy, uz);
+    const float inv = unit_dir(p, pre_on ? cam.cam : a.campos, ux, uy, uz);
     sh_basis(a.sh_degree, ux, uy, uz, b);
     const float* jp = g.shjac + (size_t)idx * kJacStride;
     float J[9];
 #pragma unroll
-    for (int k = 0; k < 9; ++k) J[k] = jp[k];
+    for (int k = 0; k < 9; ++k) J[k] = pre_on ? jac_lds[k * kPreBlock] : jp[k];
     k8_add_view_term(gr, J, ux, uy, uz, inv, d_mean);
   } else {
 #pragma unroll
@@ -1706,20 +1809,28 @@
     if (g_sync[i].words == words) g_sync[i].dirty = true;
 }
 
+bool preprocess_fwd_is_h48(const hgs_raster_args& a) {
+  return a.shs && !a.shs_rest && !a.lod_render_indices && a.M == 16;
+}
+
 int launch_preprocess_fwd(const hgs_raster_args& a, const GeomWs& g, int32_t* radii, hipStream_t s, uint32_t* super,
-                          uint32_t heavy_thr) {
+                          uint32_t heavy_thr, bool speculate) {
   const int nblk = (a.P + kPreBlock - 1) / kPreBlock;
   if (nblk > 0) {
     const bool jac = a.prepare_backward && a.shs;
     const bool plain = a.shs && !a.shs_rest && !a.lod_render_indices && ((a.M * 3) & 3) == 0;
-    const bool h48 = plain && a.M == 16;
+    const bool h48 = preprocess_fwd_is_h48(a);
     const bool defer = plain && !h48;
     const size_t lds_bytes = !a.shs ? 0 : h48 ? (size_t)kK1ImageBytes : (size_t)kPreBlock * (a.M * 3 + 4) * sizeof(float);
-    auto k1 = a.lod_render_indices ? (jac ? preprocess_fwd_kernel<true, true, false> : preprocess_fwd_kernel<false, true, false>)
-              : h48   ? (jac ? preprocess_fwd_h48_kernel<true> : preprocess_fwd_h48_kernel<false>)
-              : defer ? (jac ? preprocess_fwd_kernel<true, false, true> : preprocess_fwd_kernel<false, false, true>)
-                      : (jac ? preprocess_fwd_kernel<true, false, false> : preprocess_fwd_kernel<false, false, false>);
-    hipLaunchKernelGGL(k1, dim3(nblk), dim3(kPreBlock), lds_bytes, s, a, g, radii, super, heavy_thr);
+    if (h48) {
+      hipLaunchKernelGGL(jac ? preprocess_fwd_h48_kernel<true> : preprocess_fwd_h48_kernel<false>, dim3(nblk), dim3(kPreBlock),
+                         lds_bytes, s, a, g, radii, super, heavy_thr, speculate ? 1 : 0);
+    } else {
+      auto k1 = a.lod_render_indices ? (jac ? preprocess_fwd_kernel<true, true, false> : preprocess_fwd_kernel<false, true, false>)
+                : defer ? (jac ? preprocess_fwd_kernel<true, false, true> : preprocess_fwd_kernel<false, false, true>)
+                        : (jac ? preprocess_fwd_kernel<true, false, false> : preprocess_fwd_kernel<false, false, false>);
+      hipLaunchKernelGGL(k1, dim3(nblk), dim3(kPreBlock), lds_bytes, s, a, g, radii, super, heavy_thr);
+    }
     HGS_LAUNCH_CHECK("preprocess_fwd", s, a.debug);
   }
   return HGS_OK;
@@ -1747,7 +1858,7 @@
 
 int launch_preprocess_bwd(const hgs_raster_args& a, const GeomWs& g, const float* inst_grads, float* drgb,
                           float* dmean_rows, const uint32_t* lod_flag, const hgs_raster_grads& out, uint32_t L,
-                          uint2* work, uint32_t* work_counter, hipStream_t s) {
+                          uint2* work, uint32_t* work_counter, hipStream_t s, int k8_early) {
   const int nblk = (a.P + kPreBlock - 1) / kPreBlock;
   if (nblk > 0) {
     static const char* force = getenv("HGS_K8_PRESUM");
@@ -1767,10 +1878,11 @@
                        !a.defer_sh_bwd && a.shs && !a.shs_rest && out.dL_dshs && a.prepare_backward && !a.colors_precomp &&
                        ((a.M * 3) & 3) == 0;
     if (fused) {
-      const size_t stage_bytes = (size_t)(kPreBlock / 64) * kK8StageRec * 5 * sizeof(float2);
+      const size_t stage_bytes = kK8StageBytes + (k8_early ? kK8JacBytes : 0);
       const size_t rows_bytes = (size_t)kPreBlock * (a.M * 3 + 4) * sizeof(float);
-      hipLaunchKernelGGL(preprocess_bwd_sh_kernel, dim3(nblk), dim3(kPreBlock),
-                         stage_bytes > rows_bytes ? stage_bytes : rows_bytes, s, a, g, inst_grads, out, presum ? 1 : 0);
+      auto k8 = k8_early == 0 ? preprocess_bwd_sh_kernel<0> : k8_early == 1 ? preprocess_bwd_sh_kernel<1> : preprocess_bwd_sh_kernel<2>;
+      hipLaunchKernelGGL(k8, dim3(nblk), dim3(kPreBlock), stage_bytes > rows_bytes ? stage_bytes : rows_bytes, s, a, g,
+                         inst_grads, out, presum ? 1 : 0);
       HGS_LAUNCH_CHECK("preprocess_bwd_sh", s, a.debug);
       return HGS_OK;
     }
```

Result: no change. 1522, median of 2 (+0.1%).
